# syl051088/DynaAlign

Hardware: AMD Instinct MI355X
Metric: sequence-pairs/sec (MinHash k=4 n_hash=500; NW BLOSUM62) at 1/2/4/8 MI355X (higher is better)
Workload: dtype u32

## Files before the change

### dynaalign_amd/csrc/api.cpp

```cpp
#include <sched.h>

#include <algorithm>
#include <atomic>
#include <chrono>
#include <climits>
#include <cmath>
#include <condition_variable>
#include <cstddef>
#include <map>
#include <memory>
#include <cstdlib>
#include <cstring>
#include <functional>
#include <mutex>
#include <random>
#include <string>
#include <thread>
#include <vector>

#include "da_common.hpp"

namespace da { size_t destroy_cached_comms(); }

namespace da {
// ... 202 lines not shown
  std::condition_variable cv_, done_;
  uint64_t gen_ = 0;
  bool stop_ = false;
  const std::function<void(size_t, size_t)> *fn_ = nullptr;
  size_t len_ = 0, part_ = 0;
  int pending_ = 0;
};

void widen_u16_to_f64(double *dst, const uint16_t *src, size_t b, size_t e, const double *table) {
  typedef double v2d __attribute__((ext_vector_type(2)));
  size_t i = b;
  if (i < e && (reinterpret_cast<uintptr_t>(dst + i) & 15)) { dst[i] = table[src[i]]; ++i; }
  for (; i + 2 <= e; i += 2) {
    const v2d v = {table[src[i]], table[src[i + 1]]};
    __builtin_nontemporal_store(v, reinterpret_cast<v2d *>(dst + i));
  }
  if (i < e) dst[i] = table[src[i]];
}

int d2h_pipelined(void *dst, const void *d_src, size_t bytes, const double *table = nullptr) {
  constexpr size_t CHUNK = (size_t)64 << 20, SMALL = (size_t)8 << 20;
  constexpr int RING = 4, MAX_WORKERS = 32;
  int WORKERS = table ? 16 : 8;
  if (da::config().d2h_threads > 0) WORKERS = std::min(MAX_WORKERS, da::config().d2h_threads);
  {
    const unsigned hw = std::thread::hardware_concurrency();
    cpu_set_t cs;
    int avail = (sched_getaffinity(0, sizeof cs, &cs) == 0) ? CPU_COUNT(&cs) : (int)hw;
    if (avail > 0 && WORKERS > avail) WORKERS = avail;
  }
  if (bytes <= CHUNK && !table) {
    DA_HIP_TRY(hipMemcpy(dst, d_src, bytes, hipMemcpyDeviceToHost));
    return DA_OK;
  }
  if (bytes <= SMALL && table) {
    std::vector<uint16_t> codes(bytes / 2);
    DA_HIP_TRY(hipMemcpy(codes.data(), d_src, bytes, hipMemcpyDeviceToHost));
    widen_u16_to_f64(static_cast<double *>(dst), codes.data(), 0, bytes / 2, table);
    return DA_OK;
  }
  if (da::config().plain_d2h && !table) {
    DA_HIP_TRY(hipMemcpy(dst, d_src, bytes, hipMemcpyDeviceToHost));
    return DA_OK;
  }
  struct Slot { void *pin = nullptr; hipEvent_t ev = nullptr; };
  Slot ring[RING];
  hipStream_t st = nullptr;
  int rc = DA_OK;
  auto cleanup = [&]() {
    if (st) (void)hipStreamSynchronize(st);
    for (auto &s : ring) { if (s.pin) (void)hipHostFree(s.pin); if (s.ev) (void)hipEventDestroy(s.ev); }
    if (st) (void)hipStreamDestroy(st);
  };
  auto check = [&](hipError_t e, const char *what) {
    if (e != hipSuccess && rc == DA_OK) rc = fail(DA_ERR_HIP, "%s failed: %s", what, hipGetErrorString(e));
    return e == hipSuccess;
  };
  if (!check(hipStreamCreateWithFlags(&st, hipStreamNonBlocking), "hipStreamCreate")) { cleanup(); return rc; }
  for (auto &s : ring)
    if (!check(hipHostMalloc(&s.pin, CHUNK, hipHostMallocDefault), "hipHostMalloc") ||
        !check(hipEventCreateWithFlags(&s.ev, hipEventDisableTiming), "hipEventCreate")) { cleanup(); return rc; }
  if (!check(hipDeviceSynchronize(), "hipDeviceSynchronize")) { cleanup(); return rc; }
  {
    CopyPool pool(WORKERS - 1);
    const size_t nchunk = (bytes + CHUNK - 1) / CHUNK;
    for (size_t c = 0; c < nchunk + RING - 1 && rc == DA_OK; ++c) {
      if (c < nchunk) {
        const size_t off = c * CHUNK, len = std::min(CHUNK, bytes - off);
        if (!check(hipMemcpyAsync(ring[c % RING].pin, static_cast<const char *>(d_src) + off, len, hipMemcpyDeviceToHost, st), "hipMemcpyAsync") ||
            !check(hipEventRecord(ring[c % RING].ev, st), "hipEventRecord")) break;
      }
      if (c >= RING - 1) {
        const size_t done = c - (RING - 1), off = done * CHUNK, len = std::min(CHUNK, bytes - off);
        if (!check(hipEventSynchronize(ring[done % RING].ev), "hipEventSynchronize")) break;
        const char *src = static_cast<const char *>(ring[done % RING].pin);
        if (table) {
          double *d = static_cast<double *>(dst) + off / 2;
          const uint16_t *s16 = reinterpret_cast<const uint16_t *>(src);
          pool.run_split(len / 2, [=](size_t b, size_t e) { widen_u16_to_f64(d, s16, b, e, table); });
        } else {
          char *d = static_cast<char *>(dst) + off;
          pool.run_split(len, [=](size_t b, size_t e) { memcpy(d + b, src + b, e - b); });
        }
      }
    }
  }
  cleanup();
  return rc;
}

struct Trace {
  const bool on = da::config().trace;
  const char *what;
  std::chrono::steady_clock::time_point t0 = std::chrono::steady_clock::now(), last = t0;
  explicit Trace(const char *w) : what(w) {}
  void mark(const char *step) {
    if (!on) return;
    (void)hipDeviceSynchronize();
    const auto now = std::chrono::steady_clock::now();
    fprintf(stderr, "[dynaalign] %s: %-28s %9.3f ms (total %9.3f ms)\n", what, step,
            std::chrono::duration<double, std::milli>(now - last).count(), std::chrono::duration<double, std::milli>(now - t0).count());
    last = now;
  }
};

double now_ms() { return std::chrono::duration<double, std::milli>(std::chrono::steady_clock::now().time_since_epoch()).count(); }

int64_t rows_per_block(int64_t n, size_t bytes_per_elem) {
  size_t free_b = 0, total_b = 0;
  if (hipMemGetInfo(&free_b, &total_b) != hipSuccess) free_b = (size_t)8 << 30;
  {
    int dev = 0;
    (void)hipGetDevice(&dev);
    std::lock_guard<std::mutex> g(big_cache().m);
    for (const auto &e : big_cache().parked) if (e.dev == dev) free_b += e.bytes;
  }
  size_t budget = free_b / 2;
  if (da::config().block_bytes) budget = (size_t)da::config().block_bytes;
  int64_t rows = (int64_t)(budget / ((size_t)n * bytes_per_elem));
  rows = rows / 128 * 128;
  if (rows < 128) rows = 128;
  return std::min(rows, n);
}

}
}

using namespace da;

namespace da {
namespace {
bool env_flag(const char *name) { return getenv(name) != nullptr; }
int64_t env_i64(const char *name, int64_t dflt) { const char *e = getenv(name); return e ? atoll(e) : dflt; }
uint64_t env_u64(const char *name, uint64_t dflt) { const char *e = getenv(name); return e ? strtoull(e, nullptr, 10) : dflt; }
enum MhExpand { MH_EXPAND_DEFAULT, MH_EXPAND_ROWS, MH_EXPAND_ROWSPIPE, MH_EXPAND_PIPE, MH_EXPAND_TILES };
Config parse_config() {
  Config c;
  c.mh_no_dedup = env_flag("DYNAALIGN_MH_NO_DEDUP");
  c.mh_no_sparse = env_flag("DYNAALIGN_MH_NO_SPARSE");
  c.mh_no_pipe = env_flag("DYNAALIGN_MH_NO_PIPE");
  c.mh_pipe_one_stream = env_flag("DYNAALIGN_MH_PIPE_ONE_STREAM");
  c.mh_dedup_min_n = env_i64("DYNAALIGN_MH_DEDUP_MIN_N", -1);
  c.mh_dedup_max_pct = env_i64("DYNAALIGN_MH_DEDUP_MAX_PCT", -1);
  c.mh_sparse_max_pairs = std::min<uint64_t>(env_u64("DYNAALIGN_MH_SPARSE_MAX_PAIRS", 400000000ull), 0xfffffff0ull);
  c.mh_no_hybrid = env_flag("DYNAALIGN_MH_NO_HYBRID");
  c.mh_hybrid_min_n = env_i64("DYNAALIGN_MH_HYBRID_MIN_N", -1);
  c.mh_hybrid_dedup = env_flag("DYNAALIGN_MH_HYBRID_DEDUP");
  if (const char *e = getenv("DYNAALIGN_MH_EXPAND"))
    c.mh_expand = !strcmp(e, "rows") ? MH_EXPAND_ROWS : !strcmp(e, "rowspipe") ? MH_EXPAND_ROWSPIPE : !strcmp(e, "pipe") ? MH_EXPAND_PIPE
                : !strcmp(e, "tiles") ? MH_EXPAND_TILES : MH_EXPAND_DEFAULT;
  c.mh_pipe_step = (int)std::max<int64_t>(0, env_i64("DYNAALIGN_MH_PIPE_STEP", 0));
  c.mh_pipe_wg = (int)std::max<int64_t>(0, std::min<int64_t>(4, env_i64("DYNAALIGN_MH_PIPE_WG", 0)));
  c.mh_pipe_head = (int)std::max<int64_t>(0, env_i64("DYNAALIGN_MH_PIPE_HEAD", 0));
  const int pb = (int)env_i64("DYNAALIGN_PLANE_BITS", 0);
  c.plane_bits = (pb == 32 || pb == 16 || pb == 15 || pb == 14 || pb == 12) ? pb : 0;
  c.k2_no_asm = env_flag("DYNAALIGN_K2_NO_ASM");
  c.k2_persist = env_flag("DYNAALIGN_K2_PERSIST");
  c.k2_wg_per_cu = (int)std::max<int64_t>(0, env_i64("DYNAALIGN_K2_WG_PER_CU", 0));
  c.nw_no_dedup = env_flag("DYNAALIGN_NW_NO_DEDUP");
  c.nw_int32 = env_flag("DYNAALIGN_NW_INT32");
  c.nw_no_prefix = env_flag("DYNAALIGN_NW_NO_PREFIX_SHARE");
  c.nw_dedup_min_n = env_i64("DYNAALIGN_NW_DEDUP_MIN_N", -1);
  c.no_host_widen = env_flag("DYNAALIGN_NO_HOST_WIDEN");
  c.plain_d2h = env_flag("DYNAALIGN_PLAIN_D2H");
  c.no_buffer_cache = env_flag("DYNAALIGN_NO_BUFFER_CACHE");
  c.d2h_threads = (int)std::max<int64_t>(0, env_i64("DYNAALIGN_D2H_THREADS", 0));
  c.buffer_cache_pct = (int)std::max<int64_t>(0, std::min<int64_t>(90, env_i64("DYNAALIGN_BUFFER_CACHE_PCT", 30)));
  c.block_bytes = env_u64("DYNAALIGN_BLOCK_BYTES", 0);
  c.trace = env_flag("DYNAALIGN_TRACE");
  c.louvain_debug = env_flag("DYNAALIGN_LOUVAIN_DEBUG");
  c.louvain_threads = (int)std::max<int64_t>(0, env_i64("DYNAALIGN_LOUVAIN_THREADS", 0));
  return c;
}
std::atomic<const Config *> g_config{nullptr};
}
const Config &config() {
  const Config *c = g_config.load(std::memory_order_acquire);
  if (!c) {
    const Config *fresh = new Config(parse_config());
    if (g_config.compare_exchange_strong(c, fresh, std::memory_order_acq_rel)) c = fresh;
    else delete fresh;
  }
  return *c;
}
}
extern "C" void da_config_reload(void) { da::g_config.store(new da::Config(da::parse_config()), std::memory_order_release); }

extern "C" {

const char *da_last_error(void) { return last_error_ref().c_str(); }

const char *da_status_message(int status) {
  switch (status) {
    case DA_ERR_EMPTY_INPUT: return "Input sequences vector cannot be empty";
    case DA_ERR_BAD_K: return "'k' must be a positive integer";
    case DA_ERR_BAD_NHASH: return "Number of hash functions must be positive";
    case DA_ERR_BAD_MATRIX: return "Invalid substitution matrix name: %s";
    case DA_ERR_BAD_RESIDUE_SEQ1: return "Invalid amino acid in sequence1: %c";
    case DA_ERR_BAD_RESIDUE_SEQ2: return "Invalid amino acid in sequence2: %c";
    case DA_ERR_NOMEM: return "out of memory";
    case DA_ERR_NO_DEVICE: return "no usable HIP device";
    case DA_ERR_HIP: return "HIP runtime error";
    case DA_ERR_UNSUPPORTED: return "unsupported by the gfx950 kernels";
    case DA_ERR_BAD_ARG: return "bad argument";
    default: return "";
  }
}

int da_abi_version(void) { return DA_ABI_VERSION; }

size_t da_release_device_memory(void) {
  (void)da::destroy_cached_comms();
  return big_cache().release(-1);
}

int da_device_count(void) {
  int cnt = 0;
  if (hipGetDeviceCount(&cnt) != hipSuccess) return 0;
  return cnt;
}

int da_hash_family_seeds(uint32_t seed, int n_hash, uint32_t *seeds_out) {
  if (n_hash < 0 || (n_hash > 0 && !seeds_out)) return fail(DA_ERR_BAD_ARG, "bad n_hash / seeds_out");
  uint32_t s[624];
  s[0] = seed;
  for (uint32_t i = 1; i < 624; ++i) s[i] = 1812433253u * (s[i - 1] ^ (s[i - 1] >> 30)) + i;
  int pos = 624;
  for (int o = 0; o < n_hash; ++o) {
    if (pos == 624) {
      for (int i = 0; i < 624; ++i) {
        const uint32_t y = (s[i] & 0x80000000u) | (s[(i + 1) % 624] & 0x7fffffffu);
        s[i] = s[(i + 397) % 624] ^ (y >> 1) ^ ((y & 1u) ? 0x9908b0dfu : 0u);
      }
      pos = 0;
    }
    uint32_t y = s[pos++];
    y ^= y >> 11;
    y ^= (y << 7) & 0x9d2c5680u;
    y ^= (y << 15) & 0xefc60000u;
    y ^= y >> 18;
    seeds_out[o] = y;
  }
  return DA_OK;
}

uint32_t da_random_seed(void) { return std::random_device{}(); }

int da_matrix_id(const char *matrix_name) {
  if (matrix_name)
    for (int i = 0; i < matrix_count_host(); ++i)
      if (strcmp(matrix_name, matrix_name_host(i)) == 0) return i;
  fail(DA_ERR_BAD_MATRIX, "Invalid substitution matrix name: %s", matrix_name ? matrix_name : "");
  return -1;
}


int da_dev_minhash_signatures(const uint8_t *d_residues, const int64_t *d_offsets, int64_t n,
                              int64_t total_residues, int64_t max_len, int k, int n_hash,
                              const uint32_t *d_seeds, uint32_t *d_sig, int64_t ld_sig, void *stream) {
  (void)total_residues; (void)max_len;
  int rc = validate_mh(n, k, n_hash);
  if (rc != DA_OK) return rc;
  if (!d_residues || !d_offsets || !d_seeds || !d_sig) return fail(DA_ERR_BAD_ARG, "NULL device pointer");
  if (ld_sig < n_hash) return fail(DA_ERR_BAD_ARG, "ld_sig (%lld) < n_hash (%d)", (long long)ld_sig, n_hash);
  return launch_minhash_signatures(d_residues, d_offsets, n, k, n_hash, d_seeds, d_sig, ld_sig,
                                   static_cast<hipStream_t>(stream));
}

static int env_plane_bits() { return da::config().plane_bits; }
struct Dictionary { bool ok = false; int max_ids = 0, bits_data = 32; int *d_status = nullptr; };
static int run_dictionary(const uint32_t *d_sig, int64_t ld_sig, int64_t n, int n_hash, int min_bits, void *d_work, size_t work_bytes,
                          Dictionary *dict, hipStream_t stream) {
  if (n > DA_DICT_MAX_N || min_bits == 32) return DA_OK;
  if (!d_work || work_bytes < mh_planes_workspace_bytes(n, n_hash))
    return fail(DA_ERR_BAD_ARG, "workspace smaller than da_mh_planes_workspace_bytes(n, n_hash)");
  int rc;
  if ((rc = launch_mh_dictionary(d_sig, ld_sig, n, n_hash, d_work, &dict->d_status, stream)) != DA_OK) return rc;
  int status[2] = {0, 0};
  DA_HIP_TRY(hipMemcpyAsync(status, dict->d_status, sizeof(status), hipMemcpyDeviceToHost, stream));
  DA_HIP_TRY(hipStreamSynchronize(stream));
  dict->ok = status[0] == 0; dict->max_ids = status[1];
  dict->bits_data = dict->ok ? mh_plane_bits_for(status[1]) : 32;
  return DA_OK;
}
static int planes_from(const Dictionary &dict, const uint32_t *d_sig, int64_t ld_sig, int64_t n, int n_hash, int min_bits, const void *d_work,
                       uint32_t *d_planes, int *bits_out, hipStream_t stream) {
  *bits_out = dict.ok ? std::max(dict.bits_data, min_bits) : 32;
  return dict.ok ? launch_ids_to_planes(d_work, n, n_hash, *bits_out, d_planes, stream) : launch_sig_to_planes(d_sig, ld_sig, n, n_hash, d_planes, stream);
}
static int build_planes(const uint32_t *d_sig, int64_t ld_sig, int64_t n, int n_hash, int min_bits, void *d_work,
                        size_t work_bytes, uint32_t *d_planes, int *bits_out, hipStream_t stream) {
  min_bits = std::max(min_bits, env_plane_bits());
  Dictionary dict;
  const int rc = run_dictionary(d_sig, ld_sig, n, n_hash, min_bits, d_work, work_bytes, &dict, stream);
  return rc != DA_OK ? rc : planes_from(dict, d_sig, ld_sig, n, n_hash, min_bits, d_work, d_planes, bits_out, stream);
}

size_t da_mh_planes_workspace_bytes(int64_t n, int n_hash) { return mh_planes_workspace_bytes(n, n_hash); }
int64_t da_mh_planes_words(int64_t n, int n_hash) { return mh_planes_words(n, n_hash); }

int da_dev_mh_planes(const uint32_t *d_sig, int64_t ld_sig, int64_t n, int n_hash, int min_plane_bits, void *d_work,
                     size_t work_bytes, uint32_t *d_planes, int64_t planes_words, int *plane_bits_out, void *stream) {
  if (n <= 0) return fail(DA_ERR_EMPTY_INPUT, "%s", da_status_message(DA_ERR_EMPTY_INPUT));
  if (n_hash <= 0) return fail(DA_ERR_BAD_NHASH, "%s", da_status_message(DA_ERR_BAD_NHASH));
  if (!d_sig || !d_planes || !plane_bits_out) return fail(DA_ERR_BAD_ARG, "NULL pointer");
  if (ld_sig < n_hash) return fail(DA_ERR_BAD_ARG, "ld_sig (%lld) < n_hash (%d)", (long long)ld_sig, n_hash);
  if (min_plane_bits != 0 && min_plane_bits != 12 && min_plane_bits != 14 && min_plane_bits != 15 && min_plane_bits != 16 && min_plane_bits != 32)
    return fail(DA_ERR_BAD_ARG, "min_plane_bits must be 0, 12, 14, 15, 16 or 32 (got %d)", min_plane_bits);
  if ((reinterpret_cast<uintptr_t>(d_planes) & 15) || planes_words < mh_planes_words(n, n_hash))
    return fail(DA_ERR_BAD_ARG, "bit-plane buffer must be 16-byte aligned and hold da_mh_planes_words(n, n_hash) = %lld words",
                (long long)mh_planes_words(n, n_hash));
  if (reinterpret_cast<uintptr_t>(d_work) & 255) return fail(DA_ERR_BAD_ARG, "workspace must be 256-byte aligned");
  return build_planes(d_sig, ld_sig, n, n_hash, min_plane_bits, d_work, work_bytes, d_planes, plane_bits_out,
                      static_cast<hipStream_t>(stream));
}

int da_dev_mh_compare(const uint32_t *d_planes, int plane_bits, int64_t n, int n_hash,
                      int64_t row_begin, int64_t row_end, int symmetric, int kind, void *d_out,
                      int64_t ld, void *stream) {
  if (n <= 0) return fail(DA_ERR_EMPTY_INPUT, "%s", da_status_message(DA_ERR_EMPTY_INPUT));
  if (n_hash <= 0) return fail(DA_ERR_BAD_NHASH, "%s", da_status_message(DA_ERR_BAD_NHASH));
  if (!d_planes || !d_out) return fail(DA_ERR_BAD_ARG, "NULL device pointer");
  if (row_begin < 0 || row_end > n || row_begin > row_end) return fail(DA_ERR_BAD_ARG, "bad row range");
  if (symmetric && (row_begin != 0 || row_end != n))
    return fail(DA_ERR_BAD_ARG, "symmetric mode needs the full row range");
  if (ld < n) return fail(DA_ERR_BAD_ARG, "ld (%lld) < n (%lld)", (long long)ld, (long long)n);
  if (kind != DA_OUT_F64 && kind != DA_OUT_COMPACT) return fail(DA_ERR_BAD_ARG, "bad output kind");
  if (n_hash > 65535)
    return fail(DA_ERR_UNSUPPORTED, "the compare kernel counts in 16 bits: n_hash <= 65535 (got %d)", n_hash);
  if (reinterpret_cast<uintptr_t>(d_planes) & 15) return fail(DA_ERR_BAD_ARG, "bit-plane buffer must be 16-byte aligned");
  if (plane_bits != 8 && plane_bits != 12 && plane_bits != 14 && plane_bits != 15 && plane_bits != 16 && plane_bits != 32)
    return fail(DA_ERR_BAD_ARG, "plane_bits must be 8, 12, 14, 15, 16 or 32 (got %d)", plane_bits);
  return launch_mh_compare(d_planes, n, n_hash, row_begin, row_end, symmetric != 0, kind, d_out, ld,
                           static_cast<hipStream_t>(stream), plane_bits);
}

namespace {
struct PipeRes { hipStream_t side = nullptr, alt[2] = {nullptr, nullptr}; std::vector<hipEvent_t> ev; int dev = 0; };
struct PipePool { std::mutex m; std::vector<PipeRes *> idle[64]; };
static PipePool &pipe_pool() { static PipePool *p = new PipePool; return *p; }
static PipeRes *pipe_acquire(size_t events) {
  int dev = 0;
  if (hipGetDevice(&dev) != hipSuccess) return nullptr;
  PipeRes *r = nullptr;
  {
    std::lock_guard<std::mutex> g(pipe_pool().m);
    auto &v = pipe_pool().idle[dev & 63];
    if (!v.empty()) { r = v.back(); v.pop_back(); }
  }
  if (!r) {
    r = new PipeRes;
    r->dev = dev;
    if (hipStreamCreateWithFlags(&r->side, hipStreamNonBlocking) != hipSuccess || hipStreamCreateWithFlags(&r->alt[0], hipStreamNonBlocking) != hipSuccess ||
        hipStreamCreateWithFlags(&r->alt[1], hipStreamNonBlocking) != hipSuccess) { delete r; return nullptr; }
  }
  while (r->ev.size() < events) {
    hipEvent_t e = nullptr;
    if (hipEventCreate(&e) != hipSuccess) break;
    r->ev.push_back(e);
  }
  if (r->ev.size() < events) { std::lock_guard<std::mutex> g(pipe_pool().m); pipe_pool().idle[dev & 63].push_back(r); return nullptr; }
  return r;
}
struct PipeLease {
  PipeRes *const r;
  explicit PipeLease(size_t events, bool want = true) : r(want ? pipe_acquire(events) : nullptr) {}
  ~PipeLease() {
    if (!r) return;
    (void)hipStreamSynchronize(r->side); (void)hipStreamSynchronize(r->alt[0]); (void)hipStreamSynchronize(r->alt[1]);
    std::lock_guard<std::mutex> g(pipe_pool().m);
    pipe_pool().idle[r->dev & 63].push_back(r);
  }
};
static int count_unique(const uint8_t *d_bytes, const int64_t *d_offsets, int64_t n, const NwDedupPlan &p, hipStream_t stream, int64_t *U) {
  int rc;
  if ((rc = launch_nw_dedup_count(d_bytes, d_offsets, n, p, stream)) != DA_OK) return rc;
  int32_t M = 0, S = 0;
  DA_HIP_TRY(hipMemcpyAsync(&M, p.pm + n, 4, hipMemcpyDeviceToHost, stream));
  DA_HIP_TRY(hipMemcpyAsync(&S, p.ps + n, 4, hipMemcpyDeviceToHost, stream));
  DA_HIP_TRY(hipStreamSynchronize(stream));
  *U = (int64_t)M + S; return DA_OK;
}
enum MhForm { MH_DIRECT = 0, MH_TILES = 1, MH_SPARSE = 2, MH_TILES_PIPE = 3, MH_ROWS = 4, MH_ROWS_PIPE = 5 };
struct MhRoute { int64_t n = 0, unique = 0, hybrid_pairs = -1; int taken = MH_DIRECT, plane_bits = 0, chunks = 0, expand_launches = 0, hybrid_bits_before = 0; bool packed_table = false; float ms[6] = {0, 0, 0, 0, 0, 0}; };
static MhRoute &mh_route() { static thread_local MhRoute r; return r; }
struct MhEvents {
  hipEvent_t e[7] = {nullptr, nullptr, nullptr, nullptr, nullptr, nullptr, nullptr};
  ~MhEvents() { for (hipEvent_t x : e) if (x) (void)hipEventDestroy(x); }
  hipEvent_t operator[](int i) const { return e[i]; }
  static void ms(MhRoute &r, int i, hipEvent_t from, hipEvent_t to) { (void)hipEventElapsedTime(&r.ms[i], from, to); }
  void steps(MhRoute &r, int count) const { for (int i = 0; i < count; ++i) ms(r, i, e[i], e[i + 1]); }
};
struct LaunchUnion {
  hipEvent_t origin; float total = 0, covered_to = 0;
  void add(hipEvent_t begin, hipEvent_t end) {
    float b = 0, e = 0;
    (void)hipEventElapsedTime(&b, origin, begin); (void)hipEventElapsedTime(&e, origin, end);
    if (e > covered_to) { total += e - std::max(b, covered_to); covered_to = e; }
  }
};
struct MhDedup { int64_t U = 0; bool take = false, rows = false; DevBuf work; NwDedupPlan p{}; std::vector<int32_t> ub; };
static int mh_dedup_plan(const uint8_t *d_res, const int64_t *d_off, int64_t n, int64_t total, int n_hash, const double *d_out, int64_t ld,
                         MhDedup *d, hipStream_t stream) {
  const Config &cfg = da::config();
  int rc;
  d->U = n;
  const int64_t min_n = cfg.mh_dedup_min_n >= 0 ? cfg.mh_dedup_min_n : 2048;
  if (n < min_n || n > 0x7ffffff0LL || total <= 0 || n_hash > 2047 || cfg.mh_no_dedup) return DA_OK;
  if ((rc = d->work.alloc(nw_dedup_workspace_bytes(n, total))) != DA_OK) return rc;
  d->p = nw_dedup_layout(d->work.p, n, total);
  if ((rc = count_unique(d_res, d_off, n, d->p, stream, &d->U)) != DA_OK) return rc;
  const int64_t U = d->U;
  const int64_t max_pct = cfg.mh_dedup_max_pct >= 0 ? cfg.mh_dedup_max_pct
                        : expand_stream_ok(n, std::min<int64_t>(U, 65536), n_hash, d_out, ld) ? 68 : 60;
  d->take = U > 0 && U * 100 <= n * max_pct && expand_rows_workspace_bytes(n, U, DA_OUT_F64, false, n_hash, 0) != 0;
  if (!d->take) return DA_OK;
  if ((rc = launch_nw_dedup_build(d_res, d_off, n, U, d->p, stream, true)) != DA_OK) return rc;
  d->rows = cfg.mh_expand <= MH_EXPAND_ROWSPIPE && expand_stream_ok(n, U, n_hash, d_out, ld);
  if (d->rows) return DA_OK;
  const int64_t NB = mh_sym_bands(n);
  std::vector<int32_t> b((size_t)NB);
  d->ub.resize((size_t)NB + 1);
  DA_HIP_TRY(hipMemcpy2DAsync(d->ub.data(), 4, d->p.pm, 4096, 4, (size_t)NB, hipMemcpyDeviceToHost, stream));
  DA_HIP_TRY(hipMemcpy2DAsync(b.data(), 4, d->p.ps, 4096, 4, (size_t)NB, hipMemcpyDeviceToHost, stream));
  DA_HIP_TRY(hipStreamSynchronize(stream));
  for (int64_t q = 0; q < NB; ++q) d->ub[(size_t)q] += b[(size_t)q];
  d->ub[(size_t)NB] = (int32_t)U;
  return DA_OK;
}
constexpr int HY_KEEP = 254;
enum class MhOperand { dense, sparse, split };
struct MhAdmission { MhOperand form = MhOperand::dense; uint64_t pairs = 0; const uint16_t *codes = nullptr, *dense = nullptr; int64_t ld_ids = 0; };
static int mh_admit(const Dictionary &dict, void *d_work, int64_t n, int n_hash, bool ask_sparse, int split_from_bits, MhAdmission *a,
                    hipStream_t stream) {
  const Config &cfg = da::config();
  if (!dict.ok || env_plane_bits() != 0) return DA_OK;
  const int64_t hy_min_n = cfg.mh_hybrid_min_n >= 0 ? cfg.mh_hybrid_min_n : 16384;
  const bool sparse_ok = ask_sparse && dict.max_ids >= 1 && dict.max_ids <= 32768 && n >= 2048 && n_hash + 1 <= 2048 && !cfg.mh_no_sparse;
  const bool split_ok = dict.bits_data >= split_from_bits && dict.bits_data <= 16 && dict.max_ids <= 32768 && n >= hy_min_n && n <= 131072 &&
                        n_hash > 32 && n_hash + 1 <= 2048 && !cfg.mh_no_hybrid && !cfg.k2_no_asm;
  if (!sparse_ok && !split_ok) return DA_OK;
  int rc;
  int64_t ld_ids = 0;
  const uint16_t *ids = mh_dictionary_codes(d_work, n, n_hash, &ld_ids);
  unsigned long long *d_stats = reinterpret_cast<unsigned long long *>(dict.d_status + 4);
  const uint16_t *dense = nullptr, *rare = nullptr;
  unsigned long long st[4] = {0, 0, 0, 0};
  if ((rc = split_ok ? launch_mh_heavy_split(d_work, n, n_hash, dict.max_ids, HY_KEEP, &dense, &rare, d_stats, stream)
                     : launch_mh_sparse_count(ids, ld_ids, n, n_hash, dict.max_ids, d_stats, stream)) != DA_OK) return rc;
  DA_HIP_TRY(hipMemcpyAsync(split_ok ? st : st + 2, d_stats, split_ok ? sizeof(st) : 16, hipMemcpyDeviceToHost, stream));
  DA_HIP_TRY(hipStreamSynchronize(stream));
  const double pairs_all = 0.5 * (double)n * (double)(n - 1);
  if (sparse_ok && st[2] <= mh_sparse_pairs_limit() && st[3] <= 4096 && (double)st[2] <= pairs_all * (double)n_hash / 5000.0)
    *a = MhAdmission{MhOperand::sparse, st[2], ids, nullptr, ld_ids};
  else if (split_ok && st[0] <= mh_sparse_pairs_limit() && st[1] <= 4096 && (double)st[0] <= pairs_all * (double)n_hash / 25000.0)
    *a = MhAdmission{MhOperand::split, st[0], rare, dense, ld_ids};
  return DA_OK;
}
struct MhCodes {
  DevBuf sig, planes, pwork, scratch, entries32, entries;
  int64_t m = 0;
  int n_hash = 0, bits = 32;
  Dictionary dict;
  MhAdmission adm;
  bool split() const { return adm.form == MhOperand::split; }
  int lists(hipStream_t st) const {
    return launch_mh_sparse_lists(adm.codes, adm.ld_ids, m, n_hash, dict.max_ids, adm.pairs, scratch.as<uint32_t>(), entries32.as<uint32_t>(), entries.as<uint16_t>(), st);
  }
  int fixup(int kind, void *out, int64_t ld_out, hipStream_t st, int64_t tr0 = 0, int64_t tr1 = -1) const {
    return launch_mh_sparse_fixup(scratch.as<uint32_t>(), entries.as<uint16_t>(), m, n_hash, dict.max_ids, adm.ld_ids, kind, out, ld_out, tr0,
                                  tr1 < 0 ? (m + 127) / 128 : tr1, st);
  }
};
static int mh_codes(const uint8_t *d_res, const int64_t *d_off, int64_t m, int k, int n_hash, const uint32_t *d_seeds, bool ask_sparse,
                    int split_from_bits, MhCodes *c, hipStream_t stream) {
  int rc;
  const int64_t lds = sig_ld_for(n_hash);
  const size_t wb = mh_planes_workspace_bytes(m, n_hash);
  c->m = m; c->n_hash = n_hash;
  if ((rc = c->sig.alloc((size_t)m * lds * sizeof(uint32_t))) != DA_OK || (rc = c->planes.alloc((size_t)mh_planes_words(m, n_hash) * sizeof(uint32_t))) != DA_OK ||
      (rc = c->pwork.alloc(wb)) != DA_OK) return rc;
  uint32_t *sig = c->sig.as<uint32_t>(), *planes = c->planes.as<uint32_t>();
  if ((rc = launch_minhash_signatures(d_res, d_off, m, k, n_hash, d_seeds, sig, lds, stream)) != DA_OK) return rc;
  const int min_bits = env_plane_bits();
  const Dictionary &dict = c->dict;
  if ((rc = run_dictionary(sig, lds, m, n_hash, min_bits, c->pwork.p, wb, &c->dict, stream)) != DA_OK) return rc;
  if ((rc = mh_admit(dict, c->pwork.p, m, n_hash, ask_sparse, split_from_bits, &c->adm, stream)) != DA_OK) return rc;
  if (c->adm.form != MhOperand::dense &&
      (c->scratch.alloc(mh_sparse_scratch_words(m, n_hash, dict.max_ids, c->adm.ld_ids) * 4) != DA_OK ||
       c->entries32.alloc((size_t)c->adm.pairs * 4 + 16) != DA_OK || c->entries.alloc((size_t)c->adm.pairs * 2 + 16) != DA_OK)) {
    (void)hipGetLastError();
    c->scratch.release(); c->entries32.release(); c->entries.release();
    c->adm = MhAdmission();
  }
  if (c->adm.form == MhOperand::sparse) { c->bits = 0; return DA_OK; }
  if (c->split()) { c->bits = 8; return launch_ids_to_planes(c->pwork.p, m, n_hash, 8, planes, stream, c->adm.dense); }
  return planes_from(dict, sig, lds, m, n_hash, min_bits, c->pwork.p, planes, &c->bits, stream);
}
struct MhCall {
  int64_t n; int n_hash; double *out; int64_t ld; hipStream_t stream; MhRoute &route; const MhEvents &ev; const MhCodes &c; const MhDedup &d;
  uint16_t *dtab = nullptr; int64_t ld_d = 0; void *ex = nullptr; bool pk = false;
};
constexpr int MH_NO_PIPE = -1;
static int mh_finish(const MhCall &k, int last_event, MhForm taken, int steps) {
  DA_HIP_TRY(hipEventRecord(k.ev[last_event], k.stream));
  DA_HIP_TRY(hipStreamSynchronize(k.stream));
  k.route.taken = taken; k.ev.steps(k.route, steps);
  return DA_OK;
}
static int mh_sparse(const MhCall &k) {
  const MhCodes &c = k.c;
  int rc;
  if ((rc = launch_mh_sparse(c.adm.codes, c.adm.ld_ids, k.n, k.n_hash, c.dict.max_ids, c.adm.pairs, c.scratch.as<uint32_t>(), c.entries32.as<uint32_t>(),
                             c.entries.as<uint16_t>(), k.out, k.ld, k.stream, k.ev[3])) != DA_OK || (rc = mh_finish(k, 4, MH_SPARSE, 3)) != DA_OK) return rc;
  k.route.unique = (int64_t)c.adm.pairs;
  MhEvents::ms(k.route, 4, k.ev[3], k.ev[4]);
  return DA_OK;
}
static int mh_direct(const MhCall &k) {
  const MhCodes &c = k.c;
  int rc;
  const PipeLease lease(1, c.split());
  PipeRes *const pr = lease.r;
  if (pr) {
    DA_HIP_TRY(hipStreamWaitEvent(pr->side, k.ev[2], 0));
    if ((rc = c.lists(pr->side)) != DA_OK) return rc;
    DA_HIP_TRY(hipEventRecord(pr->ev[0], pr->side));
  } else if (c.split() && (rc = c.lists(k.stream)) != DA_OK) return rc;
  if ((rc = launch_mh_compare(c.planes.as<uint32_t>(), k.n, k.n_hash, 0, k.n, true, DA_OUT_F64, k.out, k.ld, k.stream, c.bits)) != DA_OK) return rc;
  if (pr) DA_HIP_TRY(hipStreamWaitEvent(k.stream, pr->ev[0], 0));
  if (c.split() && (rc = c.fixup(DA_OUT_F64, k.out, k.ld, k.stream)) != DA_OK) return rc;
  return mh_finish(k, 3, MH_DIRECT, 3);
}
static int mh_one_stream(const MhCall &k) {
  const MhCodes &c = k.c;
  int rc;
  if (c.split() && (rc = c.lists(k.stream)) != DA_OK) return rc;
  if ((rc = k.pk ? launch_mh_compare_pk(c.planes.as<uint32_t>(), k.d.U, k.n_hash, reinterpret_cast<uint8_t *>(k.dtab), k.stream)
                 : launch_mh_compare(c.planes.as<uint32_t>(), k.d.U, k.n_hash, 0, k.d.U, true, DA_OUT_COMPACT, k.dtab, k.ld_d, k.stream, c.bits)) != DA_OK)
    return rc;
  if (c.split() && (rc = c.fixup(DA_OUT_COMPACT, k.dtab, k.ld_d, k.stream)) != DA_OK) return rc;
  DA_HIP_TRY(hipEventRecord(k.ev[3], k.stream));
  if ((rc = k.d.rows ? launch_expand_stream(k.dtab, k.ld_d, k.d.p.uidx, k.n, k.d.U, k.n_hash, k.out, k.ld, k.ex, k.stream, k.ev[4], k.pk)
                     : launch_expand_unique(k.dtab, k.ld_d, k.d.p.uidx, k.n, DA_OUT_F64, false, k.n_hash, k.out, k.ld, k.stream, 0,
                                            static_cast<uint16_t *>(k.ex), k.d.p.ufirst, k.d.U, k.ev[4], k.ev[5])) != DA_OK) return rc;
  k.route.chunks = k.route.expand_launches = 1;
  return k.d.rows ? mh_finish(k, 5, MH_ROWS, 5) : mh_finish(k, 6, MH_TILES, 6);
}
static int mh_rows_pipe(const MhCall &k) {
  const Config &cfg = da::config();
  const MhCodes &c = k.c;
  const int64_t U = k.d.U, KB = mh_sym_bands(U);
  const hipStream_t stream = k.stream;
  int rc;
  const bool two = expand_stream_packed(k.n_hash);
  const int wg = cfg.mh_pipe_wg > 0 ? cfg.mh_pipe_wg : two ? 2 : 1, head = cfg.mh_pipe_head > 0 ? cfg.mh_pipe_head : two ? 1 : 4,
            step = cfg.mh_pipe_step > 0 ? cfg.mh_pipe_step : two ? 8 : 4;
  const bool alt = !cfg.mh_pipe_one_stream;
  std::vector<int64_t> cuts{0};
  while (cuts.back() < KB) cuts.push_back(std::min(KB, cuts.back() + (cuts.size() == 1 ? head : step)));
  const size_t C = cuts.size() - 1;
  const PipeLease lease(3 * C + 2);
  PipeRes *const pr = lease.r;
  if (!pr) return MH_NO_PIPE;
  hipEvent_t *pe = pr->ev.data();
  DA_HIP_TRY(hipStreamWaitEvent(pr->side, k.ev[2], 0));
  if ((rc = launch_mh_compare_edges_u16(c.planes.as<uint32_t>(), U, k.n_hash, k.dtab, k.ld_d, stream, c.bits, k.pk)) != DA_OK) return rc;
  if ((rc = launch_expand_stream_lists(k.d.p.uidx, k.n, U, k.ex, stream)) != DA_OK) return rc;
  DA_HIP_TRY(hipEventRecord(pe[3 * C], stream));
  if (c.split()) {
    if ((rc = c.lists(stream)) != DA_OK) return rc;
    DA_HIP_TRY(hipEventRecord(pe[3 * C + 1], stream));
  }
  if (alt) { DA_HIP_TRY(hipStreamWaitEvent(pr->alt[0], pe[3 * C], 0)); DA_HIP_TRY(hipStreamWaitEvent(pr->alt[1], pe[3 * C], 0)); }
  for (size_t ci = 0; ci < C; ++ci) {
    if ((rc = launch_mh_compare_bands_u16(c.planes.as<uint32_t>(), U, k.n_hash, k.dtab, k.ld_d, cuts[ci], cuts[ci + 1], ci == 0 ? 4 : wg, pr->side, c.bits,
                                          k.pk)) != DA_OK) return rc;
    if (c.split()) {
      if (ci == 0) { DA_HIP_TRY(hipStreamWaitEvent(pr->side, pe[3 * C], 0)); DA_HIP_TRY(hipStreamWaitEvent(pr->side, pe[3 * C + 1], 0)); }
      if ((rc = c.fixup(DA_OUT_COMPACT, k.dtab, k.ld_d, pr->side, cuts[ci] * 8, cuts[ci + 1] * 8)) != DA_OK) return rc;
    }
    DA_HIP_TRY(hipEventRecord(pe[3 * ci], pr->side));
    const hipStream_t es = alt ? pr->alt[ci & 1] : stream;
    DA_HIP_TRY(hipStreamWaitEvent(es, pe[3 * ci], 0));
    DA_HIP_TRY(hipEventRecord(pe[3 * ci + 1], es));
    if ((rc = launch_expand_stream_rows(k.dtab, k.ld_d, k.d.p.uidx, k.n, U, k.n_hash, k.out, k.ld, k.ex, cuts[ci] * 1024, cuts[ci + 1] * 1024, es,
                                        (int)ci, k.pk)) != DA_OK) return rc;
    DA_HIP_TRY(hipEventRecord(pe[3 * ci + 2], es));
  }
  if (alt) for (size_t ci = (C >= 2 ? C - 2 : 0); ci < C; ++ci) DA_HIP_TRY(hipStreamWaitEvent(stream, pe[3 * ci + 2], 0));
  if ((rc = mh_finish(k, 5, MH_ROWS_PIPE, 2)) != DA_OK) return rc;
  k.route.chunks = k.route.expand_launches = (int)C;
  MhEvents::ms(k.route, 2, k.ev[2], pe[3 * (C - 1)]);
  MhEvents::ms(k.route, 3, k.ev[2], pe[3 * C]);
  LaunchUnion expand{k.ev[2]};
  for (size_t ci = 0; ci < C; ++ci) expand.add(pe[3 * ci + 1], pe[3 * ci + 2]);
  k.route.ms[4] = expand.total;
  return DA_OK;
}
static int mh_tiles_pipe(const MhCall &k) {
  const Config &cfg = da::config();
  const MhCodes &c = k.c;
  uint16_t *ftab = static_cast<uint16_t *>(k.ex);
  const hipStream_t stream = k.stream;
  const std::vector<int32_t> &ub = k.d.ub;
  const int64_t U = k.d.U, KB = mh_sym_bands(U), NB = (int64_t)ub.size() - 1, ld_f = ceil_div(k.n, 8) * 8;
  int rc;
  const int step = cfg.mh_pipe_step > 0 ? cfg.mh_pipe_step : 4, wg = cfg.mh_pipe_wg > 0 ? cfg.mh_pipe_wg : 2;
  const bool alt = !cfg.mh_pipe_one_stream;
  struct Chunk { int64_t kb0, kb1, ob0, ob1; };
  std::vector<Chunk> chunks;
  for (int64_t kb = 0, ob = 0; kb < KB;) {
    const int64_t kb1 = std::min(KB, kb + (chunks.empty() ? 1 : step));
    int64_t ob1 = ob;
    if (kb1 == KB) ob1 = NB;
    else while (ob1 < NB && (int64_t)ub[(size_t)ob1 + 1] <= kb1 * 1024) ++ob1;
    chunks.push_back({kb, kb1, ob, ob1});
    kb = kb1; ob = ob1;
  }
  const size_t C = chunks.size();
  const PipeLease lease(5 * C);
  PipeRes *const pr = lease.r;
  if (!pr) return MH_NO_PIPE;
  hipEvent_t *pe = pr->ev.data();
  DA_HIP_TRY(hipStreamWaitEvent(pr->side, k.ev[2], 0));
  if ((rc = launch_mh_compare_edges_u16(c.planes.as<uint32_t>(), U, k.n_hash, k.dtab, k.ld_d, pr->side, c.bits)) != DA_OK) return rc;
  if (c.split() && (rc = c.lists(pr->side)) != DA_OK) return rc;
  for (size_t ci = 0; ci < C; ++ci) {
    const Chunk &ch = chunks[ci];
    if ((rc = launch_mh_compare_bands_u16(c.planes.as<uint32_t>(), U, k.n_hash, k.dtab, k.ld_d, ch.kb0, ch.kb1, wg, pr->side, c.bits)) != DA_OK) return rc;
    if (c.split() && (rc = c.fixup(DA_OUT_COMPACT, k.dtab, k.ld_d, pr->side, ch.kb0 * 8, ch.kb1 * 8)) != DA_OK) return rc;
    DA_HIP_TRY(hipEventRecord(pe[5 * ci], pr->side));
    DA_HIP_TRY(hipStreamWaitEvent(stream, pe[5 * ci], 0));
    DA_HIP_TRY(hipEventRecord(pe[5 * ci + 1], stream));
    if ((rc = launch_gather_columns(k.dtab, k.ld_d, k.d.p.uidx, k.d.p.ufirst, k.n, U, ftab, ld_f, false, stream, 1, 0, ch.kb0 * 1024,
                                    std::min(U, ch.kb1 * 1024))) != DA_OK) return rc;
    DA_HIP_TRY(hipEventRecord(pe[5 * ci + 2], stream));
    const hipStream_t es = alt ? pr->alt[ci & 1] : stream;
    if (alt) DA_HIP_TRY(hipStreamWaitEvent(es, pe[5 * ci + 2], 0));
    DA_HIP_TRY(hipEventRecord(pe[5 * ci + 3], es));
    if ((rc = launch_expand_rows(ftab, ld_f, k.d.p.uidx, k.n, false, k.n_hash, 0, k.out, k.ld, ch.ob0, ch.ob1, es)) != DA_OK) return rc;
    DA_HIP_TRY(hipEventRecord(pe[5 * ci + 4], es));
  }
  if (alt) for (size_t ci = (C >= 2 ? C - 2 : 0); ci < C; ++ci) DA_HIP_TRY(hipStreamWaitEvent(stream, pe[5 * ci + 4], 0));
  DA_HIP_TRY(hipEventRecord(k.ev[5], stream));
  if ((rc = launch_expand_unique(k.dtab, k.ld_d, k.d.p.uidx, k.n, DA_OUT_F64, false, k.n_hash, k.out, k.ld, stream, 0, ftab, k.d.p.ufirst, U,
                                 nullptr, nullptr, 1, 0, true)) != DA_OK) return rc;
  if ((rc = mh_finish(k, 6, MH_TILES_PIPE, 2)) != DA_OK) return rc;
  k.route.chunks = (int)C;
  MhEvents::ms(k.route, 2, k.ev[2], pe[5 * (C - 1)]);
  LaunchUnion expand{k.ev[2]};
  for (size_t ci = 0; ci < C; ++ci) {
    float g = 0;
    (void)hipEventElapsedTime(&g, pe[5 * ci + 1], pe[5 * ci + 2]);
    k.route.ms[3] += g;
    if (chunks[ci].ob1 > chunks[ci].ob0) { ++k.route.expand_launches; expand.add(pe[5 * ci + 3], pe[5 * ci + 4]); }
  }
  k.route.ms[4] = expand.total;
  MhEvents::ms(k.route, 5, k.ev[5], k.ev[6]);
  return DA_OK;
}
}

static int mh_full_symmetric(const uint8_t *d_res, const int64_t *d_off, int64_t n, int64_t total, int k, int n_hash,
                             const uint32_t *d_seeds, double *d_out, int64_t ld, hipStream_t stream) {
  const Config &cfg = da::config();
  int rc;
  MhRoute &route = mh_route() = MhRoute();
  route.n = n;
  MhEvents ev;
  for (auto &e : ev.e) DA_HIP_TRY(hipEventCreate(&e));
  DA_HIP_TRY(hipEventRecord(ev[0], stream));
  MhDedup d;
  if ((rc = mh_dedup_plan(d_res, d_off, n, total, n_hash, d_out, ld, &d, stream)) != DA_OK) return rc;
  route.unique = d.U;
  DA_HIP_TRY(hipEventRecord(ev[1], stream));
  MhCodes c;
  if ((rc = mh_codes(d.take ? d.p.ucodes : d_res, d.take ? d.p.uoff : d_off, d.take ? d.U : n, k, n_hash, d_seeds, !d.take && d.U * 10 >= n * 9,
                     d.take && !cfg.mh_hybrid_dedup ? 13 : 12, &c, stream)) != DA_OK) return rc;
  route.plane_bits = c.bits;
  if (c.split()) { route.hybrid_pairs = (int64_t)c.adm.pairs; route.hybrid_bits_before = c.dict.bits_data; }
  DA_HIP_TRY(hipEventRecord(ev[2], stream));
  MhCall call{n, n_hash, d_out, ld, stream, route, ev, c, d};
  if (!d.take) return c.adm.form == MhOperand::sparse ? mh_sparse(call) : mh_direct(call);
  DevBuf dtab, ex;
  call.pk = d.rows && !c.split() && mh_compare_pk_ok(d.U, n_hash, c.bits);
  route.packed_table = call.pk;
  call.ld_d = call.pk ? pk_lo_bytes(d.U) : (d.U + 7) / 8 * 8;
  if ((rc = dtab.alloc(call.pk ? pk_table_bytes(d.U) : (size_t)d.U * (size_t)call.ld_d * 2)) != DA_OK) return rc;
  if ((rc = ex.alloc(d.rows ? expand_stream_scratch_bytes(n, d.U) : expand_rows_workspace_bytes(n, d.U, DA_OUT_F64, false, n_hash, 0))) != DA_OK) return rc;
  call.dtab = dtab.as<uint16_t>(); call.ex = ex.p;
  const bool pipe = !cfg.mh_no_pipe && mh_compare_bands_ok(d.U, n_hash, c.bits, dtab.p, call.ld_d) &&
                    (d.rows ? cfg.mh_expand != MH_EXPAND_ROWS : cfg.mh_expand != MH_EXPAND_TILES && (ld & 1) == 0 && (reinterpret_cast<uintptr_t>(d_out) & 15) == 0);
  if (pipe && (rc = d.rows ? mh_rows_pipe(call) : mh_tiles_pipe(call)) != MH_NO_PIPE) return rc;
  return mh_one_stream(call);
}

int da_dev_similarity_mh(const uint8_t *d_residues, const int64_t *d_offsets, int64_t n, int64_t total_residues, int k, int n_hash,
                         const uint32_t *d_seeds, double *d_out, int64_t ld, void *stream) {
  int rc = validate_mh(n, k, n_hash);
  if (rc != DA_OK) return rc;
  if (!d_residues || !d_offsets || !d_seeds || !d_out) return fail(DA_ERR_BAD_ARG, "NULL device pointer");
  if (ld < n) return fail(DA_ERR_BAD_ARG, "ld (%lld) < n (%lld)", (long long)ld, (long long)n);
  if (n_hash > 65535) return fail(DA_ERR_UNSUPPORTED, "the compare kernel counts in 16 bits: n_hash <= 65535 (got %d); da_similarity_mh handles more", n_hash);
  return mh_full_symmetric(d_residues, d_offsets, n, total_residues, k, n_hash, d_seeds, d_out, ld, static_cast<hipStream_t>(stream));
}

int da_mh_last_route_chunks(int *chunks_out, int *expand_launches_out) {
  const MhRoute &r = mh_route();
  if (chunks_out) *chunks_out = r.chunks;
  if (expand_launches_out) *expand_launches_out = r.expand_launches;
  return DA_OK;
}

int da_mh_last_route_split(int64_t *rare_incidences_out, int *plane_bits_without_out) {
  const MhRoute &r = mh_route();
  if (rare_incidences_out) *rare_incidences_out = r.hybrid_pairs;
  if (plane_bits_without_out) *plane_bits_without_out = r.hybrid_bits_before;
  return DA_OK;
}

extern "C" int da_debug_mh_last_table_packed(int *packed_out) {
  if (!packed_out) return fail(DA_ERR_BAD_ARG, "NULL pointer");
  *packed_out = mh_route().packed_table ? 1 : 0;
  return DA_OK;
}

int da_mh_last_route(int64_t *n_out, int64_t *unique_out, int *dedup_taken_out, int *plane_bits_out, double *ms6_out) {
  const MhRoute &r = mh_route();
  if (n_out) *n_out = r.n;
  if (unique_out) *unique_out = r.unique;
  if (dedup_taken_out) *dedup_taken_out = r.taken;
  if (plane_bits_out) *plane_bits_out = r.plane_bits;
  if (ms6_out) for (int i = 0; i < 6; ++i) ms6_out[i] = r.ms[i];
  return DA_OK;
}

size_t da_dev_unique_plan_bytes(int64_t n, int64_t total_bytes) {
  if (n <= 0) return 256;
  return nw_dedup_workspace_bytes(n, total_bytes > 0 ? total_bytes : 1);
}

int da_dev_unique_plan(const uint8_t *d_bytes, const int64_t *d_offsets, int64_t n, int64_t total_bytes, void *d_work, size_t work_bytes,
                       da_unique_plan *plan, void *stream_v) {
  if (!plan || plan->struct_size < sizeof(da_unique_plan)) return fail(DA_ERR_BAD_ARG, "da_unique_plan: NULL or struct_size too small");
  if (n <= 0) return fail(DA_ERR_EMPTY_INPUT, "%s", da_status_message(DA_ERR_EMPTY_INPUT));
  if (n > 0x7ffffff0LL) return fail(DA_ERR_UNSUPPORTED, "unique plan: n too large");
  if (!d_bytes || !d_offsets || !d_work) return fail(DA_ERR_BAD_ARG, "NULL device pointer");
  if ((reinterpret_cast<uintptr_t>(d_work) & 255) || work_bytes < da_dev_unique_plan_bytes(n, total_bytes))
    return fail(DA_ERR_BAD_ARG, "workspace must be 256-byte aligned and hold da_dev_unique_plan_bytes(n, total_bytes) bytes");
  hipStream_t stream = static_cast<hipStream_t>(stream_v);
  int rc;
  const NwDedupPlan p = nw_dedup_layout(d_work, n, total_bytes > 0 ? total_bytes : 1);
  int64_t U = 0;
  if ((rc = count_unique(d_bytes, d_offsets, n, p, stream, &U)) != DA_OK) return rc;
  if (U <= 0 || U > n) return fail(DA_ERR_HIP, "unique plan: inconsistent counts (%lld unique of %lld)", (long long)U, (long long)n);
  if ((rc = launch_nw_dedup_build(d_bytes, d_offsets, n, U, p, stream)) != DA_OK) return rc;
  plan->n = n; plan->unique = U;
  plan->d_uidx = p.uidx; plan->d_ufirst = p.ufirst; plan->d_ulast = p.ulast;
  plan->d_ubytes = p.ucodes; plan->d_uoffsets = p.uoff;
  plan->d_minfirst = p.minfirst; plan->d_maxlast = p.maxlast;
  return DA_OK;
}

int da_dev_shards_to_table(const void *d_gathered, int64_t ld_g, int64_t n, int world, int value_bits, uint16_t *d_table, int64_t ld_table,
                           void *stream) {
  if (n <= 0) return fail(DA_ERR_EMPTY_INPUT, "%s", da_status_message(DA_ERR_EMPTY_INPUT));
  if (!d_gathered || !d_table) return fail(DA_ERR_BAD_ARG, "NULL device pointer");
  if (world < 1 || ld_table < n) return fail(DA_ERR_BAD_ARG, "bad world / leading dimension");
  if (value_bits != 0 && (value_bits < 1 || value_bits > 16)) return fail(DA_ERR_BAD_ARG, "value_bits must be 0 (uint16 blocks) or 1..16");
  const ShardGeom g = shard_geom(n, world, 128);
  if (value_bits == 0 && ld_g < g.W) return fail(DA_ERR_BAD_ARG, "ld_g (%lld) < da_shard_ld (%lld)", (long long)ld_g, (long long)g.W);
  return launch_shards_to_table(d_gathered, ld_g, g, value_bits, d_table, ld_table, static_cast<hipStream_t>(stream));
}

size_t da_dev_expand_workspace_bytes(int64_t n, int64_t unique, int is_nw, int n_hash, int nw_max_len) {
  const size_t b = expand_rows_workspace_bytes(n, unique, DA_OUT_F64, is_nw != 0, n_hash, nw_max_len);
  return b ? b : 256;
}

int da_dev_expand_unique(const uint16_t *d_table, int64_t ld_table, int table_world, const da_unique_plan *plan, int is_nw, int n_hash,
                         int nw_max_len, void *d_work, size_t work_bytes, double *d_out, int64_t ld, void *stream) {
  if (!plan || plan->struct_size < sizeof(da_unique_plan) || !plan->d_uidx || !plan->d_ufirst) return fail(DA_ERR_BAD_ARG, "bad da_unique_plan");
  if (!d_table || !d_out) return fail(DA_ERR_BAD_ARG, "NULL device pointer");
  const int64_t n = plan->n, U = plan->unique;
  if (n <= 0 || U <= 0 || U > n || ld < n || ld_table < U) return fail(DA_ERR_BAD_ARG, "bad sizes / leading dimensions");
  if (!is_nw && (n_hash <= 0 || n_hash > 65535)) return fail(DA_ERR_BAD_NHASH, "%s", da_status_message(DA_ERR_BAD_NHASH));
  if (table_world < 1) return fail(DA_ERR_BAD_ARG, "table_world must be >= 1");
  const int64_t rows_local = table_world > 1 ? ceil_div(ceil_div(U, 128), table_world) * 128 : 0;
  if (!is_nw && table_world == 1 && expand_stream_ok(n, U, n_hash, d_out, ld) && (ld_table & 7) == 0 && ld_table <= 65536 &&
      (reinterpret_cast<uintptr_t>(d_table) & 15) == 0) {
    const size_t lists_bytes = expand_stream_scratch_bytes(n, U);
    if (d_work && work_bytes >= lists_bytes && (reinterpret_cast<uintptr_t>(d_work) & 15) == 0)
      return launch_expand_stream(d_table, ld_table, plan->d_uidx, n, U, n_hash, d_out, ld, d_work, static_cast<hipStream_t>(stream));
    DevBuf lists;
    int rc = lists.alloc(lists_bytes);
    if (rc != DA_OK) return rc;
    rc = launch_expand_stream(d_table, ld_table, plan->d_uidx, n, U, n_hash, d_out, ld, lists.p, static_cast<hipStream_t>(stream));
    DA_HIP_TRY(hipStreamSynchronize(static_cast<hipStream_t>(stream)));
    return rc;
  }
  const size_t need = expand_rows_workspace_bytes(n, U, DA_OUT_F64, is_nw != 0, n_hash, nw_max_len);
  uint16_t *d_F = (need && d_work && work_bytes >= need && (reinterpret_cast<uintptr_t>(d_work) & 15) == 0) ? static_cast<uint16_t *>(d_work) : nullptr;
  if ((ld_table & 7) || (reinterpret_cast<uintptr_t>(d_table) & 15)) d_F = nullptr;
  return launch_expand_unique(d_table, ld_table, plan->d_uidx, n, DA_OUT_F64, is_nw != 0, n_hash, d_out, ld, static_cast<hipStream_t>(stream),
                              nw_max_len, d_F, plan->d_ufirst, U, nullptr, nullptr, table_world, rows_local);
}

size_t da_dev_unique_rows_bytes(int64_t n, int64_t unique) {
  if (n <= 0 || unique <= 0) return 256;
  return (size_t)unique * (size_t)(ceil_div(n, 8) * 8) * 2;
}

int da_dev_unique_rows(const uint16_t *d_table, int64_t ld_table, const da_unique_plan *plan, uint16_t *d_rows, void *stream) {
  if (!plan || plan->struct_size < sizeof(da_unique_plan) || !plan->d_uidx || !plan->d_ufirst) return fail(DA_ERR_BAD_ARG, "bad da_unique_plan");
  if (!d_table || !d_rows) return fail(DA_ERR_BAD_ARG, "NULL device pointer");
  if (ld_table < plan->unique) return fail(DA_ERR_BAD_ARG, "ld_table < unique");
  return launch_gather_columns(d_table, ld_table, plan->d_uidx, plan->d_ufirst, plan->n, plan->unique, d_rows, ceil_div(plan->n, 8) * 8, true,
                               static_cast<hipStream_t>(stream));
}

int da_dev_nw_unique_rows(const da_unique_plan *plan, int64_t max_len, int matrix_id, int gap_open, int gap_ext, int rank, int world,
                          uint16_t *d_out, int64_t ld, void *stream) {
  if (!plan || plan->struct_size < sizeof(da_unique_plan) || !plan->d_ubytes || !plan->d_uoffsets || !plan->d_ufirst || !plan->d_minfirst ||
      !plan->d_maxlast)
    return fail(DA_ERR_BAD_ARG, "bad da_unique_plan");
  if (!d_out) return fail(DA_ERR_BAD_ARG, "NULL device pointer");
  const int64_t U = plan->unique;
  if (world < 1 || rank < 0 || rank >= world || ld < U) return fail(DA_ERR_BAD_ARG, "bad rank / world / leading dimension");
  if (matrix_id < 0 || matrix_id >= matrix_count_host()) return fail(DA_ERR_BAD_MATRIX, "%s", da_status_message(DA_ERR_BAD_MATRIX));
  if (max_len < 1 || max_len > 64 || gap_open < 0 || gap_ext < 0)
    return fail(DA_ERR_UNSUPPORTED, "the ordered unique-table sweep serves sequences of 1..64 residues and penalties >= 0");
  return launch_nw(plan->d_ubytes, plan->d_uoffsets, U, max_len, matrix_id, gap_open, gap_ext, 0, U, false, DA_OUT_COMPACT, d_out, ld, nullptr, 0,
                   static_cast<hipStream_t>(stream), rank, world > 1 ? world : 0, plan->d_ufirst, plan->d_minfirst, plan->d_maxlast);
}

int da_dev_nw_encode(const uint8_t *d_residues, int64_t total_residues, uint8_t *d_codes,
                     int32_t *d_bad, void *stream) {
  if (total_residues > 0 && (!d_residues || !d_codes || !d_bad)) return fail(DA_ERR_BAD_ARG, "NULL device pointer");
  return launch_nw_encode(d_residues, total_residues, d_codes, d_bad, static_cast<hipStream_t>(stream));
}

struct NwRoute { int64_t n = 0, unique = 0; int taken = 0; float plan_ms = 0, dp_ms = 0, expand_ms = 0; };
static NwRoute &nw_route() { static thread_local NwRoute r; return r; }

static int nw_full_symmetric(const uint8_t *d_codes, const int64_t *d_offsets, int64_t n, int64_t total, int64_t max_len, int mid,
                             int gap_open, int gap_ext, int kind, void *d_out, int64_t ld, hipStream_t stream, int64_t *unique_out = nullptr) {
// ... 1178 lines not shown
```

### dynaalign_amd/csrc/da_common.hpp

```cpp
#pragma once

#include <hip/hip_runtime.h>

#include <cstdarg>
#include <cstdint>
#include <cstdio>
#include <string>

#include "../../include/dynaalign.h"

namespace da {
struct Config {
  bool mh_no_dedup = false, mh_no_sparse = false, mh_no_pipe = false, mh_pipe_one_stream = false;
  int64_t mh_dedup_min_n = -1, mh_dedup_max_pct = -1;
  uint64_t mh_sparse_max_pairs = 400000000ull;
  bool mh_no_hybrid = false, mh_hybrid_dedup = false;
  int64_t mh_hybrid_min_n = -1;
  int mh_expand = 0;
  int mh_pipe_step = 0, mh_pipe_wg = 0, mh_pipe_head = 0;
  int plane_bits = 0;
  bool k2_no_asm = false, k2_persist = false;
  int k2_wg_per_cu = 0;
  bool nw_no_dedup = false, nw_int32 = false, nw_no_prefix = false;
  int64_t nw_dedup_min_n = -1;
  bool no_host_widen = false, plain_d2h = false, no_buffer_cache = false;
  int d2h_threads = 0, buffer_cache_pct = 30;
  uint64_t block_bytes = 0;
  bool trace = false, louvain_debug = false;
  int louvain_threads = 0;
};
const Config &config();


std::string &last_error_ref();
int fail(int code, const char *fmt, ...) __attribute__((format(printf, 2, 3)));

#define DA_HIP_TRY(expr)                                                              \
  do {                                                                                \
    hipError_t _e = (expr);                                                           \
    if (_e != hipSuccess)                                                             \
      return ::da::fail(_e == hipErrorNoDevice || _e == hipErrorInvalidDevice         \
                            ? DA_ERR_NO_DEVICE                                        \
                            : DA_ERR_HIP,                                             \
                        "%s failed: %s (%s:%d)", #expr, hipGetErrorString(_e),        \
                        __FILE__, __LINE__);                                          \
  } while (0)

inline int64_t ceil_div(int64_t a, int64_t b) { return (a + b - 1) / b; }

struct ShardGeom {
  int64_t n, W, rows;
  int world, tile, T, Q, Qh;
};
__host__ __device__ inline int64_t shard_back(int64_t W, int64_t n) { return W - ((n + 7) / 8) * 8; }
inline ShardGeom shard_geom(int64_t n, int world, int tile) {
  ShardGeom g;
  g.n = n; g.world = world; g.tile = tile;
  g.T = (int)ceil_div(n, tile);
  g.Q = (int)ceil_div(g.T, world);
  g.Qh = (g.Q + 1) / 2;
  g.W = ceil_div(n, 8) * 8 + (int64_t)world * tile;
  g.rows = (int64_t)g.Qh * tile;
  return g;
}

__host__ __device__ inline int k2_slot(int r) { return (((r >> 5) * 2 + (r & 1)) << 4) + ((r & 31) >> 1); }
__host__ __device__ inline int k2_row_of_slot(int s) { return ((s >> 5) << 5) + ((s & 15) << 1) + ((s >> 4) & 1); }
struct PlaneGeom {
  int pl;
  int sp;
  int segs;
  int nst;
  int64_t blocks, copy_words;
};
__host__ __device__ inline PlaneGeom plane_geom(int64_t n, int n_hash, int pl) {
  PlaneGeom g;
  g.pl = pl; g.sp = pl == 32 ? 16 : pl; g.segs = g.sp / 4;
  g.nst = ((n_hash + 31) / 32) * (pl / g.sp);
  g.blocks = (n + 127) / 128;
  g.copy_words = g.blocks * g.nst * 128 * g.sp;
  return g;
}
__host__ __device__ inline int64_t plane_unit_word(const PlaneGeom &g, int64_t row, int st, int seg) {
  const int rs = k2_slot((int)(row & 127));
  const int xs = g.segs == 4 ? (rs >> 2) & 3 : 0;
  return ((((row >> 7) * g.nst + st) * 128 + rs) * g.segs + (seg ^ xs)) * 4;
}
constexpr int K2_PAD16_SLOT_WORDS = 20;
__host__ __device__ inline int64_t pad16_copy_words(int64_t n, int n_hash) {
  return ((n + 127) / 128) * (int64_t)((n_hash + 31) / 32) * 128 * K2_PAD16_SLOT_WORDS;
}
__host__ __device__ inline int64_t pad16_base_words(int64_t n, int n_hash) { return 2 * plane_geom(n, n_hash, 16).copy_words; }
__host__ __device__ inline int64_t pad16_slot_word(int64_t n, int n_hash, int64_t row, int group) {
  const int64_t nst = (n_hash + 31) / 32;
  return (((row >> 7) * nst + group) * 128 + k2_slot((int)(row & 127))) * K2_PAD16_SLOT_WORDS;
}
inline int64_t mh_planes_words(int64_t n, int n_hash) {
  if (n <= 0 || n_hash <= 0) return 0;
  const int64_t raw = 2 * plane_geom(n, n_hash, 32).copy_words;
  const int64_t p16 = pad16_base_words(n, n_hash) + 2 * pad16_copy_words(n, n_hash);
  return raw > p16 ? raw : p16;
}

__host__ __device__ inline int64_t pk_lo_bytes(int64_t U) { return (U + 127) / 128 * 128; }
__host__ __device__ inline int64_t pk_row_bytes(int64_t lo_bytes) { return lo_bytes + lo_bytes / 8; }
inline size_t pk_table_bytes(int64_t U) { return (size_t)U * (size_t)pk_row_bytes(pk_lo_bytes(U)); }

int launch_minhash_signatures(const uint8_t *d_res, const int64_t *d_off, int64_t n,
                              int k, int n_hash, const uint32_t *d_seeds, uint32_t *d_sig,
                              int64_t ld_sig, hipStream_t stream);
int launch_mh_compare(const uint32_t *d_planes, int64_t n, int n_hash,
                      int64_t row_begin, int64_t row_end, bool symmetric, int kind,
                      void *d_out, int64_t ld, hipStream_t stream, int plane_bits = 32, int tile_stride = 1,
                      bool upper_only = false, int fold_q = 0, int64_t fold_w = 0);
int64_t mh_sym_bands(int64_t n);
int64_t mh_sym_band_prefix(int64_t n, int64_t band);
bool mh_compare_bands_ok(int64_t n, int n_hash, int plane_bits, const void *d_out, int64_t ld);
int launch_mh_compare_bands_u16(const uint32_t *d_planes, int64_t n, int n_hash, uint16_t *d_out, int64_t ld, int64_t band_begin,
                                int64_t band_end, int wg_per_cu, hipStream_t stream, int plane_bits = 12, bool pk = false);
int launch_mh_compare_edges_u16(const uint32_t *d_planes, int64_t n, int n_hash, uint16_t *d_out, int64_t ld, hipStream_t stream, int plane_bits = 12,
                                bool pk = false);
bool mh_compare_pk_ok(int64_t n, int n_hash, int plane_bits);
int launch_mh_compare_pk(const uint32_t *d_planes, int64_t n, int n_hash, uint8_t *d_tab, hipStream_t stream);
size_t mh_sparse_pairs_limit();
int launch_mh_sparse_count(const uint16_t *d_idsT, int64_t ld_ids, int64_t n, int n_hash, int max_ids, unsigned long long *d_stats, hipStream_t stream);
size_t mh_sparse_scratch_words(int64_t n, int n_hash, int max_ids, int64_t ld_ids);
int launch_mh_sparse(const uint16_t *d_idsT, int64_t ld_ids, int64_t n, int n_hash, int max_ids, uint64_t pairs, uint32_t *d_scratch,
                     uint32_t *d_entries32, uint16_t *d_entries, double *d_out, int64_t ld, hipStream_t stream, hipEvent_t after_buckets = nullptr);
int launch_mh_sparse_lists(const uint16_t *d_idsT, int64_t ld_ids, int64_t n, int n_hash, int max_ids, uint64_t pairs, uint32_t *d_scratch,
                           uint32_t *d_entries32, uint16_t *d_entries, hipStream_t stream);
int launch_mh_sparse_fixup(const uint32_t *d_scratch, const uint16_t *d_entries, int64_t n, int n_hash, int max_ids, int64_t ld_ids, int kind, void *d_out,
                           int64_t ld, int64_t tile_row_begin, int64_t tile_row_end, hipStream_t stream);
const uint16_t *mh_dictionary_codes(const void *d_work, int64_t n, int n_hash, int64_t *ld_ids);
constexpr int64_t DA_DICT_MAX_N = 131068;
size_t mh_planes_workspace_bytes(int64_t n, int n_hash);
int launch_mh_dictionary(const uint32_t *d_sig, int64_t ld_sig, int64_t n, int n_hash, void *d_work,
                         int **d_status_out, hipStream_t stream);
int mh_plane_bits_for(int max_ids);
int launch_ids_to_planes(const void *d_work, int64_t n, int n_hash, int plane_bits, uint32_t *d_planes,
                         hipStream_t stream, const uint16_t *d_codes = nullptr);
int launch_mh_heavy_split(void *d_work, int64_t n, int n_hash, int max_ids, int keep, const uint16_t **d_dense_out, const uint16_t **d_sparse_out,
                          unsigned long long *d_stats, hipStream_t stream);
int launch_sig_to_planes(const uint32_t *d_sig, int64_t ld_sig, int64_t n, int n_hash, uint32_t *d_planes,
                         hipStream_t stream);
int launch_finalize_sharded(const uint16_t *d_g, int64_t ld_g, const ShardGeom &geom, bool is_nw, int n_hash,
                            double *d_out, int64_t ld, hipStream_t stream);
int64_t shard_packed_bytes(const ShardGeom &g, int value_bits);
int launch_shards_to_table(const void *d_g, int64_t ld_g, const ShardGeom &geom, int value_bits, uint16_t *d_table, int64_t ld,
                           hipStream_t stream);
int launch_pack_shard(const uint16_t *d_local, int64_t ld, const ShardGeom &geom, int value_bits, uint8_t *d_packed,
                      hipStream_t stream);
int launch_finalize_packed(const uint8_t *d_g, const ShardGeom &geom, int value_bits, int n_hash, double *d_out, int64_t ld,
                           hipStream_t stream);
int launch_nw_encode(const uint8_t *d_res, int64_t total, uint8_t *d_codes, int32_t *d_bad,
                     hipStream_t stream);
int launch_nw(const uint8_t *d_codes, const int64_t *d_off, int64_t n, int64_t max_len,
              int matrix_id, int gap_open, int gap_ext, int64_t row_begin, int64_t row_end,
              bool symmetric, int kind, void *d_out, int64_t ld, int32_t *d_score,
              int64_t ld_score, hipStream_t stream, int shard_rank = 0, int shard_world = 0,
              const int32_t *ord_first = nullptr, const int32_t *ord_minfirst = nullptr, const int32_t *ord_maxlast = nullptr,
              const int32_t *ord_perm = nullptr, const uint8_t *ord_lcp = nullptr);
size_t nw_sort_unique_workspace_bytes(int64_t n);
int launch_nw_sort_unique(const uint8_t *d_codes, const int64_t *d_off, int64_t n, void *d_work, size_t work_bytes, const int32_t **perm_out,
                          const uint8_t **lcp_out, hipStream_t stream);
struct NwDedupPlan {
  uint32_t *table; uint32_t table_size;
  int32_t *rep, *mult, *last, *fm, *fs, *pm, *ps, *uid_of, *uidx, *ufirst, *ulast, *ulen, *minfirst, *maxlast;
  int64_t *uoff;
  uint8_t *ucodes;
  size_t bytes;
};
NwDedupPlan nw_dedup_layout(void *work, int64_t n, int64_t total);
size_t nw_dedup_workspace_bytes(int64_t n, int64_t total);
int launch_nw_dedup_count(const uint8_t *d_codes, const int64_t *d_off, int64_t n, const NwDedupPlan &p, hipStream_t stream);
int launch_nw_dedup_build(const uint8_t *d_codes, const int64_t *d_off, int64_t n, int64_t U, const NwDedupPlan &p, hipStream_t stream,
                          bool first_order = false);
int launch_expand_unique(const uint16_t *d_D, int64_t ld_d, const int32_t *d_uidx, int64_t n, int kind, bool is_nw, int n_hash,
                         void *d_out, int64_t ld, hipStream_t stream, int nw_max_len = 0, uint16_t *d_F = nullptr,
                         const int32_t *d_ufirst = nullptr, int64_t U = 0, hipEvent_t after_gather = nullptr, hipEvent_t after_rows = nullptr,
                         int table_world = 1, int64_t table_rows_local = 0,
                         bool only_leftover = false);
bool expand_stream_ok(int64_t n, int64_t U, int n_hash, const void *d_out, int64_t ld);
size_t expand_stream_scratch_bytes(int64_t n, int64_t U);
bool expand_stream_packed(int n_hash);
int launch_expand_stream(const uint16_t *d_D, int64_t ld_d, const int32_t *d_uidx, int64_t n, int64_t U, int n_hash, double *d_out, int64_t ld,
                         void *d_scratch, hipStream_t stream, hipEvent_t after_lists = nullptr, bool pk = false);
int launch_expand_stream_lists(const int32_t *d_uidx, int64_t n, int64_t U, void *d_scratch, hipStream_t stream);
int launch_expand_stream_rows(const uint16_t *d_D, int64_t ld_d, const int32_t *d_uidx, int64_t n, int64_t U, int n_hash, double *d_out, int64_t ld,
                              void *d_scratch, int64_t row_begin, int64_t row_end, hipStream_t stream, int launch_no,
                              bool pk = false);
int launch_expand_rows(const uint16_t *d_F, int64_t ld_f, const int32_t *d_uidx, int64_t n, bool is_nw, int n_hash, int nw_max_len,
                       double *d_out, int64_t ld, int64_t band_begin, int64_t band_end, hipStream_t stream);
size_t expand_rows_workspace_bytes(int64_t n, int64_t U, int kind, bool is_nw, int n_hash, int nw_max_len);
int launch_upper_histogram(const uint16_t *d_m, int64_t ld, int64_t n, int nbins, unsigned long long *d_hist,
                           hipStream_t stream, int rank = 0, int world = 0, const int32_t *d_rowmap = nullptr);
int launch_extract_edges(const uint16_t *d_m, int64_t ld, int64_t n, const uint8_t *d_keep, int nbins,
                         bool include_diagonal, int32_t *d_i, int32_t *d_j, uint16_t *d_v, int64_t capacity,
                         unsigned long long *d_count, hipStream_t stream, int rank = 0, int world = 0,
                         const int32_t *d_rowmap = nullptr);
int launch_gather_columns(const uint16_t *d_D, int64_t ld_d, const int32_t *d_uidx, const int32_t *d_ufirst, int64_t n, int64_t U,
                          uint16_t *d_F, int64_t ld_f, bool from_first_tile, hipStream_t stream, int table_world = 1,
                          int64_t table_rows_local = 0, int64_t row_begin = 0, int64_t row_end = -1);
size_t edges_to_csr_workspace_bytes(int64_t m, int64_t n);
int launch_edges_to_csr(const int32_t *d_i, const int32_t *d_j, const uint16_t *d_v, int64_t m, int64_t n, void *d_work, size_t work_bytes,
                        int64_t *d_ptr, int32_t *d_adj, uint16_t *d_codes, uint16_t *d_loops, hipStream_t stream);
int launch_symmetrize(void *d_mat, int64_t n, int64_t ld, int kind, hipStream_t stream);
int launch_acc_counts(uint32_t *d_acc, const uint16_t *d_cnt, int64_t count, bool first, hipStream_t stream);
int launch_counts32_to_f64(const uint32_t *d_acc, double *d_out, int64_t count, int n_hash, hipStream_t stream);
int launch_widen(const uint16_t *d_in, double *d_out, int64_t count, bool is_nw, int n_hash,
                 hipStream_t stream);

}
```

### dynaalign_amd/csrc/minhash_kernels.hip

```cpp
#include "da_common.hpp"

#include <algorithm>
#include <atomic>
#include <mutex>
#include <vector>
#include <type_traits>

namespace da {
namespace {

__device__ __forceinline__ uint32_t rotl32(uint32_t v, int r) {
  return __builtin_rotateleft32(v, r);
}
__device__ __forceinline__ uint32_t mm3_scramble(uint32_t w) {
  w *= 0xcc9e2d51u;
  w = rotl32(w, 15);
  w *= 0x1b873593u;
  return w;
}
__device__ __forceinline__ uint32_t mm3_mix(uint32_t h, uint32_t kk) {
  h ^= kk;
  return rotl32(h, 13) * 5u + 0xe6546b64u;
}
__device__ __forceinline__ uint32_t mm3_final(uint32_t h, uint32_t len) {
  h ^= len;
  h ^= h >> 16;
  h *= 0x85ebca6bu;
  h ^= h >> 13;
  h *= 0xc2b2ae35u;
  h ^= h >> 16;
  return h;
}

constexpr int K1_THREADS = 256;
constexpr int K1_CHUNK = 1024;

template <bool K_IS_4>
__global__ __launch_bounds__(K1_THREADS) void k_minhash_signatures(
    const uint8_t *__restrict__ residues, const int64_t *__restrict__ offsets, int k, int n_hash,
    const uint32_t *__restrict__ seeds, uint32_t *__restrict__ sig, int64_t ld_sig) {
  extern __shared__ uint32_t lds_k1[];
  const int64_t seq = blockIdx.x;
  const int64_t beg = offsets[seq];
  const int64_t len = offsets[seq + 1] - beg;
  const int64_t nwin = (len >= k) ? (len - k + 1) : 0;
  const int nblk = k >> 2, rem = k & 3;
  const int span = K1_CHUNK + k;
  uint32_t *KK = lds_k1;
  uint32_t *TT = lds_k1 + span;
  uint32_t *row = sig + seq * ld_sig;
  const uint8_t *s = residues + beg;

  if (nwin == 0)
    for (int h = threadIdx.x; h < n_hash; h += K1_THREADS) row[h] = 0xffffffffu;
  for (int64_t c0 = 0; c0 < nwin; c0 += K1_CHUNK) {
    const int cw = (int)((nwin - c0 < K1_CHUNK) ? (nwin - c0) : K1_CHUNK);
    const int need = cw + k - 1;
    __syncthreads();
    for (int q = threadIdx.x; q < need; q += K1_THREADS) {
      const int64_t g = c0 + q;
      uint32_t b0 = s[g];
      uint32_t b1 = (g + 1 < len) ? s[g + 1] : 0u;
      uint32_t b2 = (g + 2 < len) ? s[g + 2] : 0u;
      uint32_t b3 = (g + 3 < len) ? s[g + 3] : 0u;
      KK[q] = mm3_scramble(b0 | (b1 << 8) | (b2 << 16) | (b3 << 24));
      if (!K_IS_4) {
        uint32_t t = b0;
        if (rem >= 2) t |= b1 << 8;
        if (rem == 3) t |= b2 << 16;
        TT[q] = mm3_scramble(t);
      }
    }
    __syncthreads();
    for (int h = threadIdx.x; h < n_hash; h += K1_THREADS) {
      const uint32_t seed = seeds[h];
      uint32_t best = (c0 == 0) ? 0xffffffffu : row[h];
      if (K_IS_4) {
#pragma unroll 4
        for (int p = 0; p < cw; ++p) {
          uint32_t v = mm3_final(mm3_mix(seed, KK[p]), 4u);
          best = v < best ? v : best;
        }
      } else {
        for (int p = 0; p < cw; ++p) {
          uint32_t hh = seed;
          for (int b = 0; b < nblk; ++b) hh = mm3_mix(hh, KK[p + 4 * b]);
          if (rem) hh ^= TT[p + 4 * nblk];
          uint32_t v = mm3_final(hh, (uint32_t)k);
          best = v < best ? v : best;
        }
      }
      row[h] = best;
    }
  }
}

constexpr int K2_TILE = 128;
constexpr int K2_GROUP = 32;
constexpr int K2_BAND = 8;
constexpr int K2_THREADS = 256;


__device__ __forceinline__ uint32_t or_xor(uint32_t d, uint32_t a, uint32_t b) {
  return __builtin_amdgcn_bitop3_b32(d, a, b, 0xF6);
}

typedef double da_double2_t __attribute__((ext_vector_type(2)));
__device__ __forceinline__ void nt_store2(double *p, double a, double b) {
  da_double2_t v = {a, b};
  __builtin_nontemporal_store(v, reinterpret_cast<da_double2_t *>(p));
}

#ifndef K2_RING_DEPTH
#define K2_RING_DEPTH(PL) 3
#endif

struct TileId { int ti, tj; bool valid; };

__host__ __device__ __forceinline__ int div_small(int l, int h) {
#ifdef __HIP_DEVICE_COMPILE__
  int q = (int)__fdividef((float)l, (float)h);
#else
  int q = (int)((float)l / (float)h);
#endif
  while (q * h > l) --q;
  while ((q + 1) * h <= l) ++q;
  return q;
}
__host__ __device__ __forceinline__ TileId decode_tile(int64_t L, int TR, int T, bool symmetric) {
  TileId o{0, 0, true};
  const int S = K2_BAND;
  if (!symmetric) {
    const int64_t per_band = (int64_t)S * T;
    int B = (int)(L / per_band);
    int64_t l = L - (int64_t)B * per_band;
    int r0 = B * S;
    int h = (TR - r0 < S) ? (TR - r0) : S;
    if (h <= 0) { o.valid = false; return o; }
    o.tj = (int)(l / h);
    o.ti = r0 + (int)(l - (int64_t)o.tj * h);
    o.valid = o.tj < T;
    return o;
  }
  const int nfull = T / S;
  const int c0 = S * (S + 1) / 2 + (T - S) * S;
  auto prefix = [&](int B) { return (int64_t)B * c0 - (int64_t)(S * S / 2) * B * (B - 1); };
  int B;
  if (nfull > 0 && L < prefix(nfull)) {
    const float a = 0.5f * S * S, b = (float)c0 + a;
    const float disc = b * b - 4.0f * a * (float)L;
    B = (int)((b - sqrtf(disc > 0.0f ? disc : 0.0f)) / (2.0f * a));
    if (B < 0) B = 0;
    if (B > nfull - 1) B = nfull - 1;
    while (B > 0 && prefix(B) > L) --B;
    while (B + 1 <= nfull - 1 && prefix(B + 1) <= L) ++B;
  } else {
    B = nfull;
  }
  const int r0 = B * S;
  const int h = (T - r0 < S) ? (T - r0) : S;
  if (h <= 0) { o.valid = false; return o; }
  int l = (int)(L - prefix(B < nfull ? B : nfull));
  const int tri = h * (h + 1) / 2;
  if (l < tri) {
    int q = 0;
    while ((q + 1) * (q + 2) / 2 <= l) ++q;
    o.tj = r0 + q;
    o.ti = r0 + (l - q * (q + 1) / 2);
  } else {
    l -= tri;
    const int cq = div_small(l, h);
    o.tj = r0 + h + cq;
    o.ti = r0 + (l - cq * h);
  }
  o.valid = o.tj < T;
  return o;
}

__host__ __device__ inline int64_t count_tiles(int TR, int T, bool symmetric) {
  if (!symmetric) return (int64_t)TR * T;
  return (int64_t)T * (T + 1) / 2;
}

#ifdef DA_K2_TIMING
__device__ unsigned long long *g_k2_timing = nullptr;
#define K2_STAMP(i) do { if (g_k2_timing && threadIdx.x == 0) g_k2_timing[(size_t)blockIdx.x * 8 + (i)] = wall_clock64(); } while (0)
#define K2_STAMP_HW() do { if (g_k2_timing && threadIdx.x == 0) { \
    unsigned hw, xcc; asm volatile("s_getreg_b32 %0, hwreg(HW_REG_HW_ID)" : "=s"(hw)); \
    asm volatile("s_getreg_b32 %0, hwreg(HW_REG_XCC_ID)" : "=s"(xcc)); \
    g_k2_timing[(size_t)blockIdx.x * 8 + 4] = hw; g_k2_timing[(size_t)blockIdx.x * 8 + 5] = xcc; } } while (0)
#else
#define K2_STAMP(i) do { } while (0)
#define K2_STAMP_HW() do { } while (0)
#endif

typedef __attribute__((address_space(3))) void lds_void_t;
typedef __attribute__((address_space(1))) const void gbl_cvoid_t;

__host__ __device__ __forceinline__ bool k2_out_ok(const void *out, int64_t ld, bool wide) {
  return (ld & 1) == 0 && (reinterpret_cast<uintptr_t>(out) & (wide ? 15 : 3)) == 0;
}
__device__ __forceinline__ bool a12_takes(int ti, int tj, int64_t n, int64_t ld, const void *out, bool f64) {
  return ti != tj && (int64_t)(ti + 1) * K2_TILE <= n && (int64_t)(tj + 1) * K2_TILE <= n && k2_out_ok(out, ld, f64);
}
__device__ __forceinline__ bool s12_takes(int64_t I0, int64_t J0, int64_t n, int64_t row_end, int64_t ld, int64_t Jloc, const void *out) {
  return I0 != J0 &&
         I0 + K2_TILE <= (row_end < n ? row_end : n) && J0 + K2_TILE <= n && (Jloc & 1) == 0 && k2_out_ok(out, ld, false);
}

struct RectTile { int ti, tj; bool valid; int64_t I0, J0, Iloc, Jloc; };
__device__ __forceinline__ RectTile sym_tile(int64_t n, int64_t ld, const void *out, int64_t ntiles, int64_t per_xcd, bool wide) {
  RectTile t{0, 0, false, 0, 0, 0, 0};
  const int64_t bid = blockIdx.x;
  const int T = (int)((n + K2_TILE - 1) / K2_TILE);
  const int64_t L = (bid & 7) * per_xcd + (bid >> 3);
  if (L >= ntiles) return t;
  const TileId tl = decode_tile(L, T, T, true);
  t.ti = tl.ti;
  t.tj = tl.tj;
  t.valid = tl.valid && a12_takes(tl.ti, tl.tj, n, ld, out, wide);
  t.I0 = (int64_t)tl.ti * K2_TILE;
  t.J0 = (int64_t)tl.tj * K2_TILE;
  return t;
}
__device__ __forceinline__ RectTile rect_tile(int64_t bid, int64_t n, int64_t row_begin, int64_t row_end, int tile_stride, int upper_only, int TR,
                                              int fold_q, int64_t fold_w, int band, int64_t ld, const void *out) {
  RectTile t{0, 0, false, 0, 0, 0, 0};
  const int T = (int)((n + K2_TILE - 1) / K2_TILE);
  const uint32_t per_band = (uint32_t)band * (uint32_t)T;
  const uint32_t k = (uint32_t)(bid >> 3);
  const uint32_t kb = k / per_band;
  const int r0 = ((int)(bid & 7) + 8 * (int)kb) * band;
  const int l = (int)(k - kb * per_band);
  const int h = (TR - r0 < band) ? (TR - r0) : band;
  if (h <= 0) return t;
  t.tj = __builtin_amdgcn_readfirstlane(div_small(l, h));
  t.ti = __builtin_amdgcn_readfirstlane(r0 + (l - t.tj * h));
  if (t.tj >= T) return t;
  t.I0 = row_begin + (int64_t)t.ti * tile_stride * K2_TILE;
  t.J0 = (int64_t)t.tj * K2_TILE;
  t.Iloc = (int64_t)t.ti * K2_TILE - t.I0;
  t.Jloc = 0;
  if (fold_q > 0) {
    const int q = t.ti;
    const bool front = q <= fold_q - 1 - q;
    t.Iloc = (int64_t)(front ? q : fold_q - 1 - q) * K2_TILE - t.I0;
    t.Jloc = front ? -t.I0 : shard_back(fold_w, n);
  }
  if (t.I0 >= row_end || t.I0 >= n) return t;
  if (upper_only && t.J0 + K2_TILE <= t.I0) return t;
  t.valid = s12_takes(t.I0, t.J0, n, row_end, ld, t.Jloc, out);
  return t;
}

constexpr int PK_STAGE_LD = 144;
constexpr int PK_STAGE_BYTES = 32 * PK_STAGE_LD * 2;
__device__ __forceinline__ uint32_t pk_bit8(uint4 v) {
  return ((v.x >> 8) & 1u) | ((v.x >> 23) & 2u) | ((v.y >> 6) & 4u) | ((v.y >> 21) & 8u) | ((v.z >> 4) & 16u) | ((v.z >> 19) & 32u) |
         ((v.w >> 2) & 64u) | ((v.w >> 17) & 128u);
}
__device__ __forceinline__ void store_tile_pk(uint16_t *stage, const uint32_t (&mis)[8][4], uint32_t nn, int tid, int64_t I0, int64_t J0,
                                              bool mirror, int64_t n, uint8_t *tab, int64_t ld_lo) {
  const int wave = tid >> 6, lane = tid & 63;
  const int tx = ((wave & 1) << 3) + (lane & 7), ty = ((wave >> 1) << 3) + (lane >> 3);
  const int s = tid >> 3, ch = tid & 7;
  const bool dir = __builtin_amdgcn_readfirstlane(wave) < 2;
  const int64_t r0 = dir ? I0 : J0, c0 = dir ? J0 : I0, stride = pk_row_bytes(ld_lo);
  const uint64_t o = (uint64_t)(r0 * stride + c0);
  uint8_t *const base = tab + (((uint64_t)(uint32_t)__builtin_amdgcn_readfirstlane((uint32_t)(o >> 32)) << 32) |
                               (uint64_t)(uint32_t)__builtin_amdgcn_readfirstlane((uint32_t)o));
  const uint32_t hi_off = (uint32_t)(ld_lo - c0 + (c0 >> 3));
  const uint32_t lane_off = (uint32_t)(2 * (s & 15)) * (uint32_t)stride;
  const int rows_left = (int)min<int64_t>(n - r0, K2_TILE);
  const bool live = dir || mirror;
#pragma unroll
  for (int p = 0; p < 8; ++p) {
    __syncthreads();
    uint32_t *d = reinterpret_cast<uint32_t *>(stage + ty * PK_STAGE_LD + 2 * tx);
#pragma unroll
    for (int g = 0; g < 4; ++g) d[16 * g] = nn - mis[p][g];
    if (mirror) {
      uint32_t *m = reinterpret_cast<uint32_t *>(stage + (16 + tx) * PK_STAGE_LD + 2 * ty);
#pragma unroll
      for (int g = 0; g < 4; ++g) {
        const uint32_t lo = mis[2 * g][p >> 1], hi = mis[2 * g + 1][p >> 1];
        const uint32_t pk = (p & 1) ? ((lo >> 16) | (hi & 0xffff0000u)) : ((lo & 0xffffu) | (hi << 16));
        m[16 * g] = nn - pk;
      }
    }
    __syncthreads();
    const uint4 *src = reinterpret_cast<const uint4 *>(stage + s * PK_STAGE_LD + 16 * ch);
    const uint4 a = src[0], bb = src[1];
    uint4 lo;
    lo.x = __builtin_amdgcn_perm(a.y, a.x, 0x06040200u);
    lo.y = __builtin_amdgcn_perm(a.w, a.z, 0x06040200u);
    lo.z = __builtin_amdgcn_perm(bb.y, bb.x, 0x06040200u);
    lo.w = __builtin_amdgcn_perm(bb.w, bb.z, 0x06040200u);
    const uint32_t h = pk_bit8(a) | (pk_bit8(bb) << 8);
    auto pull = [&](uint32_t v, int d) { return (uint32_t)__builtin_amdgcn_ds_bpermute(((lane + d) & 63) << 2, (int)v); };
    const uint32_t x = h | (pull(h, 1) << 16);
    const uint4 hv = make_uint4(x, pull(x, 2), pull(x, 4), pull(x, 6));
    const int pr = 32 * (p >> 1) + (p & 1);
    if (live && pr + 2 * (s & 15) < rows_left) {
      uint8_t *rp = base + ((uint32_t)pr * (uint32_t)stride + lane_off);
      *reinterpret_cast<uint4 *>(rp + 16 * ch) = lo;
      if (ch == 0) *reinterpret_cast<uint4 *>(rp + hi_off) = hv;
    }
  }
  __syncthreads();
}
__device__ __forceinline__ void store_counts_f64(double *out, int64_t ld, const char *tb, const uint32_t (&mis)[8][4], uint32_t nn,
                                                   int64_t I0, int64_t J0, int tx, int ty) {
#pragma unroll
  for (int g = 0; g < 4; ++g) {
    double v0[8], v1[8];
#pragma unroll
    for (int c = 0; c < 4; ++c) {
      const uint32_t m0 = nn - mis[2 * g][c], m1 = nn - mis[2 * g + 1][c];
      v0[2 * c] = *reinterpret_cast<const double *>(tb + ((m0 << 3) & 0x7fff8u));
      v0[2 * c + 1] = *reinterpret_cast<const double *>(tb + ((m0 >> 13) & 0x7fff8u));
      v1[2 * c] = *reinterpret_cast<const double *>(tb + ((m1 << 3) & 0x7fff8u));
      v1[2 * c + 1] = *reinterpret_cast<const double *>(tb + ((m1 >> 13) & 0x7fff8u));
    }
    double *orow = out + (I0 + 32 * g + 2 * ty) * ld + (J0 + 2 * tx);
#pragma unroll
    for (int q = 0; q < 4; ++q) {
      nt_store2(orow + 32 * q, v0[2 * q], v0[2 * q + 1]);
      nt_store2(orow + ld + 32 * q, v1[2 * q], v1[2 * q + 1]);
    }
// ... 71 lines not shown
#define K2_PERSIST : K2_OUT : K2_IN, [nl] "s"(x.nl), [nh] "s"(x.nh), [fl] "s"(x.fl), [sp] "s"(x.sp), K2_VIN : K2_CLOBBER, "v122", "v123"
  if constexpr (B == K2_P12) {
    register uint32_t r122 asm("v122") = src_lo;
    register uint32_t r123 asm("v123") = src_hi;
    asm volatile(
#include K2_LOOP_INC
        : "+v"(r122), "+v"(r123), K2_OUT : K2_IN, K2_VIN : K2_CLOBBER);
  } else if constexpr (B == K2_P14) {
    asm volatile(
#include K2_LOOP_INC_14
        K2_UNIFORM);
  } else if constexpr (B == K2_P15) {
    asm volatile(
#include K2_LOOP_INC_15
        K2_UNIFORM);
  } else if constexpr (B == K2_P16) {
    asm volatile(
#include K2_LOOP_INC_16
        K2_UNIFORM);
  } else if constexpr (B == K2_P12P) {
    asm volatile(
#include K2_LOOP_INC_P
        K2_PERSIST);
  } else if constexpr (B == K2_P8P) {
    asm volatile(
#include "k2_loop_p8p.inc"
        K2_PERSIST);
  } else {
    static_assert(B == K2_P8, "a generated block");
    asm volatile(
#include "k2_loop_p8.inc"
        K2_PERSIST);
  }
#undef K2_PERSIST
#undef K2_UNIFORM
#undef K2_CLOBBER
#undef K2_VIN
#undef K2_IN
#undef K2_OUT
  asm volatile("" : "+v"(r124));
  const uint32_t cnt[32] = {c64, c65, c66, c67, c68, c69, c70, c71, c72, c73, c74, c75, c76, c77, c78, c79,
                            c80, c81, c82, c83, c84, c85, c86, c87, c88, c89, c90, c91, c92, c93, c94, c95};
#pragma unroll
  for (int r = 0; r < 8; ++r)
#pragma unroll
    for (int c = 0; c < 4; ++c) mis[r][c] = cnt[4 * r + c];
  return r124;
}

#ifndef K2_PRO_PRIO
#define K2_PRO_PRIO 0
#endif
__device__ __forceinline__ void k2_entry() {
  if (K2_PRO_PRIO) __builtin_amdgcn_s_setprio(K2_PRO_PRIO);
  K2_STAMP(0);
  K2_STAMP_HW();
}
constexpr int K2_A12_TABLE_MAX = 3 * 2 * K2_TILE * 3 * 16 / 8;
constexpr int K2_A16_TABLE_MAX = 2 * 2 * K2_TILE * 80 / 8;
template <K2Block B, bool SYM, bool F64, bool PK>
__device__ __forceinline__ void k2_one_tile(const uint32_t *planes, int64_t n, int n_hash, void *out_v, int64_t ld, const RectTile &t) {
  static_assert(B == K2_P12 || B == K2_P14 || B == K2_P15 || B == K2_P16, "a one-tile block");
  static_assert(SYM || (!F64 && !PK), "the rect geometry stores uint16 counts");
  constexpr int PL = 12, SEGS = 3, SLOT = B == K2_P12 ? 4 * PL : 80;
  __shared__ __attribute__((aligned(16))) uint4 lds_ab[(B == K2_P12 ? 3 : 2) * 2 * K2_TILE * SLOT / 16];
  static_assert(sizeof(lds_ab) / (sizeof(double)) == (B == K2_P12 ? K2_A12_TABLE_MAX : K2_A16_TABLE_MAX),
                "launch_mh_compare's table guard must match the ring size");
  if (!t.valid) return;
  if (!F64) K2_STAMP(6);
  const int64_t I0 = t.I0, J0 = t.J0;
  const int tid = threadIdx.x, wave = tid >> 6, lane = tid & 63;
  const int tx = ((wave & 1) << 3) + (lane & 7), ty = ((wave >> 1) << 3) + (lane >> 3);
  const uint32_t wave_u = __builtin_amdgcn_readfirstlane((uint32_t)wave);
  const uint32_t nstage = (uint32_t)((n_hash + K2_GROUP - 1) / K2_GROUP), stage_bytes = (uint32_t)(K2_TILE * SLOT);
  uint32_t src_lo = 0, src_hi = 0, sl, sh;
  if constexpr (B == K2_P12) {
    const PlaneGeom pg = plane_geom(n, n_hash, PL);
    const int u = wave * SEGS * 64 + lane, sl0 = u / SEGS, slot = sl0 & 127;
    const uint32_t *src = planes + (sl0 < 128 ? 0 : pg.copy_words) +
                          plane_unit_word(pg, (sl0 < 128 ? I0 : J0) + k2_row_of_slot(slot), 0, u - sl0 * SEGS);
    src_lo = (uint32_t)reinterpret_cast<uintptr_t>(src);
    src_hi = (uint32_t)(reinterpret_cast<uintptr_t>(src) >> 32);
    sl = __builtin_amdgcn_readfirstlane(src_lo);
    sh = __builtin_amdgcn_readfirstlane(src_hi);
  } else {
    const uint64_t blk = SYM ? (uint64_t)(wave_u >= 2 ? t.tj : t.ti) : (uint64_t)((wave_u >= 2 ? J0 : I0) / K2_TILE);
    const uint64_t src = reinterpret_cast<uint64_t>(planes) +
                         4u * (uint64_t)(pad16_base_words(n, n_hash) + (wave_u >= 2 ? pad16_copy_words(n, n_hash) : 0)) +
                         blk * nstage * stage_bytes + (wave_u & 1u) * (64u * SLOT);
    sl = __builtin_amdgcn_readfirstlane((uint32_t)src);
    sh = __builtin_amdgcn_readfirstlane((uint32_t)(src >> 32));
  }
  if (!F64) K2_STAMP(7);
  const uint32_t lds_base = __builtin_amdgcn_readfirstlane((uint32_t)(uintptr_t)(lds_void_t *)lds_ab);
  K2_STAMP(1);
  uint32_t mis[8][4];
  const uint32_t v124 = k2_block<B>(mis, {lds_base, nstage, stage_bytes, wave_u, sl, sh}, lds_base + (uint32_t)(ty * SLOT),
                                    lds_base + (uint32_t)((K2_TILE + tx) * SLOT), (uint32_t)tid * 4u, src_lo, src_hi);
  K2_STAMP(2);
  const uint32_t nn = (uint32_t)n_hash * 0x10001u;
  const int tid_e = (int)(v124 >> 2), wave_e = tid_e >> 6, lane_e = tid_e & 63;
  const int tx_e = ((wave_e & 1) << 3) + (lane_e & 7), ty_e = ((wave_e >> 1) << 3) + (lane_e >> 3);
  if constexpr (!SYM) {
    store_counts_u16(static_cast<uint16_t *>(out_v), ld, mis, nn, I0, J0, t.Iloc, t.Jloc, tx_e, ty_e, false);
  } else if constexpr (PK) {
    store_tile_pk(reinterpret_cast<uint16_t *>(lds_ab), mis, nn, tid_e, I0, J0, true, n, reinterpret_cast<uint8_t *>(out_v), ld);
  } else if constexpr (F64) {
    double *ratio = reinterpret_cast<double *>(lds_ab);
    __syncthreads();
    for (int c = tid_e; c <= n_hash; c += K2_THREADS) ratio[c] = (double)c / (double)n_hash;
    __syncthreads();
    K2_STAMP(6);
    K2_STAMP(7);
    store_counts_f64(static_cast<double *>(out_v), ld, reinterpret_cast<const char *>(ratio), mis, nn, I0, J0, tx_e, ty_e);
  } else {
    store_counts_u16(static_cast<uint16_t *>(out_v), ld, mis, nn, I0, J0, 0, 0, tx_e, ty_e, true);
  }
  K2_STAMP(3);
}
template <bool F64, bool PK = false>
__global__ __launch_bounds__(K2_THREADS, 4) void k_mh_compare_a12(const uint32_t *__restrict__ planes, int64_t n, int n_hash,
                                                                  void *__restrict__ out_v, int64_t ld, int64_t ntiles,
                                                                  int64_t per_xcd) {
  k2_entry();
  k2_one_tile<K2_P12, true, F64, PK>(planes, n, n_hash, out_v, ld, sym_tile(n, ld, out_v, ntiles, per_xcd, F64 || PK));
}
__global__ __launch_bounds__(K2_THREADS, 4) void k_mh_compare_s12(const uint32_t *__restrict__ planes, int64_t n, int n_hash, int64_t row_begin,
                                                                  int64_t row_end, int tile_stride, int upper_only, int TR, uint16_t *__restrict__ out,
                                                                  int64_t ld, int fold_q, int64_t fold_w, int band) {
  k2_entry();
  k2_one_tile<K2_P12, false, false, false>(planes, n, n_hash, out, ld,
                                           rect_tile(blockIdx.x, n, row_begin, row_end, tile_stride, upper_only, TR, fold_q, fold_w, band, ld, out));
}
template <bool F64, int CODE_BITS = 16>
__global__ __launch_bounds__(K2_THREADS, 4) void k_mh_compare_a16(const uint32_t *__restrict__ planes, int64_t n, int n_hash,
                                                                  void *__restrict__ out_v, int64_t ld, int64_t ntiles,
                                                                  int64_t per_xcd) {
  k2_entry();
  k2_one_tile<K2Block(CODE_BITS), true, F64, false>(planes, n, n_hash, out_v, ld, sym_tile(n, ld, out_v, ntiles, per_xcd, F64));
}
template <int CODE_BITS>
__global__ __launch_bounds__(K2_THREADS, 4) void k_mh_compare_s16(const uint32_t *__restrict__ planes, int64_t n, int n_hash, int64_t row_begin,
                                                                  int64_t row_end, int tile_stride, int upper_only, int TR, uint16_t *__restrict__ out,
                                                                  int64_t ld, int fold_q, int64_t fold_w, int band) {
  k2_entry();
  k2_one_tile<K2Block(CODE_BITS), false, false, false>(planes, n, n_hash, out, ld,
                                                       rect_tile(blockIdx.x, n, row_begin, row_end, tile_stride, upper_only, TR, fold_q, fold_w, band, ld, out));
}

constexpr int K2_P12_TABLE = 512, K2_P8_TABLE = 2048;
template <bool F64, int PL = 12, bool ONE = false, bool PK = false>
__global__ __launch_bounds__(K2_THREADS, 4) void k_mh_compare_p12(const uint32_t *__restrict__ planes, int64_t n, int n_hash,
                                                                  void *__restrict__ out_v, int64_t ld, int64_t ntiles,
                                                                  int64_t per_xcd, int wg_per_xcd, int64_t tile_begin) {
  static_assert(PL == 12 || PL == 8, "generated blocks exist for 12 and 8 planes");
  static_assert(!PK || (!F64 && PL == 12 && !ONE), "the packed table is written by the 12-plane band kernel");
  constexpr int SEGS = PL / 4, STAGE_UNITS = 2 * K2_TILE * SEGS;
  __shared__ __attribute__((aligned(16))) uint4 lds_ab[3 * STAGE_UNITS];
  __shared__ double ratio_tab[F64 ? (PL == 8 ? K2_P8_TABLE : K2_P12_TABLE) : 1];
  const int T = (int)((n + K2_TILE - 1) / K2_TILE);
  const int xcd = blockIdx.x & 7, slot = blockIdx.x >> 3;
  const int lim = (int)((tile_begin + (int64_t)(xcd + 1) * per_xcd < ntiles) ? tile_begin + (int64_t)(xcd + 1) * per_xcd : ntiles);
  const int tid = threadIdx.x, wave = tid >> 6, lane = tid & 63;
  if (F64) {
    for (int c = tid; c <= n_hash; c += K2_THREADS) ratio_tab[c] = (double)c / (double)n_hash;
    __syncthreads();
  }
  const PlaneGeom pg = plane_geom(n, n_hash, PL);
  const uint32_t wave_u = __builtin_amdgcn_readfirstlane((uint32_t)wave);
  const uint64_t block_bytes = (uint64_t)pg.nst * (128u * PL * 4u);
  const uint64_t wave_base = reinterpret_cast<uint64_t>(planes) + (wave_u >= 2 ? (uint64_t)pg.copy_words * 4u : 0u) + (wave_u & 1u) * (uint32_t)(SEGS * 1024);
  auto source_of = [&](const TileId &t) -> uint64_t { return wave_base + (uint64_t)(wave_u >= 2 ? t.tj : t.ti) * block_bytes; };
  auto next_taken = [&](int from, TileId &t) -> int {
    for (int L = from; L < lim; L += wg_per_xcd) {
      int To = T;
      asm volatile("" : "+s"(To));
      t = decode_tile(L, To, To, true);
      t.ti = __builtin_amdgcn_readfirstlane(t.ti);
      t.tj = __builtin_amdgcn_readfirstlane(t.tj);
      if (t.valid && a12_takes(t.ti, t.tj, n, ld, out_v, F64 || PK)) return L;
    }
    return lim;
  };
  const int tx0 = ((wave & 1) << 3) + (lane & 7), ty0 = ((wave >> 1) << 3) + (lane >> 3);
  const uint32_t lds_base = __builtin_amdgcn_readfirstlane((uint32_t)(uintptr_t)(lds_void_t *)lds_ab);
  const uint32_t nstage = (uint32_t)((n_hash + K2_GROUP - 1) / K2_GROUP), stage_bytes = 128u * PL * 4u;
  const uint32_t nn = (uint32_t)n_hash * 0x10001u;
  const uint32_t a_off = lds_base + (uint32_t)(ty0 * SEGS * 16);
  const uint32_t b_off = lds_base + (uint32_t)((K2_TILE * SEGS + tx0 * SEGS) * 16);
  uint32_t v124 = (uint32_t)tid * 4u;

  TileId cur, nxt;
  int L = next_taken((int)(tile_begin + (int64_t)xcd * per_xcd) + slot, cur);
  uint32_t flags = 1u, phase = 0u;
#ifdef DA_K2_TIMING
  int it_stamp = 0;
#define K2P_STAMP(j) do { if (g_k2_timing && threadIdx.x == 0 && it_stamp < 64) \
    g_k2_timing[((size_t)blockIdx.x * 64 + it_stamp) * 4 + (j)] = wall_clock64(); } while (0)
#else
#define K2P_STAMP(j) do { } while (0)
#endif
  while (L < lim) {
    K2P_STAMP(0);
    const int Ln = next_taken(L + wg_per_xcd, nxt);
    if (Ln < lim) flags |= 2u;
    const uint64_t src = source_of(cur), src_n = source_of(nxt);
    const uint32_t sl = __builtin_amdgcn_readfirstlane((uint32_t)src), sh = __builtin_amdgcn_readfirstlane((uint32_t)(src >> 32));
    const uint32_t nl = __builtin_amdgcn_readfirstlane((uint32_t)src_n), nh = __builtin_amdgcn_readfirstlane((uint32_t)(src_n >> 32));
    const uint32_t fl = __builtin_amdgcn_readfirstlane(flags), sp = __builtin_amdgcn_readfirstlane(phase * (uint32_t)(STAGE_UNITS * 16));
    uint32_t mis[8][4];
    K2P_STAMP(1);
    v124 = k2_block<PL == 12 ? K2_P12P : ONE ? K2_P8 : K2_P8P>(mis, {lds_base, nstage, stage_bytes, wave_u, sl, sh}, a_off, b_off, v124, 0, 0,
                                                              {nl, nh, fl, sp});
    K2P_STAMP(2);
    const int tid_e = (int)(v124 >> 2), wave_e = tid_e >> 6, lane_e = tid_e & 63;
    const int tx = ((wave_e & 1) << 3) + (lane_e & 7), ty = ((wave_e >> 1) << 3) + (lane_e >> 3);
    const int64_t I0 = (int64_t)cur.ti * K2_TILE, J0 = (int64_t)cur.tj * K2_TILE;
    if constexpr (PK) {
      static_assert(STAGE_UNITS * 16 >= PK_STAGE_BYTES, "the packed epilogue stages in one ring slot");
      uint16_t *stage = reinterpret_cast<uint16_t *>(lds_ab + ((phase + nstage + 2u) % 3u) * STAGE_UNITS);
      store_tile_pk(stage, mis, nn, tid_e, I0, J0, true, n, reinterpret_cast<uint8_t *>(out_v), ld);
    } else if constexpr (F64) {
      store_counts_f64(reinterpret_cast<double *>(out_v), ld, reinterpret_cast<const char *>(ratio_tab), mis, nn, I0, J0, tx, ty);
    } else {
      store_counts_u16(reinterpret_cast<uint16_t *>(out_v), ld, mis, nn, I0, J0, 0, 0, tx, ty, true);
    }
    K2P_STAMP(3);
#ifdef DA_K2_TIMING
    ++it_stamp;
#endif
    cur = nxt;
    L = Ln;
    flags = 0u;
    phase = (phase + nstage) % 3u;
  }
#undef K2P_STAMP
}

template <bool SYM, bool F64, int PL, bool PK = false>
__global__ __launch_bounds__(K2_THREADS, 3) void k_mh_compare(
    const uint32_t *__restrict__ planes, int64_t n, int n_hash, int64_t row_begin,
    int64_t row_end, int tile_stride, int upper_only, int TR, void *__restrict__ out_v, int64_t ld,
    int64_t ntiles, int64_t per_xcd, int fold_q, int64_t fold_w, int band, int only_edge) {
  constexpr int SP = (PL == 32) ? 16 : PL;
  constexpr int SEGS = SP / 4;
  constexpr int SPG = PL / SP;
  constexpr int STAGE_UNITS = 2 * K2_TILE * SEGS;
  constexpr int K2_NSTAGE = K2_RING_DEPTH(PL);
  __shared__ __attribute__((aligned(16))) uint4 lds_ab[K2_NSTAGE * STAGE_UNITS];

  K2_STAMP(0);
  K2_STAMP_HW();
  const int64_t bid = blockIdx.x;
  const int T = (int)((n + K2_TILE - 1) / K2_TILE);
  TileId tid2;
  if (SYM && only_edge) {
    tid2.valid = bid < 2 * (int64_t)T - 1;
    tid2.ti = bid < T ? (int)bid : (int)(bid - T);
    tid2.tj = bid < T ? (int)bid : T - 1;
  } else if (SYM) {
    const int64_t L = (bid & 7) * per_xcd + (bid >> 3);
    if (L >= ntiles) return;
    tid2 = decode_tile(L, TR, T, true);
  } else {
    const uint32_t per_band = (uint32_t)band * (uint32_t)T;
    const uint32_t k = (uint32_t)(bid >> 3);
    const uint32_t kb = k / per_band;
    const int r0 = ((int)(bid & 7) + 8 * (int)kb) * band;
    const int l = (int)(k - kb * per_band);
    const int h = (TR - r0 < band) ? (TR - r0) : band;
    if (h <= 0) return;
    tid2.tj = div_small(l, h);
    tid2.ti = r0 + (l - tid2.tj * h);
    tid2.valid = tid2.tj < T;
  }
  if (!tid2.valid) return;
  const int64_t I0 = row_begin + (int64_t)tid2.ti * tile_stride * K2_TILE;
  const int64_t J0 = (int64_t)tid2.tj * K2_TILE;
  int64_t Iloc = (int64_t)tid2.ti * K2_TILE - I0;
  int64_t Jloc = 0;
  if (!SYM && fold_q > 0) {
    const int q = tid2.ti;
    const bool front = q <= fold_q - 1 - q;
    Iloc = (int64_t)(front ? q : fold_q - 1 - q) * K2_TILE - I0;
    Jloc = front ? -I0 : shard_back(fold_w, n);
  }
  if (I0 >= row_end || I0 >= n) return;
  if (!SYM && upper_only && J0 + K2_TILE <= I0) return;
  if (SYM && only_edge && a12_takes(tid2.ti, tid2.tj, n, ld, out_v, F64 || PK)) return;
  if (!SYM && !F64 && only_edge && s12_takes(I0, J0, n, row_end, ld, Jloc, out_v)) return;

  const int tid = threadIdx.x;
  const int wave = tid >> 6, lane = tid & 63;
  const int tx = ((wave & 1) << 3) + (lane & 7);
  const int ty = ((wave >> 1) << 3) + (lane >> 3);

  const PlaneGeom pg = plane_geom(n, n_hash, PL);
  const uint32_t *src[SEGS];
#pragma unroll
  for (int q = 0; q < SEGS; ++q) {
    const int u = (wave * SEGS + q) * 64 + lane;
    const int s = u / SEGS;
    const int sl = s & 127;
    const int seg = (u - s * SEGS) ^ (SEGS == 4 ? ((sl >> 2) & 3) : 0);
    int64_t g = ((s < 128) ? I0 : J0) + k2_row_of_slot(sl);
    if (g > n - 1) g = n - 1;
    src[q] = planes + ((s < 128) ? 0 : pg.copy_words) + plane_unit_word(pg, g, 0, seg);
  }
  const uint32_t lds_wave_base =
      __builtin_amdgcn_readfirstlane((uint32_t)(uintptr_t)(lds_void_t *)(lds_ab + wave * SEGS * 64));
  auto issue = [&](int stage) {
    const uint32_t base = lds_wave_base + (uint32_t)(stage % K2_NSTAGE) * (uint32_t)(STAGE_UNITS * sizeof(uint4));
#pragma unroll
    for (int q = 0; q < SEGS; ++q) {
      const uint32_t *g = src[q] + stage * (128 * SP);
      uint32_t keep_m0;
      asm volatile("s_mov_b32 %0, m0\n\ts_mov_b32 m0, %2\n\ts_nop 0\n\tglobal_load_lds_dwordx4 %1, off\n\ts_mov_b32 m0, %0"
                   : "=&s"(keep_m0) : "v"(g), "s"(base + (uint32_t)(q * 64 * sizeof(uint4))) : "memory");
    }
  };
  auto wait_stage = [&](int younger) {
    const int outstanding = younger * SEGS;
    if (outstanding >= 8) asm volatile("s_waitcnt vmcnt(8)" ::: "memory");
    else if (outstanding == 6) asm volatile("s_waitcnt vmcnt(6)" ::: "memory");
    else if (outstanding == 4) asm volatile("s_waitcnt vmcnt(4)" ::: "memory");
    else if (outstanding == 3) asm volatile("s_waitcnt vmcnt(3)" ::: "memory");
    else if (outstanding == 2) asm volatile("s_waitcnt vmcnt(2)" ::: "memory");
    else asm volatile("s_waitcnt vmcnt(0)" ::: "memory");
  };

// ... 211 lines not shown
      if (SYM && tid2.ti != tid2.tj) {
#pragma unroll
        for (int c = 0; c < 8; ++c) {
          uint16_t *orow = out + (J0 + 32 * (c >> 1) + 2 * tx + (c & 1)) * ld + (I0 + 2 * ty);
#pragma unroll
          for (int g = 0; g < 4; ++g) *reinterpret_cast<uint32_t *>(orow + 32 * g) = nn - mis_col(mis, g, c);
        }
      }
      K2_STAMP(3);
      return;
    }
#pragma unroll
    for (int r = 0; r < 8; ++r) {
      const int64_t gi = I0 + 32 * (r >> 1) + 2 * ty + (r & 1);
      if (gi >= row_end || gi >= n) continue;
      uint16_t *orow = out + (gi + Iloc) * ld + Jloc;
#pragma unroll
      for (int g = 0; g < 4; ++g) {
        const int64_t gj = J0 + 32 * g + 2 * tx;
        if (gj < n) orow[gj] = (uint16_t)matches(r, 2 * g);
        if (gj + 1 < n) orow[gj + 1] = (uint16_t)matches(r, 2 * g + 1);
      }
    }
    if (SYM && tid2.ti != tid2.tj) {
#pragma unroll
      for (int c = 0; c < 8; ++c) {
        const int64_t gj = J0 + 32 * (c >> 1) + 2 * tx + (c & 1);
        if (gj >= n) continue;
        uint16_t *orow = out + gj * ld;
#pragma unroll
        for (int g = 0; g < 4; ++g) {
          const int64_t gi = I0 + 32 * g + 2 * ty;
          if (gi < n) orow[gi] = (uint16_t)matches(2 * g, c);
          if (gi + 1 < n) orow[gi + 1] = (uint16_t)matches(2 * g + 1, c);
        }
      }
    }
  }
  K2_STAMP(3);
}

template <typename T>
__global__ __launch_bounds__(256) void k_symmetrize(T *__restrict__ m, int64_t n, int64_t ld) {
  __shared__ T tile[32][33];
  const int64_t bi = blockIdx.y, bj = blockIdx.x;
  if (bj < bi) return;
  const int tx = threadIdx.x & 31, ty = threadIdx.x >> 5;
  for (int r = ty; r < 32; r += 8) {
    const int64_t i = bi * 32 + r, j = bj * 32 + tx;
    if (i < n && j < n) tile[r][tx] = m[i * ld + j];
  }
  __syncthreads();
  for (int r = ty; r < 32; r += 8) {
    const int64_t j = bj * 32 + r, i = bi * 32 + tx;
    if (i < n && j < n && j > i) m[j * ld + i] = tile[tx][r];
  }
}

__global__ __launch_bounds__(256) void k_widen(const uint16_t *__restrict__ in, double *__restrict__ out,
                                               int64_t count, int is_nw, int n_hash) {
  const int64_t stride = (int64_t)gridDim.x * blockDim.x;
  for (int64_t i = (int64_t)blockIdx.x * blockDim.x + threadIdx.x; i < count; i += stride) {
    const uint32_t v = in[i];
    out[i] = is_nw ? (double)(v >> 8) / (double)(v & 255u) : (double)v / (double)n_hash;
  }
}

__global__ __launch_bounds__(256) void k_acc_counts(uint32_t *__restrict__ acc, const uint16_t *__restrict__ cnt, int64_t count, int first) {
  const int64_t stride = (int64_t)gridDim.x * blockDim.x;
  for (int64_t i = (int64_t)blockIdx.x * blockDim.x + threadIdx.x; i < count; i += stride)
    acc[i] = (first ? 0u : acc[i]) + cnt[i];
}
__global__ __launch_bounds__(256) void k_counts32_to_f64(const uint32_t *__restrict__ acc, double *__restrict__ out, int64_t count, int n_hash) {
  const int64_t stride = (int64_t)gridDim.x * blockDim.x;
  for (int64_t i = (int64_t)blockIdx.x * blockDim.x + threadIdx.x; i < count; i += stride)
    out[i] = (double)acc[i] / (double)n_hash;
}

}

int launch_acc_counts(uint32_t *d_acc, const uint16_t *d_cnt, int64_t count, bool first, hipStream_t stream) {
  if (count <= 0) return DA_OK;
  hipLaunchKernelGGL(k_acc_counts, dim3(256 * 16), dim3(256), 0, stream, d_acc, d_cnt, count, first ? 1 : 0);
  DA_HIP_TRY(hipGetLastError());
  return DA_OK;
}
int launch_counts32_to_f64(const uint32_t *d_acc, double *d_out, int64_t count, int n_hash, hipStream_t stream) {
  if (count <= 0) return DA_OK;
  hipLaunchKernelGGL(k_counts32_to_f64, dim3(256 * 16), dim3(256), 0, stream, d_acc, d_out, count, n_hash);
  DA_HIP_TRY(hipGetLastError());
  return DA_OK;
}

#ifdef DA_K2_TIMING
extern "C" int da_debug_set_k2_timing(unsigned long long *d_buf) {
  return (int)hipMemcpyToSymbol(HIP_SYMBOL(g_k2_timing), &d_buf, sizeof(d_buf));
}
#endif

int launch_minhash_signatures(const uint8_t *d_res, const int64_t *d_off, int64_t n, int k,
                              int n_hash, const uint32_t *d_seeds, uint32_t *d_sig,
                              int64_t ld_sig, hipStream_t stream) {
  if (n <= 0) return DA_OK;
  if (n > 0x7fffffffLL) return fail(DA_ERR_UNSUPPORTED, "more than 2^31-1 sequences");
  const size_t lds = 2 * (size_t)(K1_CHUNK + k) * sizeof(uint32_t);
  if (lds > 64 * 1024) return fail(DA_ERR_UNSUPPORTED, "k = %d is larger than the signature kernel supports (k <= 7168)", k);
  dim3 grid((unsigned)n), block(K1_THREADS);
  if (k == 4)
    hipLaunchKernelGGL(k_minhash_signatures<true>, grid, block, lds, stream, d_res, d_off, k, n_hash, d_seeds, d_sig, ld_sig);
  else
    hipLaunchKernelGGL(k_minhash_signatures<false>, grid, block, lds, stream, d_res, d_off, k, n_hash, d_seeds, d_sig, ld_sig);
  DA_HIP_TRY(hipGetLastError());
  return DA_OK;
}

template <auto V, auto... MORE, typename X, typename F>
static void dispatch(X x, F &&f) {
  if constexpr (sizeof...(MORE) == 0) f(std::integral_constant<decltype(V), V>{});
  else if (x == V) f(std::integral_constant<decltype(V), V>{});
  else dispatch<MORE...>(x, f);
}

int launch_mh_compare(const uint32_t *d_planes, int64_t n, int n_hash,
                      int64_t row_begin, int64_t row_end, bool symmetric, int kind,
                      void *d_out, int64_t ld, hipStream_t stream, int plane_bits, int tile_stride, bool upper_only,
                      int fold_q, int64_t fold_w) {
  if (row_end <= row_begin) return DA_OK;
  if (plane_bits != 8 && plane_bits != 12 && plane_bits != 14 && plane_bits != 15 && plane_bits != 16 && plane_bits != 32)
    return fail(DA_ERR_BAD_ARG, "plane_bits must be 8, 12, 14, 15, 16 or 32 (got %d)", plane_bits);
  const int code_bits = plane_bits;
  if (plane_bits == 14 || plane_bits == 15) plane_bits = 16;
  const int T = (int)ceil_div(n, K2_TILE);
  const int TR = (int)ceil_div(ceil_div(row_end - row_begin, K2_TILE), tile_stride);
  const int64_t ntiles = count_tiles(TR, T, symmetric);
  const int64_t per_xcd = ceil_div(ntiles, 8);
  int band = K2_BAND;
  while (band > 1 && ceil_div(TR, band) < 48) band >>= 1;
  const int64_t nblocks = symmetric ? per_xcd * 8 : 8 * ceil_div(ceil_div(TR, band), 8) * (int64_t)band * T;
  if (nblocks > 0x7fffffffLL) return fail(DA_ERR_UNSUPPORTED, "pair space too large for one launch");
  dim3 grid((unsigned)nblocks), block(K2_THREADS);
  const bool f64 = kind == DA_OUT_F64, asm_ok = !config().k2_no_asm && k2_out_ok(d_out, ld, f64);
  const bool a12 = symmetric && plane_bits == 12 && asm_ok && (!f64 || (int64_t)n_hash + 1 <= K2_A12_TABLE_MAX);
  const bool a16 = symmetric && plane_bits == 16 && asm_ok && (!f64 || (int64_t)n_hash + 1 <= K2_A16_TABLE_MAX);
  const bool a8 = symmetric && plane_bits == 8 && asm_ok && n_hash > K2_GROUP && (!f64 || n_hash < K2_P8_TABLE) && per_xcd < 0x7fffffffLL;
  const bool s12 = !symmetric && plane_bits == 12 && kind == DA_OUT_COMPACT && asm_ok && (row_begin % K2_TILE) == 0;
  const bool s16 = !symmetric && plane_bits == 16 && kind == DA_OUT_COMPACT && asm_ok && (row_begin % K2_TILE) == 0;
  if (a8)
    dispatch<false, true>(f64, [&](auto F64) {
      if (config().k2_persist) {
        int wg_per_xcd = 4 * 32;
        if (config().k2_wg_per_cu > 0) wg_per_xcd = config().k2_wg_per_cu * 32;
        if ((int64_t)wg_per_xcd > per_xcd) wg_per_xcd = (int)(per_xcd > 0 ? per_xcd : 1);
        hipLaunchKernelGGL((k_mh_compare_p12<decltype(F64)::value, 8, false>), dim3((unsigned)(8 * wg_per_xcd)), block, 0, stream, d_planes, n, n_hash,
                           d_out, ld, ntiles, per_xcd, wg_per_xcd, (int64_t)0);
      } else {
        hipLaunchKernelGGL((k_mh_compare_p12<decltype(F64)::value, 8, true>), grid, block, 0, stream, d_planes, n, n_hash, d_out, ld, ntiles, per_xcd,
                           (int)per_xcd, (int64_t)0);
      }
    });
  if (a16)
    dispatch<false, true>(f64, [&](auto F64) {
      dispatch<14, 15, 16>(code_bits, [&](auto B) {
        hipLaunchKernelGGL((k_mh_compare_a16<decltype(F64)::value, decltype(B)::value>), grid, block, 0, stream, d_planes, n, n_hash, d_out, ld, ntiles,
                           per_xcd);
      });
    });
  const bool p12 = a12 && n_hash > K2_GROUP && (!f64 || n_hash < K2_P12_TABLE) && config().k2_persist;
  if (p12) {
    static std::atomic<int> occ_cache[2], cus_cache;
    const int ki = kind == DA_OUT_F64 ? 0 : 1;
    if (!occ_cache[ki].load()) {
      int occ = 0;
      if (ki == 0) DA_HIP_TRY(hipOccupancyMaxActiveBlocksPerMultiprocessor(&occ, k_mh_compare_p12<true>, K2_THREADS, 0));
      else DA_HIP_TRY(hipOccupancyMaxActiveBlocksPerMultiprocessor(&occ, k_mh_compare_p12<false>, K2_THREADS, 0));
      int dev = 0;
      hipDeviceProp_t prop;
      DA_HIP_TRY(hipGetDevice(&dev));
      DA_HIP_TRY(hipGetDeviceProperties(&prop, dev));
      if (config().k2_wg_per_cu > 0) occ = config().k2_wg_per_cu;
      cus_cache.store(prop.multiProcessorCount > 0 ? prop.multiProcessorCount : 256);
      occ_cache[ki].store(occ > 0 ? occ : 1);
      if (config().trace)
        fprintf(stderr, "[dynaalign] k_mh_compare_p12<%s>: %d resident workgroups per CU, %d CUs\n", ki == 0 ? "f64" : "u16", occ_cache[ki].load(), cus_cache.load());
    }
    int wg_per_xcd = occ_cache[ki].load() * ((cus_cache.load() + 7) / 8);
    if ((int64_t)wg_per_xcd > per_xcd) wg_per_xcd = (int)(per_xcd > 0 ? per_xcd : 1);
    const dim3 pgrid((unsigned)(8 * wg_per_xcd));
    if (kind == DA_OUT_F64)
      hipLaunchKernelGGL(k_mh_compare_p12<true>, pgrid, block, 0, stream, d_planes, n, n_hash, d_out, ld, ntiles, per_xcd, wg_per_xcd, (int64_t)0);
    else
      hipLaunchKernelGGL(k_mh_compare_p12<false>, pgrid, block, 0, stream, d_planes, n, n_hash, d_out, ld, ntiles, per_xcd, wg_per_xcd, (int64_t)0);
  } else if (a12) {
    if (f64)
      hipLaunchKernelGGL(k_mh_compare_a12<true>, grid, block, 0, stream, d_planes, n, n_hash, d_out, ld, ntiles, per_xcd);
    else
      hipLaunchKernelGGL(k_mh_compare_a12<false>, grid, block, 0, stream, d_planes, n, n_hash, d_out, ld, ntiles, per_xcd);
  }
  if (s12)
    hipLaunchKernelGGL(k_mh_compare_s12, grid, block, 0, stream, d_planes, n, n_hash, row_begin, row_end, tile_stride, upper_only ? 1 : 0, TR,
                       static_cast<uint16_t *>(d_out), ld, fold_q, fold_w, band);
  if (s16)
    dispatch<14, 15, 16>(code_bits, [&](auto B) {
      hipLaunchKernelGGL((k_mh_compare_s16<decltype(B)::value>), grid, block, 0, stream, d_planes, n, n_hash, row_begin, row_end, tile_stride,
                         upper_only ? 1 : 0, TR, static_cast<uint16_t *>(d_out), ld, fold_q, fold_w, band);
    });
  const int only_edge = (a12 || a16 || a8 || s12 || s16) ? 1 : 0;
  if (a12 || a16 || a8) grid = dim3((unsigned)(2 * (int64_t)T - 1));
  dispatch<false, true>(symmetric, [&](auto SYM) {
    dispatch<false, true>(f64, [&](auto F64) {
      dispatch<8, 12, 16, 32>(plane_bits, [&](auto PL) {
        hipLaunchKernelGGL((k_mh_compare<decltype(SYM)::value, decltype(F64)::value, decltype(PL)::value>), grid, block, 0, stream, d_planes, n,
                           n_hash, row_begin, row_end, tile_stride, upper_only ? 1 : 0, TR, d_out, ld, ntiles, per_xcd, fold_q, fold_w, band, only_edge);
      });
    });
  });
  DA_HIP_TRY(hipGetLastError());
  return DA_OK;
}

int64_t mh_sym_band_prefix(int64_t n, int64_t band) {
  const int64_t T = ceil_div(n, K2_TILE), S = K2_BAND, nfull = T / S;
  if (band <= 0) return 0;
  if (band > nfull) return T * (T + 1) / 2;
  const int64_t c0 = S * (S + 1) / 2 + (T - S) * S;
  return band * c0 - (S * S / 2) * band * (band - 1);
}
int64_t mh_sym_bands(int64_t n) { return ceil_div(ceil_div(n, K2_TILE), K2_BAND); }
extern "C" int64_t da_debug_sym_band_prefix(int64_t n, int64_t band) { return mh_sym_band_prefix(n, band); }
extern "C" int da_debug_decode_sym_tile(int64_t L, int T, int *ti, int *tj) {
  const TileId t = decode_tile(L, T, T, true);
  if (ti) *ti = t.ti;
  if (tj) *tj = t.tj;
  return t.valid ? 1 : 0;
}
bool mh_compare_bands_ok(int64_t n, int n_hash, int plane_bits, const void *d_out, int64_t ld) {
  const int64_t T = ceil_div(n, K2_TILE);
  return (plane_bits == 12 || plane_bits == 8) && n_hash > K2_GROUP && n_hash <= 65535 && !config().k2_no_asm &&
         k2_out_ok(d_out, ld, false) && T * (T + 1) / 2 < 0x7fffffffLL;
}
int launch_mh_compare_bands_u16(const uint32_t *d_planes, int64_t n, int n_hash, uint16_t *d_out, int64_t ld, int64_t band_begin,
                                int64_t band_end, int wg_per_cu, hipStream_t stream, int plane_bits, bool pk) {
  if (!mh_compare_bands_ok(n, n_hash, plane_bits, d_out, ld) ||
      (pk && (!mh_compare_pk_ok(n, n_hash, plane_bits) || !k2_out_ok(d_out, ld, true))))
    return fail(DA_ERR_UNSUPPORTED, "banded compare: shape not covered");
  const int64_t t0 = mh_sym_band_prefix(n, band_begin), t1 = mh_sym_band_prefix(n, band_end);
  if (t1 <= t0) return DA_OK;
  static std::atomic<int> cus_cache;
  if (!cus_cache.load()) {
    int dev = 0;
    hipDeviceProp_t prop;
    DA_HIP_TRY(hipGetDevice(&dev));
    DA_HIP_TRY(hipGetDeviceProperties(&prop, dev));
    cus_cache.store(prop.multiProcessorCount > 0 ? prop.multiProcessorCount : 256);
  }
  const int64_t per_xcd = ceil_div(t1 - t0, 8);
  int wg_per_xcd = std::max(1, std::min(wg_per_cu, 4)) * ((cus_cache.load() + 7) / 8);
  if ((int64_t)wg_per_xcd > per_xcd) wg_per_xcd = (int)per_xcd;
  if (plane_bits == 8)
    hipLaunchKernelGGL((k_mh_compare_p12<false, 8, false>), dim3((unsigned)(8 * wg_per_xcd)), dim3(K2_THREADS), 0, stream, d_planes, n, n_hash,
                       static_cast<void *>(d_out), ld, t1, per_xcd, wg_per_xcd, t0);
  else if (pk)
    hipLaunchKernelGGL((k_mh_compare_p12<false, 12, false, true>), dim3((unsigned)(8 * wg_per_xcd)), dim3(K2_THREADS), 0, stream, d_planes, n, n_hash,
                       static_cast<void *>(d_out), ld, t1, per_xcd, wg_per_xcd, t0);
  else
    hipLaunchKernelGGL(k_mh_compare_p12<false>, dim3((unsigned)(8 * wg_per_xcd)), dim3(K2_THREADS), 0, stream, d_planes, n, n_hash,
                       static_cast<void *>(d_out), ld, t1, per_xcd, wg_per_xcd, t0);
  DA_HIP_TRY(hipGetLastError());
  return DA_OK;
}
int launch_mh_compare_edges_u16(const uint32_t *d_planes, int64_t n, int n_hash, uint16_t *d_out, int64_t ld, hipStream_t stream, int plane_bits,
                                bool pk) {
  const int T = (int)ceil_div(n, K2_TILE);
  const int64_t ntiles = count_tiles(T, T, true);
  if (pk && (!mh_compare_pk_ok(n, n_hash, plane_bits) || !k2_out_ok(d_out, ld, true)))
    return fail(DA_ERR_UNSUPPORTED, "packed count table: shape not covered");
  if (pk)
    hipLaunchKernelGGL((k_mh_compare<true, false, 12, true>), dim3((unsigned)(2 * (int64_t)T - 1)), dim3(K2_THREADS), 0, stream, d_planes, n, n_hash,
                       (int64_t)0, n, 1, 0, T, static_cast<void *>(d_out), ld, ntiles, ceil_div(ntiles, 8), 0, (int64_t)0, K2_BAND, 1);
  else if (plane_bits == 8)
    hipLaunchKernelGGL((k_mh_compare<true, false, 8>), dim3((unsigned)(2 * (int64_t)T - 1)), dim3(K2_THREADS), 0, stream, d_planes, n, n_hash,
                       (int64_t)0, n, 1, 0, T, static_cast<void *>(d_out), ld, ntiles, ceil_div(ntiles, 8), 0, (int64_t)0, K2_BAND, 1);
  else
  hipLaunchKernelGGL((k_mh_compare<true, false, 12>), dim3((unsigned)(2 * (int64_t)T - 1)), dim3(K2_THREADS), 0, stream, d_planes, n, n_hash,
                     (int64_t)0, n, 1, 0, T, static_cast<void *>(d_out), ld, ntiles, ceil_div(ntiles, 8), 0, (int64_t)0, K2_BAND, 1);
  DA_HIP_TRY(hipGetLastError());
  return DA_OK;
}

bool mh_compare_pk_ok(int64_t n, int n_hash, int plane_bits) {
  return plane_bits == 12 && n >= 1 && n <= 65536 && n_hash >= 1 && expand_stream_packed(n_hash) && !config().k2_no_asm;
}
int launch_mh_compare_pk(const uint32_t *d_planes, int64_t n, int n_hash, uint8_t *d_tab, hipStream_t stream) {
  if (!mh_compare_pk_ok(n, n_hash, 12) || !k2_out_ok(d_tab, pk_lo_bytes(n), true)) return fail(DA_ERR_UNSUPPORTED, "packed count table: shape not covered");
  const int T = (int)ceil_div(n, K2_TILE);
  const int64_t ntiles = count_tiles(T, T, true), per_xcd = ceil_div(ntiles, 8);
  hipLaunchKernelGGL((k_mh_compare_a12<false, true>), dim3((unsigned)(per_xcd * 8)), dim3(K2_THREADS), 0, stream, d_planes, n, n_hash,
                     static_cast<void *>(d_tab), pk_lo_bytes(n), ntiles, per_xcd);
  DA_HIP_TRY(hipGetLastError());
  return launch_mh_compare_edges_u16(d_planes, n, n_hash, reinterpret_cast<uint16_t *>(d_tab), pk_lo_bytes(n), stream, 12, true);
}

template <int FT, typename WIDEN>
__device__ __forceinline__ void store_tile_f64(const uint16_t (&t)[FT][FT + 2], WIDEN widen, double *__restrict__ out, int64_t ld, int n,
                                                int i0, int j0) {
  const int tx = threadIdx.x & (FT - 1), ty = threadIdx.x / FT;
  const bool fast = i0 != j0 && i0 + FT <= n && j0 + FT <= n && (ld & 1) == 0 && (reinterpret_cast<uintptr_t>(out) & 15) == 0 &&
                    ((i0 | j0) & 1) == 0;
  if (fast) {
    constexpr int PAIRS = FT / 2, RG = 256 / PAIRS;
    const int k2 = 2 * (threadIdx.x % PAIRS), rg = threadIdx.x / PAIRS;
#pragma unroll 8
    for (int r = rg; r < FT; r += RG)
      nt_store2(out + (int64_t)(i0 + r) * ld + j0 + k2, widen(t[r][k2]), widen(t[r][k2 + 1]));
#pragma unroll 8
    for (int r = rg; r < FT; r += RG)
      nt_store2(out + (int64_t)(j0 + r) * ld + i0 + k2, widen(t[k2][r]), widen(t[k2 + 1][r]));
    return;
  }
  constexpr int RS = 256 / FT;
  const int j = j0 + tx;
  double *o = out + (int64_t)i0 * ld + j;
  for (int r = ty; r < FT; r += RS) {
    const int i = i0 + r;
    if (i < n && j < n && j >= i) o[(int64_t)r * ld] = widen(t[r][tx]);
  }
  const int im = i0 + tx;
  double *om = out + (int64_t)j0 * ld + im;
  for (int r = ty; r < FT; r += RS) {
    const int jm = j0 + r;
    if (im < n && jm < n && jm > im) om[(int64_t)r * ld] = widen(t[tx][r]);
  }
}

struct TableRows { int world; int64_t rows_local; };
__device__ __forceinline__ int64_t table_row(int r, const TableRows &tr) {
  if (tr.world <= 1) return r;
  const int t = r >> 7;
  return (int64_t)(t % tr.world) * tr.rows_local + (int64_t)(t / tr.world) * 128 + (r & 127);
}

__device__ __forceinline__ TileId leftover_tile64(unsigned b, int n, int TB) {
  const int T128 = (n + 127) >> 7, t = (int)(b >> 2), sub = (int)(b & 3);
  const int ti128 = t < T128 ? t : t - T128, tj128 = t < T128 ? t : T128 - 1;
  TileId o;
  o.ti = 2 * ti128 + (sub >> 1); o.tj = 2 * tj128 + (sub & 1);
  o.valid = o.ti <= o.tj && o.ti < TB && o.tj < TB;
  return o;
}
__device__ __forceinline__ TileId decode_tile_xcd(unsigned b, int64_t per_xcd, int64_t ntiles, int TB) {
  const int64_t L = (int64_t)(b & 7) * per_xcd + (b >> 3);
  if (L >= ntiles) { TileId o; o.ti = o.tj = 0; o.valid = false; return o; }
  return decode_tile(L, TB, TB, true);
}
static unsigned leftover_blocks64(int64_t n) {
  const int T128 = (int)ceil_div(n, 128);
  return (unsigned)(4 * (T128 + ((n & 127) ? T128 - 1 : 0)));
}
constexpr int ER_STRIDE = 272;
template <typename WIDEN>
__device__ __forceinline__ void er_store_tile(const unsigned char *er_lds, WIDEN widen, double *__restrict__ out, int64_t ld, int64_t I0,
                                              int64_t J0, int tx, int ty) {
#pragma unroll
  for (int g = 0; g < 4; ++g) {
    double v0[8], v1[8];
#pragma unroll
    for (int q = 0; q < 4; ++q) {
      const uint32_t w0 = *reinterpret_cast<const uint32_t *>(er_lds + (32 * g + 2 * ty) * ER_STRIDE + (32 * q + 2 * tx) * 2);
      const uint32_t w1 = *reinterpret_cast<const uint32_t *>(er_lds + (32 * g + 2 * ty + 1) * ER_STRIDE + (32 * q + 2 * tx) * 2);
      v0[2 * q] = widen(w0 & 0xffffu); v0[2 * q + 1] = widen(w0 >> 16);
      v1[2 * q] = widen(w1 & 0xffffu); v1[2 * q + 1] = widen(w1 >> 16);
    }
    double *orow = out + (I0 + 32 * g + 2 * ty) * ld + (J0 + 2 * tx);
#pragma unroll
    for (int q = 0; q < 4; ++q) {
      nt_store2(orow + 32 * q, v0[2 * q], v0[2 * q + 1]);
      nt_store2(orow + ld + 32 * q, v1[2 * q], v1[2 * q + 1]);
    }
#pragma unroll
    for (int c = 0; c < 8; ++c)
      nt_store2(out + (J0 + 32 * (c >> 1) + 2 * tx + (c & 1)) * ld + (I0 + 32 * g + 2 * ty), v0[c], v1[c]);
  }
}
__device__ __forceinline__ bool expand_fast_takes(int ti128, int tj128, int n, int64_t ld, const void *out) {
  return ti128 != tj128 && (ti128 + 1) * 128 <= n && (tj128 + 1) * 128 <= n && (ld & 1) == 0 &&
         (reinterpret_cast<uintptr_t>(out) & 15) == 0;
}

template <bool IS_NW, bool PACKED>
__global__ __launch_bounds__(256, 4) void k_finalize_rows(const void *__restrict__ G_v, int64_t ld_g_or_block_bytes, ShardGeom geom, int nhi,
                                                          int n_hash, int tab_entries, double *__restrict__ out, int64_t ld, int T128,
                                                          int64_t ntiles, int64_t per_xcd) {
  extern __shared__ __attribute__((aligned(16))) unsigned char er_lds[];
  double *tab = reinterpret_cast<double *>(er_lds + 128 * ER_STRIDE);
  const int n = (int)geom.n;
  const int64_t L = (int64_t)(blockIdx.x & 7) * per_xcd + (blockIdx.x >> 3);
  if (L >= ntiles) return;
  const TileId tt = decode_tile(L, T128, T128, true);
  if (!tt.valid || !expand_fast_takes(tt.ti, tt.tj, n, ld, out)) return;
  const int tid = threadIdx.x, wave = tid >> 6, lane = tid & 63;
  const int tx = ((wave & 1) << 3) + (lane & 7), ty = ((wave >> 1) << 3) + (lane >> 3);
  const int64_t I0 = (int64_t)tt.ti * 128, J0 = (int64_t)tt.tj * 128;
  const int tr = tt.ti, q_loc = tr / geom.world, owner = tr - q_loc * geom.world;
  const bool front = q_loc <= geom.Q - 1 - q_loc;
  const int64_t lrow0 = (int64_t)(front ? q_loc : geom.Q - 1 - q_loc) * 128;
  const int64_t col0 = (front ? -(int64_t)tr * 128 : shard_back(geom.W, geom.n)) + J0;
  const int unit = tid & 15, row0 = tid >> 4;
  uint4 st[8];
  if (!PACKED) {
    const uint16_t *G = static_cast<const uint16_t *>(G_v);
    const int64_t ld_g = ld_g_or_block_bytes;
    const uint16_t *src = G + ((int64_t)owner * geom.rows + lrow0 + row0) * ld_g + col0 + 8 * unit;
#pragma unroll
    for (int q = 0; q < 8; ++q) st[q] = *reinterpret_cast<const uint4 *>(src + (int64_t)(16 * q) * ld_g);
  } else {
    const uint8_t *blk = static_cast<const uint8_t *>(G_v) + (int64_t)owner * ld_g_or_block_bytes;
    const int64_t W = geom.W, groups = W >> 3, rows = geom.rows, col = col0 + 8 * unit;
#pragma unroll
    for (int q = 0; q < 8; ++q) {
      const int64_t row = lrow0 + row0 + 16 * q;
// ... 66 lines not shown
    const uint32_t ln = v & 255u;
    if (ln == 0) return __longlong_as_double(0xFFF8000000000000ULL);
    return (double)(v >> 8) / (double)ln;
  };
  const int tile = geom.tile;
  const int tr = i0 / tile;
  const int q = tr / geom.world, owner = tr - q * geom.world;
  const bool front = q <= geom.Q - 1 - q;
  const int64_t lrow0 = (int64_t)owner * geom.rows + (int64_t)(front ? q : geom.Q - 1 - q) * tile + (i0 - tr * tile);
  const int64_t coff = front ? -(int64_t)tr * tile : shard_back(geom.W, geom.n);
  const uint16_t *src = G + lrow0 * ld_g + coff + j0 + tx;
  const int j = j0 + tx;
  for (int r = ty; r < FT; r += 4) {
    const int i = i0 + r;
    if (i < n && j < n && j >= i) t[r][tx] = src[(int64_t)r * ld_g];
  }
  __syncthreads();
  if (U16) store_tile_u16<64>(t, static_cast<uint16_t *>(out_v), ld, n, i0, j0);
  else store_tile_f64<64>(t, widen, out, ld, n, i0, j0);
}

template <bool F64, bool IS_NW, int FT>
__global__ __launch_bounds__(256) void k_expand_unique(const uint16_t *__restrict__ D, int64_t ld_d, const int32_t *__restrict__ uidx,
                                                       int n, int n_hash, void *__restrict__ out_v, int64_t ld, int TB,
                                                       int64_t ntiles, int64_t per_xcd, int skip_fast, TableRows trows) {
  __shared__ uint16_t t[FT][FT + 2];
  __shared__ int32_t ur[FT], uc[FT];
  const TileId tt = skip_fast ? leftover_tile64(blockIdx.x, n, TB) : decode_tile_xcd(blockIdx.x, per_xcd, ntiles, TB);
  if (!tt.valid) return;
  const int i0 = tt.ti * FT, j0 = tt.tj * FT;
  constexpr int RS = 256 / FT;
  const int tx = threadIdx.x & (FT - 1), ty = threadIdx.x / FT;
  for (int q = threadIdx.x; q < 2 * FT; q += 256) {
    if (q < FT) ur[q] = (i0 + q < n) ? uidx[i0 + q] : 0;
    else uc[q - FT] = (j0 + q - FT < n) ? uidx[j0 + q - FT] : 0;
  }
  __syncthreads();
  auto widen = [&](uint32_t v) -> double {
    if (!IS_NW) return (double)v / (double)n_hash;
    const uint32_t ln = v & 255u;
    if (ln == 0) return __longlong_as_double(0xFFF8000000000000ULL);
    return (double)(v >> 8) / (double)ln;
  };
  const int j = j0 + tx;
  const int32_t cj = uc[tx];
  for (int r = ty; r < FT; r += RS) {
    const int i = i0 + r;
    if (i < n && j < n && j >= i) t[r][tx] = D[table_row(ur[r], trows) * ld_d + cj];
  }
  __syncthreads();
  if (F64) {
    store_tile_f64<FT>(t, widen, reinterpret_cast<double *>(out_v), ld, n, i0, j0);
  } else {
    uint16_t *out = reinterpret_cast<uint16_t *>(out_v);
    uint16_t *o = out + (int64_t)i0 * ld + j;
    for (int r = ty; r < FT; r += RS) {
      const int i = i0 + r;
      if (i < n && j < n && j >= i) o[(int64_t)r * ld] = t[r][tx];
    }
    const int im = i0 + tx;
    uint16_t *om = out + (int64_t)j0 * ld + im;
    for (int r = ty; r < FT; r += RS) {
      const int jm = j0 + r;
      if (im < n && jm < n && jm > im) om[(int64_t)r * ld] = t[tx][r];
    }
  }
}

constexpr int GC_THREADS = 1024;
__global__ __launch_bounds__(GC_THREADS) void k_gather_columns(const uint16_t *__restrict__ D, int64_t ld_d, const int32_t *__restrict__ uidx,
                                                               const int32_t *__restrict__ ufirst, int n, int U, uint16_t *__restrict__ F,
                                                               int64_t ld_f, TableRows trows, int from_first_tile, int row_begin) {
  extern __shared__ __attribute__((aligned(16))) uint16_t gc_row[];
  const int units = (int)(ld_d >> 3);
  uint4 pre[8];
#define GC_FETCH(row)                                                                                   \
  {                                                                                                     \
    const uint4 *src_ = reinterpret_cast<const uint4 *>(D + table_row((row), trows) * ld_d);            \
    _Pragma("unroll") for (int q = 0; q < 8; ++q) {                                                     \
      const int u = (int)threadIdx.x + q * GC_THREADS;                                                  \
      pre[q] = u < units ? src_[u] : make_uint4(0, 0, 0, 0);                                            \
    }                                                                                                   \
  }
  int r = row_begin + (int)blockIdx.x;
  if (r < U) GC_FETCH(r)
  const int2 *u2 = reinterpret_cast<const int2 *>(uidx);
  const int j2_end = n >> 1;
  for (; r < U; r += gridDim.x) {
    __syncthreads();
    uint4 *dst = reinterpret_cast<uint4 *>(gc_row);
#pragma unroll
    for (int q = 0; q < 8; ++q) {
      const int u = (int)threadIdx.x + q * GC_THREADS;
      if (u < units) dst[u] = pre[q];
    }
    __syncthreads();
    if (r + (int)gridDim.x < U) GC_FETCH(r + (int)gridDim.x)
    const int j_begin = ((ufirst[r] >> 7) + (from_first_tile ? 0 : 1)) << 7;
    uint32_t *frow = reinterpret_cast<uint32_t *>(F + (int64_t)r * ld_f);
    for (int j2 = (j_begin >> 1) + threadIdx.x; j2 < j2_end; j2 += GC_THREADS) {
      const int2 c = u2[j2];
      __builtin_nontemporal_store((uint32_t)gc_row[c.x] | ((uint32_t)gc_row[c.y] << 16), frow + j2);
    }
    if ((n & 1) && threadIdx.x == 0 && n - 1 >= j_begin) F[(int64_t)r * ld_f + n - 1] = gc_row[uidx[n - 1]];
  }
#undef GC_FETCH
}

template <bool IS_NW>
__global__ __launch_bounds__(256, 4) void k_expand_rows(const uint16_t *__restrict__ F, int64_t ld_f, const int32_t *__restrict__ uidx,
                                                        int n, int n_hash, int tab_stride, int tab_entries, double *__restrict__ out,
                                                        int64_t ld, int T128, int64_t ntiles, int64_t per_xcd, int64_t tile_begin) {
  extern __shared__ __attribute__((aligned(16))) unsigned char er_lds[];
  double *tab = reinterpret_cast<double *>(er_lds + 128 * ER_STRIDE);
  const int64_t L = tile_begin + (int64_t)(blockIdx.x & 7) * per_xcd + (blockIdx.x >> 3);
  if (L >= ntiles || L >= tile_begin + (int64_t)((blockIdx.x & 7) + 1) * per_xcd) return;
  const TileId tt = decode_tile(L, T128, T128, true);
  if (!tt.valid || !expand_fast_takes(tt.ti, tt.tj, n, ld, out)) return;
  const int tid = threadIdx.x, wave = tid >> 6, lane = tid & 63;
  const int tx = ((wave & 1) << 3) + (lane & 7), ty = ((wave >> 1) << 3) + (lane >> 3);
  const int64_t I0 = (int64_t)tt.ti * 128, J0 = (int64_t)tt.tj * 128;
  uint4 st[8];
#pragma unroll
  for (int q = 0; q < 8; ++q) {
    const int row = (tid >> 4) + 16 * q;
    st[q] = *(reinterpret_cast<const uint4 *>(F + (int64_t)uidx[I0 + row] * ld_f + J0) + (tid & 15));
  }
  if (IS_NW) {
    for (int e = tid; e < tab_entries; e += 256) {
      const int mt = e / tab_stride, ln = e - mt * tab_stride;
      tab[e] = ln == 0 ? __longlong_as_double(0xFFF8000000000000ULL) : (double)mt / (double)ln;
    }
  } else {
    for (int e = tid; e < tab_entries; e += 256) tab[e] = (double)e / (double)n_hash;
  }
#pragma unroll
  for (int q = 0; q < 8; ++q)
    *reinterpret_cast<uint4 *>(er_lds + ((tid >> 4) + 16 * q) * ER_STRIDE + (tid & 15) * 16) = st[q];
  __syncthreads();
  auto widen = [&](uint32_t x) -> double {
    if (IS_NW) return tab[(x >> 8) * (uint32_t)tab_stride + (x & 255u)];
    return tab[x];
  };
  er_store_tile(er_lds, widen, out, ld, I0, J0, tx, ty);
}

constexpr int ES_THREADS = 1024, ES_COPIES = 4, ES_TICKETS = 128;
__global__ __launch_bounds__(256) void k_es_count(const int32_t *__restrict__ uidx, int n, uint32_t *__restrict__ cnt) {
  const int i = blockIdx.x * 256 + threadIdx.x;
  if (i < n) atomicAdd(&cnt[uidx[i]], 1u);
}
__global__ __launch_bounds__(1024) void k_es_scan(const uint32_t *__restrict__ cnt, int U, uint32_t *__restrict__ cstart, uint32_t *__restrict__ istart) {
  __shared__ uint64_t wsum[16];
  __shared__ uint64_t carry_s;
  const int tid = threadIdx.x, lane = tid & 63, wave = tid >> 6;
  if (tid == 0) carry_s = 0;
  __syncthreads();
  for (int base = 0; base < U; base += 1024) {
    const int u = base + tid;
    const uint32_t c = u < U ? cnt[u] : 0u;
    const uint64_t v = (uint64_t)c | ((uint64_t)((c + ES_COPIES - 1) / ES_COPIES) << 32);
    uint64_t x = v;
#pragma unroll
    for (int d = 1; d < 64; d <<= 1) {
      const uint64_t y = __shfl_up(x, d, 64);
      if (lane >= d) x += y;
    }
    if (lane == 63) wsum[wave] = x;
    __syncthreads();
    uint64_t woff = 0;
    for (int w = 0; w < wave; ++w) woff += wsum[w];
    const uint64_t carry = carry_s;
    if (u < U) {
      const uint64_t e = carry + woff + x - v;
      cstart[u] = (uint32_t)e;
      istart[u] = (uint32_t)(e >> 32);
    }
    __syncthreads();
    if (tid == 1023) carry_s = carry + woff + x;
    __syncthreads();
  }
  if (tid == 0) { cstart[U] = (uint32_t)carry_s; istart[U] = (uint32_t)(carry_s >> 32); }
}
__global__ __launch_bounds__(256) void k_es_fill(const int32_t *__restrict__ uidx, int n, int U, const uint32_t *__restrict__ cstart,
                                                 const uint32_t *__restrict__ istart, uint32_t *__restrict__ cursor, int32_t *__restrict__ cpos,
                                                 int2 *__restrict__ items) {
  const int i = blockIdx.x * 256 + threadIdx.x;
  if (i < n) {
    const int u = uidx[i];
    cpos[cstart[u] + atomicAdd(&cursor[u], 1u)] = i;
  }
  if (i < U) {
    const uint32_t first = istart[i], cnt = istart[i + 1] - first;
    for (uint32_t q = 0; q < cnt; ++q) items[first + q] = make_int2(i, (int)(q * ES_COPIES));
  }
}
__device__ __forceinline__ double es_ratio(uint32_t c, double dn, double rcp) {
  const double dc = (double)c, q0 = __dmul_rn(dc, rcp), e = __fma_rn(-q0, dn, dc);
  return __fma_rn(e, rcp, q0);
}
__global__ __launch_bounds__(256) void k_es_ratio_check(int n_hash, double *__restrict__ out) {
  const int c = blockIdx.x * 256 + threadIdx.x;
  const double dn = (double)n_hash, rcp = 1.0 / dn;
  if (c <= n_hash) out[c] = es_ratio((uint32_t)c, dn, rcp);
}
enum { ES_U16 = 0, ES_U16_PK = 1, ES_PK = 2 };
template <int FMT, int NQ>
__global__ __launch_bounds__(ES_THREADS, 8)
void k_expand_stream(const uint16_t *__restrict__ D, int64_t ld_d, const int32_t *__restrict__ uidx,
                                                              const uint32_t *__restrict__ cstart, const int32_t *__restrict__ cpos,
                                                              const int2 *__restrict__ items, const uint32_t *__restrict__ istart, int row_begin,
                                                              int row_end, int n, int n_hash, double *__restrict__ out, int64_t ld,
                                                              uint32_t *__restrict__ ticket) {
  extern __shared__ __attribute__((aligned(16))) unsigned char es_lds[];
#ifdef ES_PRIO
  __builtin_amdgcn_s_setprio(ES_PRIO);
#endif
  constexpr bool PACKED = FMT != ES_U16;
  uint16_t *row = reinterpret_cast<uint16_t *>(es_lds);
  unsigned char *row_lo = es_lds, *row_hi = row_lo + ld_d;
  const int tid = threadIdx.x;
  const double dn = (double)n_hash, rcp = 1.0 / dn;
  auto count_of = [&](int c) -> uint32_t {
    if (!PACKED) return row[c];
    return (uint32_t)row_lo[c] | ((((uint32_t)row_hi[c >> 3] >> (c & 7)) & 1u) << 8);
  };
  const int n_items = (int)istart[row_end];
  const int64_t row_bytes = FMT == ES_PK ? pk_row_bytes(ld_d) : 2 * ld_d;
  const int units = (int)(row_bytes >> 4);
  uint4 pre[NQ];
#define ES_FETCH(r_)                                                                                    \
  {                                                                                                     \
    const uint4 *src_ = reinterpret_cast<const uint4 *>(reinterpret_cast<const unsigned char *>(D) + (int64_t)(r_) * row_bytes); \
    _Pragma("unroll") for (int q = 0; q < NQ; ++q) {                                                    \
      const int u = tid + q * ES_THREADS;                                                               \
      pre[q] = u < units ? src_[u] : make_uint4(0, 0, 0, 0);                                            \
    }                                                                                                   \
  }
  __shared__ int s_next;
  const int base = (int)istart[row_begin];
  int k = base + (int)blockIdx.x;
  int2 it = k < n_items ? items[k] : make_int2(0, 0);
  if (k < n_items) ES_FETCH(it.x)
  const int2 *u2 = reinterpret_cast<const int2 *>(uidx);
  const int j2_end = n >> 1;
  while (k < n_items) {
    __syncthreads();
    if (tid == 0) s_next = base + (int)gridDim.x + (int)atomicAdd(ticket, 1u);
    uint4 *dst = reinterpret_cast<uint4 *>(row);
#pragma unroll
    for (int q = 0; q < NQ; ++q) {
      const int u = tid + q * ES_THREADS;
      if (u >= units) continue;
      if (FMT != ES_U16_PK) { dst[u] = pre[q]; continue; }
      const uint4 v = pre[q];
      uint2 lo;
      lo.x = __builtin_amdgcn_perm(v.y, v.x, 0x06040200u);
      lo.y = __builtin_amdgcn_perm(v.w, v.z, 0x06040200u);
      *reinterpret_cast<uint2 *>(row_lo + 8 * u) = lo;
      row_hi[u] = (unsigned char)(((v.x >> 8) & 1u) | ((v.x >> 23) & 2u) | ((v.y >> 6) & 4u) | ((v.y >> 21) & 8u) | ((v.z >> 4) & 16u) |
                                  ((v.z >> 19) & 32u) | ((v.w >> 2) & 64u) | ((v.w >> 17) & 128u));
    }
    __syncthreads();
    const uint32_t c0 = cstart[it.x] + (uint32_t)it.y, c_end = cstart[it.x + 1];
    const int ncop = (int)min((uint32_t)ES_COPIES, c_end - c0);
    double *orow[ES_COPIES];
#pragma unroll
    for (int q = 0; q < ES_COPIES; ++q) orow[q] = out + (int64_t)cpos[c0 + (uint32_t)min(q, ncop - 1)] * ld;
    const int kn = __builtin_amdgcn_readfirstlane(s_next);
    int2 itn = make_int2(0, 0);
    if (kn < n_items) { itn = items[kn]; ES_FETCH(itn.x) }
#pragma unroll 4
    for (int j2 = tid; j2 < j2_end; j2 += ES_THREADS) {
      const int2 c = u2[j2];
      const double v0 = es_ratio(count_of(c.x), dn, rcp), v1 = es_ratio(count_of(c.y), dn, rcp);
      nt_store2(orow[0] + 2 * j2, v0, v1);
      if (ncop > 1) nt_store2(orow[1] + 2 * j2, v0, v1);
      if (ncop > 2) nt_store2(orow[2] + 2 * j2, v0, v1);
      if (ncop > 3) nt_store2(orow[3] + 2 * j2, v0, v1);
    }
    if ((n & 1) && tid == 0) {
      const double v = es_ratio(count_of(uidx[n - 1]), dn, rcp);
      for (int q = 0; q < ncop; ++q) orow[q][n - 1] = v;
    }
    it = itn;
    k = kn;
  }
#undef ES_FETCH
}

bool expand_stream_ok(int64_t n, int64_t U, int n_hash, const void *d_out, int64_t ld) {
  return n >= 2 && n <= 0x7fffffffLL && U >= 1 && U <= 65536 && n_hash >= 1 && n_hash <= 2047 && (ld & 1) == 0 &&
         (reinterpret_cast<uintptr_t>(d_out) & 15) == 0;
}
extern "C" int da_debug_ratio_check(int n_hash, double *d_out, void *stream) {
  if (n_hash < 1 || !d_out) return fail(DA_ERR_BAD_ARG, "ratio check: bad arguments");
  hipLaunchKernelGGL(k_es_ratio_check, dim3((unsigned)(n_hash / 256 + 1)), dim3(256), 0, static_cast<hipStream_t>(stream), n_hash, d_out);
  DA_HIP_TRY(hipGetLastError());
  return DA_OK;
}
bool expand_stream_packed(int n_hash) { return n_hash <= 511; }
size_t expand_stream_scratch_bytes(int64_t n, int64_t U) {
  return ((size_t)(4 * U + 8 + ES_TICKETS) * 4 + (size_t)n * 4 + (size_t)(U + n / ES_COPIES + 2) * 8 + 1024);
}
struct EsLists { uint32_t *cnt, *cursor, *ticket, *cstart, *istart; int32_t *cpos; int2 *items; };
static EsLists es_layout(void *d_scratch, int64_t n, int64_t U) {
  uint32_t *w = static_cast<uint32_t *>(d_scratch);
  EsLists L;
  L.cnt = w; L.cursor = w + U; L.ticket = w + 2 * U; L.cstart = L.ticket + ES_TICKETS; L.istart = L.cstart + (U + 1);
  L.cpos = reinterpret_cast<int32_t *>(L.istart + (U + 1));
  L.items = reinterpret_cast<int2 *>((reinterpret_cast<uintptr_t>(L.cpos + n) + 15) & ~(uintptr_t)15);
  return L;
}
int launch_expand_stream_lists(const int32_t *d_uidx, int64_t n, int64_t U, void *d_scratch, hipStream_t stream) {
  const EsLists L = es_layout(d_scratch, n, U);
  DA_HIP_TRY(hipMemsetAsync(L.cnt, 0, ((size_t)U * 2 + ES_TICKETS) * 4, stream));
  const unsigned nb = (unsigned)ceil_div(std::max(n, U), 256);
  hipLaunchKernelGGL(k_es_count, dim3((unsigned)ceil_div(n, 256)), dim3(256), 0, stream, d_uidx, (int)n, L.cnt);
  hipLaunchKernelGGL(k_es_scan, dim3(1), dim3(1024), 0, stream, L.cnt, (int)U, L.cstart, L.istart);
  hipLaunchKernelGGL(k_es_fill, dim3(nb), dim3(256), 0, stream, d_uidx, (int)n, (int)U, L.cstart, L.istart, L.cursor, L.cpos, L.items);
  DA_HIP_TRY(hipGetLastError());
  return DA_OK;
}
int launch_expand_stream_rows(const uint16_t *d_D, int64_t ld_d, const int32_t *d_uidx, int64_t n, int64_t U, int n_hash, double *d_out, int64_t ld,
                              void *d_scratch, int64_t row_begin, int64_t row_end, hipStream_t stream, int launch_no, bool pk) {
  if (!expand_stream_ok(n, U, n_hash, d_out, ld) || (ld_d & (pk ? 127 : 7)) || ld_d > 65536 || (reinterpret_cast<uintptr_t>(d_D) & 15) || launch_no < 0 ||
      launch_no >= ES_TICKETS || (pk && !expand_stream_packed(n_hash)))
    return fail(DA_ERR_UNSUPPORTED, "row expansion: shape not covered");
  if (row_end > U) row_end = U;
  if (row_begin >= row_end) return DA_OK;
  const EsLists L = es_layout(d_scratch, n, U);
  static std::atomic<int> es_cus;
  static std::atomic<uint64_t> es_attr_done;
  int dev = 0;
  DA_HIP_TRY(hipGetDevice(&dev));
  if (!((es_attr_done.load() >> (dev & 63)) & 1u)) {
    hipDeviceProp_t prop;
    DA_HIP_TRY(hipGetDeviceProperties(&prop, dev));
#define DA_ES_ATTR(P, Q) DA_HIP_TRY(hipFuncSetAttribute(reinterpret_cast<const void *>(k_expand_stream<P, Q>), hipFuncAttributeMaxDynamicSharedMemorySize, 65536 * 2))
    DA_ES_ATTR(ES_U16, 2); DA_ES_ATTR(ES_U16, 4); DA_ES_ATTR(ES_U16, 6); DA_ES_ATTR(ES_U16, 8);
    DA_ES_ATTR(ES_U16_PK, 2); DA_ES_ATTR(ES_U16_PK, 4); DA_ES_ATTR(ES_U16_PK, 6); DA_ES_ATTR(ES_U16_PK, 8);
    DA_ES_ATTR(ES_PK, 2); DA_ES_ATTR(ES_PK, 4); DA_ES_ATTR(ES_PK, 6); DA_ES_ATTR(ES_PK, 8);
#undef DA_ES_ATTR
    es_cus.store(prop.multiProcessorCount > 0 ? prop.multiProcessorCount : 256);
    es_attr_done.fetch_or(1ull << (dev & 63));
  }
  const bool packed = pk || expand_stream_packed(n_hash);
  size_t lds = packed ? (size_t)pk_row_bytes(ld_d) : (size_t)ld_d * 2;
  lds = std::max<size_t>(lds, 82 * 1024);
  int64_t grid = (int64_t)es_cus.load();
  grid = std::min<int64_t>(grid, (row_end - row_begin) + n / ES_COPIES + 1);
#define DA_ES(P, Q) hipLaunchKernelGGL((k_expand_stream<P, Q>), dim3((unsigned)grid), dim3(ES_THREADS), lds, stream, d_D, ld_d, d_uidx, L.cstart, L.cpos, L.items, \
                                       L.istart, (int)row_begin, (int)row_end, (int)n, n_hash, d_out, ld, L.ticket + launch_no)
  const int64_t nq = ceil_div((pk ? pk_row_bytes(ld_d) : 2 * ld_d) >> 4, ES_THREADS);
#define DA_ES_NQ(F) do { if (nq <= 2) DA_ES(F, 2); else if (nq <= 4) DA_ES(F, 4); else if (nq <= 6) DA_ES(F, 6); else DA_ES(F, 8); } while (0)
  if (pk) DA_ES_NQ(ES_PK);
  else if (packed) DA_ES_NQ(ES_U16_PK);
  else DA_ES_NQ(ES_U16);
#undef DA_ES_NQ
#undef DA_ES
  DA_HIP_TRY(hipGetLastError());
  return DA_OK;
}
int launch_expand_stream(const uint16_t *d_D, int64_t ld_d, const int32_t *d_uidx, int64_t n, int64_t U, int n_hash, double *d_out, int64_t ld,
                         void *d_scratch, hipStream_t stream, hipEvent_t after_lists, bool pk) {
  if (!expand_stream_ok(n, U, n_hash, d_out, ld)) return fail(DA_ERR_UNSUPPORTED, "row expansion: shape not covered");
  int rc = launch_expand_stream_lists(d_uidx, n, U, d_scratch, stream);
  if (rc != DA_OK) return rc;
  if (after_lists) DA_HIP_TRY(hipEventRecord(after_lists, stream));
  return launch_expand_stream_rows(d_D, ld_d, d_uidx, n, U, n_hash, d_out, ld, d_scratch, 0, U, stream, 0, pk);
}

size_t expand_rows_workspace_bytes(int64_t n, int64_t U, int kind, bool is_nw, int n_hash, int nw_max_len) {
  if (kind != DA_OUT_F64 || n < 256 || U > 65536 || U < 1) return 0;
  if (is_nw ? (nw_max_len < 1 || (int64_t)(nw_max_len + 1) * (2 * nw_max_len + 1) > 2048) : (n_hash < 1 || n_hash + 1 > 2048)) return 0;
  return (size_t)U * (size_t)(ceil_div(n, 8) * 8) * 2;
}

int launch_gather_columns(const uint16_t *d_D, int64_t ld_d, const int32_t *d_uidx, const int32_t *d_ufirst, int64_t n, int64_t U,
                          uint16_t *d_F, int64_t ld_f, bool from_first_tile, hipStream_t stream, int table_world, int64_t table_rows_local,
                          int64_t row_begin, int64_t row_end) {
  if (row_end < 0 || row_end > U) row_end = U;
  if (row_begin < 0) row_begin = 0;
  if (U >= 1 && row_begin >= row_end) return DA_OK;
  if (U < 1 || U > 65536 || (ld_d & 7) || ld_d > 65536 || (reinterpret_cast<uintptr_t>(d_D) & 15) || (ld_f & 1))
    return fail(DA_ERR_UNSUPPORTED, "column gather: at most 65536 unique strings, 16-byte aligned table rows");
  const TableRows trows{table_world, table_rows_local};
  const size_t row_bytes = (size_t)ld_d * 2;
  static std::atomic<int> gc_cus;
  static std::atomic<uint64_t> gc_attr_done;
  int dev = 0;
  DA_HIP_TRY(hipGetDevice(&dev));
  if (!((gc_attr_done.load() >> (dev & 63)) & 1u)) {
    hipDeviceProp_t prop;
    DA_HIP_TRY(hipGetDeviceProperties(&prop, dev));
    DA_HIP_TRY(hipFuncSetAttribute(reinterpret_cast<const void *>(k_gather_columns), hipFuncAttributeMaxDynamicSharedMemorySize, 65536 * 2));
    gc_cus.store(prop.multiProcessorCount > 0 ? prop.multiProcessorCount : 256);
    gc_attr_done.fetch_or(1ull << (dev & 63));
  }
  const int gc_wg = row_bytes <= 40 * 1024 ? 2 : 1;
  const int64_t gc_grid = std::min<int64_t>(row_end - row_begin, (int64_t)gc_cus.load() * gc_wg);
  hipLaunchKernelGGL(k_gather_columns, dim3((unsigned)gc_grid), dim3(GC_THREADS), row_bytes, stream, d_D, ld_d, d_uidx, d_ufirst, (int)n,
                     (int)row_end, d_F, ld_f, trows, from_first_tile ? 1 : 0, (int)row_begin);
  DA_HIP_TRY(hipGetLastError());
  return DA_OK;
}

int launch_expand_rows(const uint16_t *d_F, int64_t ld_f, const int32_t *d_uidx, int64_t n, bool is_nw, int n_hash, int nw_max_len,
                       double *d_out, int64_t ld, int64_t band_begin, int64_t band_end, hipStream_t stream) {
  const int T128 = (int)ceil_div(n, 128);
  if (band_end < 0) band_end = mh_sym_bands(n);
  const int64_t t0 = mh_sym_band_prefix(n, band_begin), t1 = mh_sym_band_prefix(n, band_end);
  if (t1 <= t0) return DA_OK;
  const int64_t px = ceil_div(t1 - t0, 8);
  const int stride = is_nw ? 2 * nw_max_len + 1 : 1;
  const int entries = is_nw ? (nw_max_len + 1) * stride : n_hash + 1;
  const size_t lds = 128 * ER_STRIDE + (size_t)entries * 8;
  if (is_nw) hipLaunchKernelGGL(k_expand_rows<true>, dim3((unsigned)(px * 8)), dim3(256), lds, stream, d_F, ld_f, d_uidx, (int)n, n_hash,
                                stride, entries, d_out, ld, T128, t1, px, t0);
  else hipLaunchKernelGGL(k_expand_rows<false>, dim3((unsigned)(px * 8)), dim3(256), lds, stream, d_F, ld_f, d_uidx, (int)n, n_hash,
                          stride, entries, d_out, ld, T128, t1, px, t0);
  DA_HIP_TRY(hipGetLastError());
  return DA_OK;
}

int launch_expand_unique(const uint16_t *d_D, int64_t ld_d, const int32_t *d_uidx, int64_t n, int kind, bool is_nw, int n_hash,
                         void *d_out, int64_t ld, hipStream_t stream, int nw_max_len, uint16_t *d_F, const int32_t *d_ufirst, int64_t U,
                         hipEvent_t after_gather, hipEvent_t after_rows, int table_world, int64_t table_rows_local, bool only_leftover) {
  const TableRows trows{table_world, table_rows_local};
  if (n <= 0) return DA_OK;
  if (n > 0x7fffffffLL) return fail(DA_ERR_UNSUPPORTED, "expand: matrix too large");
  if (kind != DA_OUT_F64 && kind != DA_OUT_COMPACT) return fail(DA_ERR_BAD_ARG, "expand: bad output kind");
  const int TB = (int)ceil_div(n, 64);
  const int64_t tiles = (int64_t)TB * (TB + 1) / 2;
  if (tiles > 0x7fffffffLL) return fail(DA_ERR_UNSUPPORTED, "matrix too large for one launch");
  const int64_t per_xcd = ceil_div(tiles, 8);
  dim3 grid((unsigned)(per_xcd * 8));
  const bool fast = d_F != nullptr && expand_rows_workspace_bytes(n, U, kind, is_nw, n_hash, nw_max_len) != 0 && (ld & 1) == 0 &&
                    (reinterpret_cast<uintptr_t>(d_out) & 15) == 0;
  if (only_leftover && !fast) return fail(DA_ERR_BAD_ARG, "expand: the streaming passes do not cover this shape");
  if (fast && !only_leftover) {
    const int64_t ld_f = ceil_div(n, 8) * 8;
    int rc_g = launch_gather_columns(d_D, ld_d, d_uidx, d_ufirst, n, U, d_F, ld_f, false, stream, table_world, table_rows_local);
    if (rc_g != DA_OK) return rc_g;
    if (after_gather) DA_HIP_TRY(hipEventRecord(after_gather, stream));
    rc_g = launch_expand_rows(d_F, ld_f, d_uidx, n, is_nw, n_hash, nw_max_len, static_cast<double *>(d_out), ld, 0, -1, stream);
    if (rc_g != DA_OK) return rc_g;
  }
  else if (after_gather) DA_HIP_TRY(hipEventRecord(after_gather, stream));
  if (after_rows) DA_HIP_TRY(hipEventRecord(after_rows, stream));
  const int skip_fast = fast ? 1 : 0;
  if (fast) grid.x = leftover_blocks64(n);
#define DA_EXP(F, W, T) hipLaunchKernelGGL((k_expand_unique<F, W, T>), grid, dim3(256), 0, stream, d_D, ld_d, d_uidx, (int)n, n_hash, d_out, ld, TB, tiles, per_xcd, skip_fast, trows)
  if (kind == DA_OUT_F64) { if (is_nw) DA_EXP(true, true, 64); else DA_EXP(true, false, 64); }
  else { if (is_nw) DA_EXP(false, true, 64); else DA_EXP(false, false, 64); }
#undef DA_EXP
  DA_HIP_TRY(hipGetLastError());
  return DA_OK;
}

int launch_finalize_sharded(const uint16_t *d_g, int64_t ld_g, const ShardGeom &geom, bool is_nw, int n_hash,
                            double *d_out, int64_t ld, hipStream_t stream) {
  if (geom.n <= 0) return DA_OK;
  if (geom.n > 0x7fffffffLL || (geom.tile % 64) != 0) return fail(DA_ERR_UNSUPPORTED, "finalize: unsupported geometry");
  const int TB = (int)ceil_div(geom.n, 64);
  const int64_t tiles = (int64_t)TB * (TB + 1) / 2;
// ... 535 lines not shown
```

Before: 334.7 billion.

## Overlap expansion-list build with signatures and pipeline compare by tile-row strips

Moves the expand-stream list construction onto an alternate stream that starts right after the dedup plan, so it overlaps the MinHash signature and dictionary work instead of serialising behind the edge compare. The compare pipeline is now cut at tile-row granularity (a new strip decode in the compare kernel) and can take a small first chunk, sized by a host cost model that reads a row count through a pinned host word. The scan kernel is also rewritten as a per-wave segmented scan, removing the per-iteration block barriers. This adds more streams and events, plus a host-side heuristic that depends on event timing.

```diff
diff --git a/dynaalign_amd/csrc/api.cpp b/dynaalign_amd/csrc/api.cpp
--- a/dynaalign_amd/csrc/api.cpp
+++ b/dynaalign_amd/csrc/api.cpp
@@ -378,6 +378,7 @@
   c.mh_pipe_step = (int)std::max<int64_t>(0, env_i64("DYNAALIGN_MH_PIPE_STEP", 0));
   c.mh_pipe_wg = (int)std::max<int64_t>(0, std::min<int64_t>(4, env_i64("DYNAALIGN_MH_PIPE_WG", 0)));
   c.mh_pipe_head = (int)std::max<int64_t>(0, env_i64("DYNAALIGN_MH_PIPE_HEAD", 0));
+  c.mh_pipe_first = (int)std::max<int64_t>(-1, env_i64("DYNAALIGN_MH_PIPE_FIRST", -1));
   const int pb = (int)env_i64("DYNAALIGN_PLANE_BITS", 0);
   c.plane_bits = (pb == 32 || pb == 16 || pb == 15 || pb == 14 || pb == 12) ? pb : 0;
   c.k2_no_asm = env_flag("DYNAALIGN_K2_NO_ASM");
@@ -496,13 +497,14 @@
 static int env_plane_bits() { return da::config().plane_bits; }
 struct Dictionary { bool ok = false; int max_ids = 0, bits_data = 32; int *d_status = nullptr; };
 static int run_dictionary(const uint32_t *d_sig, int64_t ld_sig, int64_t n, int n_hash, int min_bits, void *d_work, size_t work_bytes,
-                          Dictionary *dict, hipStream_t stream) {
+                          Dictionary *dict, hipStream_t stream, hipEvent_t join = nullptr) {
   if (n > DA_DICT_MAX_N || min_bits == 32) return DA_OK;
   if (!d_work || work_bytes < mh_planes_workspace_bytes(n, n_hash))
     return fail(DA_ERR_BAD_ARG, "workspace smaller than da_mh_planes_workspace_bytes(n, n_hash)");
   int rc;
   if ((rc = launch_mh_dictionary(d_sig, ld_sig, n, n_hash, d_work, &dict->d_status, stream)) != DA_OK) return rc;
   int status[2] = {0, 0};
+  if (join) DA_HIP_TRY(hipStreamWaitEvent(stream, join, 0));
   DA_HIP_TRY(hipMemcpyAsync(status, dict->d_status, sizeof(status), hipMemcpyDeviceToHost, stream));
   DA_HIP_TRY(hipStreamSynchronize(stream));
   dict->ok = status[0] == 0; dict->max_ids = status[1];
@@ -562,7 +564,7 @@
 }
 
 namespace {
-struct PipeRes { hipStream_t side = nullptr, alt[2] = {nullptr, nullptr}; std::vector<hipEvent_t> ev; int dev = 0; };
+struct PipeRes { hipStream_t side = nullptr, alt[2] = {nullptr, nullptr}; std::vector<hipEvent_t> ev; int dev = 0; uint32_t *word = nullptr; };
 struct PipePool { std::mutex m; std::vector<PipeRes *> idle[64]; };
 static PipePool &pipe_pool() { static PipePool *p = new PipePool; return *p; }
 static PipeRes *pipe_acquire(size_t events) {
@@ -578,7 +580,8 @@
     r = new PipeRes;
     r->dev = dev;
     if (hipStreamCreateWithFlags(&r->side, hipStreamNonBlocking) != hipSuccess || hipStreamCreateWithFlags(&r->alt[0], hipStreamNonBlocking) != hipSuccess ||
-        hipStreamCreateWithFlags(&r->alt[1], hipStreamNonBlocking) != hipSuccess) { delete r; return nullptr; }
+        hipStreamCreateWithFlags(&r->alt[1], hipStreamNonBlocking) != hipSuccess ||
+        hipHostMalloc(reinterpret_cast<void **>(&r->word), sizeof(uint32_t), hipHostMallocDefault) != hipSuccess) { delete r; return nullptr; }
   }
   while (r->ev.size() < events) {
     hipEvent_t e = nullptr;
@@ -698,8 +701,9 @@
                                   tr1 < 0 ? (m + 127) / 128 : tr1, st);
   }
 };
+struct Beside { std::function<int()> enqueue; hipEvent_t done = nullptr; };
 static int mh_codes(const uint8_t *d_res, const int64_t *d_off, int64_t m, int k, int n_hash, const uint32_t *d_seeds, bool ask_sparse,
-                    int split_from_bits, MhCodes *c, hipStream_t stream) {
+                    int split_from_bits, MhCodes *c, hipStream_t stream, const Beside &beside = Beside()) {
   int rc;
   const int64_t lds = sig_ld_for(n_hash);
   const size_t wb = mh_planes_workspace_bytes(m, n_hash);
@@ -708,9 +712,10 @@
       (rc = c->pwork.alloc(wb)) != DA_OK) return rc;
   uint32_t *sig = c->sig.as<uint32_t>(), *planes = c->planes.as<uint32_t>();
   if ((rc = launch_minhash_signatures(d_res, d_off, m, k, n_hash, d_seeds, sig, lds, stream)) != DA_OK) return rc;
+  if (beside.enqueue && (rc = beside.enqueue()) != DA_OK) return rc;
   const int min_bits = env_plane_bits();
   const Dictionary &dict = c->dict;
-  if ((rc = run_dictionary(sig, lds, m, n_hash, min_bits, c->pwork.p, wb, &c->dict, stream)) != DA_OK) return rc;
+  if ((rc = run_dictionary(sig, lds, m, n_hash, min_bits, c->pwork.p, wb, &c->dict, stream, beside.done)) != DA_OK) return rc;
   if ((rc = mh_admit(dict, c->pwork.p, m, n_hash, ask_sparse, split_from_bits, &c->adm, stream)) != DA_OK) return rc;
   if (c->adm.form != MhOperand::dense &&
       (c->scratch.alloc(mh_sparse_scratch_words(m, n_hash, dict.max_ids, c->adm.ld_ids) * 4) != DA_OK ||
@@ -723,9 +728,11 @@
   if (c->split()) { c->bits = 8; return launch_ids_to_planes(c->pwork.p, m, n_hash, 8, planes, stream, c->adm.dense); }
   return planes_from(dict, sig, lds, m, n_hash, min_bits, c->pwork.p, planes, &c->bits, stream);
 }
+struct RowsPipeCuts;
 struct MhCall {
   int64_t n; int n_hash; double *out; int64_t ld; hipStream_t stream; MhRoute &route; const MhEvents &ev; const MhCodes &c; const MhDedup &d;
   uint16_t *dtab = nullptr; int64_t ld_d = 0; void *ex = nullptr; bool pk = false;
+  PipeRes *rows_pipe = nullptr; const RowsPipeCuts *rows_cuts = nullptr;
 };
 constexpr int MH_NO_PIPE = -1;
 static int mh_finish(const MhCall &k, int last_event, MhForm taken, int steps) {
@@ -773,54 +780,86 @@
   k.route.chunks = k.route.expand_launches = 1;
   return k.d.rows ? mh_finish(k, 5, MH_ROWS, 5) : mh_finish(k, 6, MH_TILES, 6);
 }
+struct RowsPipeCuts {
+  int wg, first; bool alt; std::vector<int64_t> tr;
+  RowsPipeCuts(const Config &cfg, int64_t U, int n_hash) {
+    const bool two = expand_stream_packed(n_hash);
+    const int64_t T = ceil_div(U, 128), head = cfg.mh_pipe_head > 0 ? cfg.mh_pipe_head : two ? 1 : 4, step = cfg.mh_pipe_step > 0 ? cfg.mh_pipe_step : two ? 8 : 4;
+    wg = cfg.mh_pipe_wg > 0 ? cfg.mh_pipe_wg : two ? 2 : 1;
+    alt = !cfg.mh_pipe_one_stream;
+    const bool built_in = cfg.mh_pipe_head <= 0 && cfg.mh_pipe_step <= 0 && cfg.mh_pipe_wg <= 0 && alt;
+    first = !built_in ? 0 : cfg.mh_pipe_first >= 0 ? (int)std::min<int64_t>(cfg.mh_pipe_first, 7) : two ? 1 : 0;
+    if (T <= 8 || first >= T) first = 0;
+    tr.push_back(0);
+    while (tr.back() < T) tr.push_back(std::min(T, tr.back() + 8 * (tr.size() == 1 ? head : step)));
+  }
+  size_t events() const { return 3 * tr.size() + 3; }
+};
+static int mh_rows_pipe_begin(const PipeLease &lease, const RowsPipeCuts &cuts, const MhDedup &d, int64_t n, hipEvent_t plan_done, DevBuf *ex) {
+  PipeRes *const pr = lease.r;
+  int rc;
+  if ((rc = ex->alloc(expand_stream_scratch_bytes(n, d.U))) != DA_OK) return rc;
+  DA_HIP_TRY(hipStreamWaitEvent(pr->alt[0], plan_done, 0));
+  if ((rc = launch_expand_stream_lists(d.p.uidx, n, d.U, ex->p, pr->alt[0])) != DA_OK) return rc;
+  *pr->word = 0;
+  if (cuts.first > 0)
+    DA_HIP_TRY(hipMemcpyAsync(pr->word, expand_stream_row_starts(ex->p, n, d.U) + 128 * cuts.first, sizeof(uint32_t), hipMemcpyDeviceToHost, pr->alt[0]));
+  DA_HIP_TRY(hipEventRecord(pr->ev[0], pr->alt[0]));
+  return DA_OK;
+}
 static int mh_rows_pipe(const MhCall &k) {
-  const Config &cfg = da::config();
   const MhCodes &c = k.c;
-  const int64_t U = k.d.U, KB = mh_sym_bands(U);
+  const int64_t U = k.d.U;
   const hipStream_t stream = k.stream;
   int rc;
-  const bool two = expand_stream_packed(k.n_hash);
-  const int wg = cfg.mh_pipe_wg > 0 ? cfg.mh_pipe_wg : two ? 2 : 1, head = cfg.mh_pipe_head > 0 ? cfg.mh_pipe_head : two ? 1 : 4,
-            step = cfg.mh_pipe_step > 0 ? cfg.mh_pipe_step : two ? 8 : 4;
-  const bool alt = !cfg.mh_pipe_one_stream;
-  std::vector<int64_t> cuts{0};
-  while (cuts.back() < KB) cuts.push_back(std::min(KB, cuts.back() + (cuts.size() == 1 ? head : step)));
-  const size_t C = cuts.size() - 1;
-  const PipeLease lease(3 * C + 2);
-  PipeRes *const pr = lease.r;
+  PipeRes *const pr = k.rows_pipe;
   if (!pr) return MH_NO_PIPE;
-  hipEvent_t *pe = pr->ev.data();
+  RowsPipeCuts cuts = *k.rows_cuts;
+  int cus = 0;
+  DA_HIP_TRY(hipDeviceGetAttribute(&cus, hipDeviceAttributeMultiprocessorCount, pr->dev));
+  if (cuts.first > 0) {
+    const bool arrived = hipEventQuery(pr->ev[0]) == hipSuccess;
+    (void)hipGetLastError();
+    const int64_t rows = arrived ? (int64_t)*pr->word : 0, h = 8 - cuts.first, rest = h * (h + 1) / 2 + (ceil_div(U, 128) - 8) * h;
+    const double expand_us = (double)rows * (double)k.n * 8.0 / 6.0e6, compare_us = (double)rest * (double)ceil_div(k.n_hash, 32) * 4.0 / ((double)cus * cuts.wg);
+    if (rows < 4 * (int64_t)cus || expand_us < 1.25 * compare_us) cuts.first = 0;
+  }
+  std::vector<int64_t> &tr = cuts.tr;
+  if (cuts.first > 0) tr.insert(tr.begin() + 1, cuts.first);
+  const size_t C = tr.size() - 1;
+  const bool alt = cuts.alt;
+  hipEvent_t *pe = pr->ev.data(), *ce = pe + 3;
   DA_HIP_TRY(hipStreamWaitEvent(pr->side, k.ev[2], 0));
   if ((rc = launch_mh_compare_edges_u16(c.planes.as<uint32_t>(), U, k.n_hash, k.dtab, k.ld_d, stream, c.bits, k.pk)) != DA_OK) return rc;
-  if ((rc = launch_expand_stream_lists(k.d.p.uidx, k.n, U, k.ex, stream)) != DA_OK) return rc;
-  DA_HIP_TRY(hipEventRecord(pe[3 * C], stream));
+  DA_HIP_TRY(hipEventRecord(pe[2], stream));
   if (c.split()) {
     if ((rc = c.lists(stream)) != DA_OK) return rc;
-    DA_HIP_TRY(hipEventRecord(pe[3 * C + 1], stream));
-  }
-  if (alt) { DA_HIP_TRY(hipStreamWaitEvent(pr->alt[0], pe[3 * C], 0)); DA_HIP_TRY(hipStreamWaitEvent(pr->alt[1], pe[3 * C], 0)); }
+    DA_HIP_TRY(hipEventRecord(pe[1], stream));
+  }
+  if (alt) for (const hipStream_t es : pr->alt) { DA_HIP_TRY(hipStreamWaitEvent(es, pe[0], 0)); DA_HIP_TRY(hipStreamWaitEvent(es, pe[2], 0)); }
+  else DA_HIP_TRY(hipStreamWaitEvent(stream, pe[0], 0));
   for (size_t ci = 0; ci < C; ++ci) {
-    if ((rc = launch_mh_compare_bands_u16(c.planes.as<uint32_t>(), U, k.n_hash, k.dtab, k.ld_d, cuts[ci], cuts[ci + 1], ci == 0 ? 4 : wg, pr->side, c.bits,
-                                          k.pk)) != DA_OK) return rc;
+    if ((rc = launch_mh_compare_tile_rows_u16(c.planes.as<uint32_t>(), U, k.n_hash, k.dtab, k.ld_d, tr[ci], tr[ci + 1],
+                                              ci == 0 ? 4 : cuts.wg, pr->side, c.bits, k.pk)) != DA_OK) return rc;
     if (c.split()) {
-      if (ci == 0) { DA_HIP_TRY(hipStreamWaitEvent(pr->side, pe[3 * C], 0)); DA_HIP_TRY(hipStreamWaitEvent(pr->side, pe[3 * C + 1], 0)); }
-      if ((rc = c.fixup(DA_OUT_COMPACT, k.dtab, k.ld_d, pr->side, cuts[ci] * 8, cuts[ci + 1] * 8)) != DA_OK) return rc;
+      if (ci == 0) { DA_HIP_TRY(hipStreamWaitEvent(pr->side, pe[2], 0)); DA_HIP_TRY(hipStreamWaitEvent(pr->side, pe[1], 0)); }
+      if ((rc = c.fixup(DA_OUT_COMPACT, k.dtab, k.ld_d, pr->side, tr[ci], tr[ci + 1])) != DA_OK) return rc;
     }
-    DA_HIP_TRY(hipEventRecord(pe[3 * ci], pr->side));
+    DA_HIP_TRY(hipEventRecord(ce[3 * ci], pr->side));
     const hipStream_t es = alt ? pr->alt[ci & 1] : stream;
-    DA_HIP_TRY(hipStreamWaitEvent(es, pe[3 * ci], 0));
-    DA_HIP_TRY(hipEventRecord(pe[3 * ci + 1], es));
-    if ((rc = launch_expand_stream_rows(k.dtab, k.ld_d, k.d.p.uidx, k.n, U, k.n_hash, k.out, k.ld, k.ex, cuts[ci] * 1024, cuts[ci + 1] * 1024, es,
+    DA_HIP_TRY(hipStreamWaitEvent(es, ce[3 * ci], 0));
+    DA_HIP_TRY(hipEventRecord(ce[3 * ci + 1], es));
+    if ((rc = launch_expand_stream_rows(k.dtab, k.ld_d, k.d.p.uidx, k.n, U, k.n_hash, k.out, k.ld, k.ex, tr[ci] * 128, tr[ci + 1] * 128, es,
                                         (int)ci, k.pk)) != DA_OK) return rc;
-    DA_HIP_TRY(hipEventRecord(pe[3 * ci + 2], es));
-  }
-  if (alt) for (size_t ci = (C >= 2 ? C - 2 : 0); ci < C; ++ci) DA_HIP_TRY(hipStreamWaitEvent(stream, pe[3 * ci + 2], 0));
+    DA_HIP_TRY(hipEventRecord(ce[3 * ci + 2], es));
+  }
+  if (alt) for (size_t ci = (C >= 2 ? C - 2 : 0); ci < C; ++ci) DA_HIP_TRY(hipStreamWaitEvent(stream, ce[3 * ci + 2], 0));
   if ((rc = mh_finish(k, 5, MH_ROWS_PIPE, 2)) != DA_OK) return rc;
   k.route.chunks = k.route.expand_launches = (int)C;
-  MhEvents::ms(k.route, 2, k.ev[2], pe[3 * (C - 1)]);
-  MhEvents::ms(k.route, 3, k.ev[2], pe[3 * C]);
+  MhEvents::ms(k.route, 2, k.ev[2], ce[3 * (C - 1)]);
+  MhEvents::ms(k.route, 3, k.ev[1], pe[0]);
   LaunchUnion expand{k.ev[2]};
-  for (size_t ci = 0; ci < C; ++ci) expand.add(pe[3 * ci + 1], pe[3 * ci + 2]);
+  for (size_t ci = 0; ci < C; ++ci) expand.add(ce[3 * ci + 1], ce[3 * ci + 2]);
   k.route.ms[4] = expand.total;
   return DA_OK;
 }
@@ -854,7 +893,7 @@
   if (c.split() && (rc = c.lists(pr->side)) != DA_OK) return rc;
   for (size_t ci = 0; ci < C; ++ci) {
     const Chunk &ch = chunks[ci];
-    if ((rc = launch_mh_compare_bands_u16(c.planes.as<uint32_t>(), U, k.n_hash, k.dtab, k.ld_d, ch.kb0, ch.kb1, wg, pr->side, c.bits)) != DA_OK) return rc;
+    if ((rc = launch_mh_compare_tile_rows_u16(c.planes.as<uint32_t>(), U, k.n_hash, k.dtab, k.ld_d, ch.kb0 * 8, ch.kb1 * 8, wg, pr->side, c.bits)) != DA_OK) return rc;
     if (c.split() && (rc = c.fixup(DA_OUT_COMPACT, k.dtab, k.ld_d, pr->side, ch.kb0 * 8, ch.kb1 * 8)) != DA_OK) return rc;
     DA_HIP_TRY(hipEventRecord(pe[5 * ci], pr->side));
     DA_HIP_TRY(hipStreamWaitEvent(stream, pe[5 * ci], 0));
@@ -898,27 +937,33 @@
   for (auto &e : ev.e) DA_HIP_TRY(hipEventCreate(&e));
   DA_HIP_TRY(hipEventRecord(ev[0], stream));
   MhDedup d;
+  MhCodes c;
+  DevBuf dtab, ex;
   if ((rc = mh_dedup_plan(d_res, d_off, n, total, n_hash, d_out, ld, &d, stream)) != DA_OK) return rc;
   route.unique = d.U;
   DA_HIP_TRY(hipEventRecord(ev[1], stream));
-  MhCodes c;
+  const bool rows_pipe = d.take && d.rows && !cfg.mh_no_pipe && cfg.mh_expand != MH_EXPAND_ROWS;
+  const RowsPipeCuts cuts(cfg, rows_pipe ? d.U : 0, n_hash);
+  const PipeLease lease(cuts.events(), rows_pipe);
+  Beside lists;
+  if (lease.r) lists = Beside{[&] { return mh_rows_pipe_begin(lease, cuts, d, n, ev[1], &ex); }, lease.r->ev[0]};
   if ((rc = mh_codes(d.take ? d.p.ucodes : d_res, d.take ? d.p.uoff : d_off, d.take ? d.U : n, k, n_hash, d_seeds, !d.take && d.U * 10 >= n * 9,
-                     d.take && !cfg.mh_hybrid_dedup ? 13 : 12, &c, stream)) != DA_OK) return rc;
+                     d.take && !cfg.mh_hybrid_dedup ? 13 : 12, &c, stream, lists)) != DA_OK) return rc;
   route.plane_bits = c.bits;
   if (c.split()) { route.hybrid_pairs = (int64_t)c.adm.pairs; route.hybrid_bits_before = c.dict.bits_data; }
   DA_HIP_TRY(hipEventRecord(ev[2], stream));
   MhCall call{n, n_hash, d_out, ld, stream, route, ev, c, d};
   if (!d.take) return c.adm.form == MhOperand::sparse ? mh_sparse(call) : mh_direct(call);
-  DevBuf dtab, ex;
   call.pk = d.rows && !c.split() && mh_compare_pk_ok(d.U, n_hash, c.bits);
   route.packed_table = call.pk;
   call.ld_d = call.pk ? pk_lo_bytes(d.U) : (d.U + 7) / 8 * 8;
   if ((rc = dtab.alloc(call.pk ? pk_table_bytes(d.U) : (size_t)d.U * (size_t)call.ld_d * 2)) != DA_OK) return rc;
-  if ((rc = ex.alloc(d.rows ? expand_stream_scratch_bytes(n, d.U) : expand_rows_workspace_bytes(n, d.U, DA_OUT_F64, false, n_hash, 0))) != DA_OK) return rc;
-  call.dtab = dtab.as<uint16_t>(); call.ex = ex.p;
+  if (!ex.p && (rc = ex.alloc(d.rows ? expand_stream_scratch_bytes(n, d.U) : expand_rows_workspace_bytes(n, d.U, DA_OUT_F64, false, n_hash, 0))) != DA_OK) return rc;
+  call.dtab = dtab.as<uint16_t>(); call.ex = ex.p; call.rows_pipe = lease.r; call.rows_cuts = &cuts;
   const bool pipe = !cfg.mh_no_pipe && mh_compare_bands_ok(d.U, n_hash, c.bits, dtab.p, call.ld_d) &&
                     (d.rows ? cfg.mh_expand != MH_EXPAND_ROWS : cfg.mh_expand != MH_EXPAND_TILES && (ld & 1) == 0 && (reinterpret_cast<uintptr_t>(d_out) & 15) == 0);
   if (pipe && (rc = d.rows ? mh_rows_pipe(call) : mh_tiles_pipe(call)) != MH_NO_PIPE) return rc;
+  if (lease.r) DA_HIP_TRY(hipStreamWaitEvent(stream, lease.r->ev[0], 0));
   return mh_one_stream(call);
 }
 
diff --git a/dynaalign_amd/csrc/da_common.hpp b/dynaalign_amd/csrc/da_common.hpp
--- a/dynaalign_amd/csrc/da_common.hpp
+++ b/dynaalign_amd/csrc/da_common.hpp
@@ -18,6 +18,7 @@
   int64_t mh_hybrid_min_n = -1;
   int mh_expand = 0;
   int mh_pipe_step = 0, mh_pipe_wg = 0, mh_pipe_head = 0;
+  int mh_pipe_first = -1;
   int plane_bits = 0;
   bool k2_no_asm = false, k2_persist = false;
   int k2_wg_per_cu = 0;
@@ -116,8 +117,8 @@
 int64_t mh_sym_bands(int64_t n);
 int64_t mh_sym_band_prefix(int64_t n, int64_t band);
 bool mh_compare_bands_ok(int64_t n, int n_hash, int plane_bits, const void *d_out, int64_t ld);
-int launch_mh_compare_bands_u16(const uint32_t *d_planes, int64_t n, int n_hash, uint16_t *d_out, int64_t ld, int64_t band_begin,
-                                int64_t band_end, int wg_per_cu, hipStream_t stream, int plane_bits = 12, bool pk = false);
+int launch_mh_compare_tile_rows_u16(const uint32_t *d_planes, int64_t n, int n_hash, uint16_t *d_out, int64_t ld, int64_t tr_begin,
+                                    int64_t tr_end, int wg_per_cu, hipStream_t stream, int plane_bits = 12, bool pk = false);
 int launch_mh_compare_edges_u16(const uint32_t *d_planes, int64_t n, int n_hash, uint16_t *d_out, int64_t ld, hipStream_t stream, int plane_bits = 12,
                                 bool pk = false);
 bool mh_compare_pk_ok(int64_t n, int n_hash, int plane_bits);
@@ -186,6 +187,7 @@
 int launch_expand_stream(const uint16_t *d_D, int64_t ld_d, const int32_t *d_uidx, int64_t n, int64_t U, int n_hash, double *d_out, int64_t ld,
                          void *d_scratch, hipStream_t stream, hipEvent_t after_lists = nullptr, bool pk = false);
 int launch_expand_stream_lists(const int32_t *d_uidx, int64_t n, int64_t U, void *d_scratch, hipStream_t stream);
+const uint32_t *expand_stream_row_starts(const void *d_scratch, int64_t n, int64_t U);
 int launch_expand_stream_rows(const uint16_t *d_D, int64_t ld_d, const int32_t *d_uidx, int64_t n, int64_t U, int n_hash, double *d_out, int64_t ld,
                               void *d_scratch, int64_t row_begin, int64_t row_end, hipStream_t stream, int launch_no,
                               bool pk = false);
diff --git a/dynaalign_amd/csrc/minhash_kernels.hip b/dynaalign_amd/csrc/minhash_kernels.hip
--- a/dynaalign_amd/csrc/minhash_kernels.hip
+++ b/dynaalign_amd/csrc/minhash_kernels.hip
@@ -127,6 +127,23 @@
   while ((q + 1) * h <= l) ++q;
   return q;
 }
+__host__ __device__ __forceinline__ TileId decode_strip(int l, int r0, int h, int T) {
+  TileId o{0, 0, true};
+  const int tri = h * (h + 1) / 2;
+  if (l < tri) {
+    int q = 0;
+    while ((q + 1) * (q + 2) / 2 <= l) ++q;
+    o.tj = r0 + q;
+    o.ti = r0 + (l - q * (q + 1) / 2);
+  } else {
+    l -= tri;
+    const int cq = div_small(l, h);
+    o.tj = r0 + h + cq;
+    o.ti = r0 + (l - cq * h);
+  }
+  o.valid = o.tj < T;
+  return o;
+}
 __host__ __device__ __forceinline__ TileId decode_tile(int64_t L, int TR, int T, bool symmetric) {
   TileId o{0, 0, true};
   const int S = K2_BAND;
@@ -160,21 +177,7 @@
   const int r0 = B * S;
   const int h = (T - r0 < S) ? (T - r0) : S;
   if (h <= 0) { o.valid = false; return o; }
-  int l = (int)(L - prefix(B < nfull ? B : nfull));
-  const int tri = h * (h + 1) / 2;
-  if (l < tri) {
-    int q = 0;
-    while ((q + 1) * (q + 2) / 2 <= l) ++q;
-    o.tj = r0 + q;
-    o.ti = r0 + (l - q * (q + 1) / 2);
-  } else {
-    l -= tri;
-    const int cq = div_small(l, h);
-    o.tj = r0 + h + cq;
-    o.ti = r0 + (l - cq * h);
-  }
-  o.valid = o.tj < T;
-  return o;
+  return decode_strip((int)(L - prefix(B < nfull ? B : nfull)), r0, h, T);
 }
 
 __host__ __device__ inline int64_t count_tiles(int TR, int T, bool symmetric) {
@@ -552,7 +555,7 @@
 template <bool F64, int PL = 12, bool ONE = false, bool PK = false>
 __global__ __launch_bounds__(K2_THREADS, 4) void k_mh_compare_p12(const uint32_t *__restrict__ planes, int64_t n, int n_hash,
                                                                   void *__restrict__ out_v, int64_t ld, int64_t ntiles,
-                                                                  int64_t per_xcd, int wg_per_xcd, int64_t tile_begin) {
+                                                                  int64_t per_xcd, int wg_per_xcd, int64_t tile_begin, int strip_r0, int strip_h) {
   static_assert(PL == 12 || PL == 8, "generated blocks exist for 12 and 8 planes");
   static_assert(!PK || (!F64 && PL == 12 && !ONE), "the packed table is written by the 12-plane band kernel");
   constexpr int SEGS = PL / 4, STAGE_UNITS = 2 * K2_TILE * SEGS;
@@ -573,9 +576,10 @@
   auto source_of = [&](const TileId &t) -> uint64_t { return wave_base + (uint64_t)(wave_u >= 2 ? t.tj : t.ti) * block_bytes; };
   auto next_taken = [&](int from, TileId &t) -> int {
     for (int L = from; L < lim; L += wg_per_xcd) {
-      int To = T;
-      asm volatile("" : "+s"(To));
-      t = decode_tile(L, To, To, true);
+      int To = T, ho = strip_h;
+      asm volatile("" : "+s"(To), "+s"(ho));
+      if (ho > 0) t = decode_strip(L, strip_r0, ho, To);
+      else t = decode_tile(L, To, To, true);
       t.ti = __builtin_amdgcn_readfirstlane(t.ti);
       t.tj = __builtin_amdgcn_readfirstlane(t.tj);
       if (t.valid && a12_takes(t.ti, t.tj, n, ld, out_v, F64 || PK)) return L;
@@ -1093,10 +1097,10 @@
         if (config().k2_wg_per_cu > 0) wg_per_xcd = config().k2_wg_per_cu * 32;
         if ((int64_t)wg_per_xcd > per_xcd) wg_per_xcd = (int)(per_xcd > 0 ? per_xcd : 1);
         hipLaunchKernelGGL((k_mh_compare_p12<decltype(F64)::value, 8, false>), dim3((unsigned)(8 * wg_per_xcd)), block, 0, stream, d_planes, n, n_hash,
-                           d_out, ld, ntiles, per_xcd, wg_per_xcd, (int64_t)0);
+                           d_out, ld, ntiles, per_xcd, wg_per_xcd, (int64_t)0, 0, 0);
       } else {
         hipLaunchKernelGGL((k_mh_compare_p12<decltype(F64)::value, 8, true>), grid, block, 0, stream, d_planes, n, n_hash, d_out, ld, ntiles, per_xcd,
-                           (int)per_xcd, (int64_t)0);
+                           (int)per_xcd, (int64_t)0, 0, 0);
       }
     });
   if (a16)
@@ -1128,9 +1132,9 @@
     if ((int64_t)wg_per_xcd > per_xcd) wg_per_xcd = (int)(per_xcd > 0 ? per_xcd : 1);
     const dim3 pgrid((unsigned)(8 * wg_per_xcd));
     if (kind == DA_OUT_F64)
-      hipLaunchKernelGGL(k_mh_compare_p12<true>, pgrid, block, 0, stream, d_planes, n, n_hash, d_out, ld, ntiles, per_xcd, wg_per_xcd, (int64_t)0);
+      hipLaunchKernelGGL(k_mh_compare_p12<true>, pgrid, block, 0, stream, d_planes, n, n_hash, d_out, ld, ntiles, per_xcd, wg_per_xcd, (int64_t)0, 0, 0);
     else
-      hipLaunchKernelGGL(k_mh_compare_p12<false>, pgrid, block, 0, stream, d_planes, n, n_hash, d_out, ld, ntiles, per_xcd, wg_per_xcd, (int64_t)0);
+      hipLaunchKernelGGL(k_mh_compare_p12<false>, pgrid, block, 0, stream, d_planes, n, n_hash, d_out, ld, ntiles, per_xcd, wg_per_xcd, (int64_t)0, 0, 0);
   } else if (a12) {
     if (f64)
       hipLaunchKernelGGL(k_mh_compare_a12<true>, grid, block, 0, stream, d_planes, n, n_hash, d_out, ld, ntiles, per_xcd);
@@ -1179,12 +1183,22 @@
   return (plane_bits == 12 || plane_bits == 8) && n_hash > K2_GROUP && n_hash <= 65535 && !config().k2_no_asm &&
          k2_out_ok(d_out, ld, false) && T * (T + 1) / 2 < 0x7fffffffLL;
 }
-int launch_mh_compare_bands_u16(const uint32_t *d_planes, int64_t n, int n_hash, uint16_t *d_out, int64_t ld, int64_t band_begin,
-                                int64_t band_end, int wg_per_cu, hipStream_t stream, int plane_bits, bool pk) {
+int launch_mh_compare_tile_rows_u16(const uint32_t *d_planes, int64_t n, int n_hash, uint16_t *d_out, int64_t ld, int64_t tr_begin,
+                                    int64_t tr_end, int wg_per_cu, hipStream_t stream, int plane_bits, bool pk) {
   if (!mh_compare_bands_ok(n, n_hash, plane_bits, d_out, ld) ||
       (pk && (!mh_compare_pk_ok(n, n_hash, plane_bits) || !k2_out_ok(d_out, ld, true))))
     return fail(DA_ERR_UNSUPPORTED, "banded compare: shape not covered");
-  const int64_t t0 = mh_sym_band_prefix(n, band_begin), t1 = mh_sym_band_prefix(n, band_end);
+  const int64_t T = ceil_div(n, K2_TILE);
+  tr_end = std::min(tr_end, T);
+  if (tr_begin < 0 || tr_begin >= tr_end) return DA_OK;
+  const bool bands = tr_begin % K2_BAND == 0 && (tr_end % K2_BAND == 0 || tr_end == T);
+  if (const int64_t cut = (tr_begin / K2_BAND + 1) * K2_BAND; !bands && cut < tr_end) {
+    const int rc = launch_mh_compare_tile_rows_u16(d_planes, n, n_hash, d_out, ld, tr_begin, cut, wg_per_cu, stream, plane_bits, pk);
+    return rc != DA_OK ? rc : launch_mh_compare_tile_rows_u16(d_planes, n, n_hash, d_out, ld, cut, tr_end, wg_per_cu, stream, plane_bits, pk);
+  }
+  const int strip_r0 = bands ? 0 : (int)tr_begin, strip_h = bands ? 0 : (int)(tr_end - tr_begin);
+  const int64_t t0 = bands ? mh_sym_band_prefix(n, tr_begin / K2_BAND) : 0,
+                t1 = bands ? mh_sym_band_prefix(n, ceil_div(tr_end, K2_BAND)) : (int64_t)strip_h * (strip_h + 1) / 2 + (T - tr_end) * strip_h;
   if (t1 <= t0) return DA_OK;
   static std::atomic<int> cus_cache;
   if (!cus_cache.load()) {
@@ -1199,13 +1213,13 @@
   if ((int64_t)wg_per_xcd > per_xcd) wg_per_xcd = (int)per_xcd;
   if (plane_bits == 8)
     hipLaunchKernelGGL((k_mh_compare_p12<false, 8, false>), dim3((unsigned)(8 * wg_per_xcd)), dim3(K2_THREADS), 0, stream, d_planes, n, n_hash,
-                       static_cast<void *>(d_out), ld, t1, per_xcd, wg_per_xcd, t0);
+                       static_cast<void *>(d_out), ld, t1, per_xcd, wg_per_xcd, t0, strip_r0, strip_h);
   else if (pk)
     hipLaunchKernelGGL((k_mh_compare_p12<false, 12, false, true>), dim3((unsigned)(8 * wg_per_xcd)), dim3(K2_THREADS), 0, stream, d_planes, n, n_hash,
-                       static_cast<void *>(d_out), ld, t1, per_xcd, wg_per_xcd, t0);
+                       static_cast<void *>(d_out), ld, t1, per_xcd, wg_per_xcd, t0, strip_r0, strip_h);
   else
     hipLaunchKernelGGL(k_mh_compare_p12<false>, dim3((unsigned)(8 * wg_per_xcd)), dim3(K2_THREADS), 0, stream, d_planes, n, n_hash,
-                       static_cast<void *>(d_out), ld, t1, per_xcd, wg_per_xcd, t0);
+                       static_cast<void *>(d_out), ld, t1, per_xcd, wg_per_xcd, t0, strip_r0, strip_h);
   DA_HIP_TRY(hipGetLastError());
   return DA_OK;
 }
@@ -1578,35 +1592,34 @@
 }
 __global__ __launch_bounds__(1024) void k_es_scan(const uint32_t *__restrict__ cnt, int U, uint32_t *__restrict__ cstart, uint32_t *__restrict__ istart) {
   __shared__ uint64_t wsum[16];
-  __shared__ uint64_t carry_s;
   const int tid = threadIdx.x, lane = tid & 63, wave = tid >> 6;
-  if (tid == 0) carry_s = 0;
-  __syncthreads();
-  for (int base = 0; base < U; base += 1024) {
-    const int u = base + tid;
-    const uint32_t c = u < U ? cnt[u] : 0u;
-    const uint64_t v = (uint64_t)c | ((uint64_t)((c + ES_COPIES - 1) / ES_COPIES) << 32);
+  const int seg = ((U + 15) / 16 + 63) & ~63, u0 = wave * seg, u1 = min(U, u0 + seg);
+  auto both = [](uint32_t c) -> uint64_t { return (uint64_t)c | ((uint64_t)((c + ES_COPIES - 1) / ES_COPIES) << 32); };
+  uint64_t acc = 0;
+  for (int u = u0 + lane; u < u1; u += 64) acc += both(cnt[u]);
+#pragma unroll
+  for (int d = 32; d >= 1; d >>= 1) acc += __shfl_xor(acc, d, 64);
+  if (lane == 0) wsum[wave] = acc;
+  __syncthreads();
+  uint64_t carry = 0;
+  for (int w = 0; w < wave; ++w) carry += wsum[w];
+  for (int base = u0; base < u1; base += 64) {
+    const int u = base + lane;
+    const uint64_t v = u < u1 ? both(cnt[u]) : 0;
     uint64_t x = v;
 #pragma unroll
     for (int d = 1; d < 64; d <<= 1) {
       const uint64_t y = __shfl_up(x, d, 64);
       if (lane >= d) x += y;
     }
-    if (lane == 63) wsum[wave] = x;
-    __syncthreads();
-    uint64_t woff = 0;
-    for (int w = 0; w < wave; ++w) woff += wsum[w];
-    const uint64_t carry = carry_s;
-    if (u < U) {
-      const uint64_t e = carry + woff + x - v;
+    if (u < u1) {
+      const uint64_t e = carry + x - v;
       cstart[u] = (uint32_t)e;
       istart[u] = (uint32_t)(e >> 32);
     }
-    __syncthreads();
-    if (tid == 1023) carry_s = carry + woff + x;
-    __syncthreads();
-  }
-  if (tid == 0) { cstart[U] = (uint32_t)carry_s; istart[U] = (uint32_t)(carry_s >> 32); }
+    carry += __shfl(x, 63, 64);
+  }
+  if (tid == 1023) { cstart[U] = (uint32_t)carry; istart[U] = (uint32_t)(carry >> 32); }
 }
 __global__ __launch_bounds__(256) void k_es_fill(const int32_t *__restrict__ uidx, int n, int U, const uint32_t *__restrict__ cstart,
                                                  const uint32_t *__restrict__ istart, uint32_t *__restrict__ cursor, int32_t *__restrict__ cpos,
@@ -1738,6 +1751,7 @@
   L.items = reinterpret_cast<int2 *>((reinterpret_cast<uintptr_t>(L.cpos + n) + 15) & ~(uintptr_t)15);
   return L;
 }
+const uint32_t *expand_stream_row_starts(const void *d_scratch, int64_t n, int64_t U) { return es_layout(const_cast<void *>(d_scratch), n, U).cstart; }
 int launch_expand_stream_lists(const int32_t *d_uidx, int64_t n, int64_t U, void *d_scratch, hipStream_t stream) {
   const EsLists L = es_layout(d_scratch, n, U);
   DA_HIP_TRY(hipMemsetAsync(L.cnt, 0, ((size_t)U * 2 + ES_TICKETS) * 4, stream));
```

New measurement: 333.5 billion (median of 3 runs). No clear change (-0.4%).
